# leaner-forever/SEGS-SLAM

Hardware: AMD Instinct MI355X
Metric: mapper train-iters/sec (fwd+bwd raster) (higher is better)
Workload: dtype f32; 1 GPU; 1080p_3m: 3000000 Gaussians, 1920x1080, 1 keyframe per GPU, fwd+bwd raster; P=3000000, P_visible=2096178, num_rendered=10472370, instances_binned=7913347, instances_live=6766534, width=1920, height=1080, parallelism=keyframe-dp1, forward=resident (no host sync), hipgraph=off

## Files before the change

include/segs_raster.h:

```cpp
#ifndef SEGS_RASTER_H_
#define SEGS_RASTER_H_

#include <stddef.h>
#include <stdint.h>

#ifdef __cplusplus
extern "C" {
#endif

#define SEGS_OK 0
#define SEGS_ERR_INVALID_ARGUMENT (-1)
#define SEGS_ERR_UNSUPPORTED (-2)
#define SEGS_ERR_ALLOC (-3)

typedef char* (*segs_alloc_fn)(void* ctx, size_t bytes);

const char* segs_last_error(void);

#define SEGS_RASTER_SKIP_NONPOSITIVE_OPACITY 1u
#define SEGS_RASTER_KEEP_DEAD_INSTANCES 2u
#define SEGS_RASTER_GATHER_TILES_TOUCHED 4u
#define SEGS_RASTER_TEST_NARROW_PACK 8u
#define SEGS_RASTER_UNFUSED_BINNING 16u
#define SEGS_RASTER_TIGHT_BINNING 32u
#define SEGS_RASTER_MFMA_MOMENTS 64u
uint32_t segs_raster_set_flags(uint32_t flags);

uint32_t* segs_raster_set_status_mirror(uint32_t* host_mapped_status);

size_t segs_geometry_bytes(int P);
size_t segs_image_bytes(int width, int height);
size_t segs_binning_bytes(int num_rendered);

int segs_rasterize_forward(segs_alloc_fn geometry_alloc, void* geometry_ctx,
                           segs_alloc_fn binning_alloc, void* binning_ctx,
                           segs_alloc_fn image_alloc, void* image_ctx,
                           int P, int D, int M,
                           const float* background, int width, int height,
                           const float* means3D, const float* shs, const float* colors_precomp,
                           const float* opacities, const float* scales, float scale_modifier,
                           const float* rotations, const float* cov3D_precomp,
                           const float* viewmatrix, const float* projmatrix, const float* cam_pos,
                           float tan_fovx, float tan_fovy, int prefiltered,
                           float* out_color, int* radii, void* stream, int* num_rendered);

int segs_rasterize_backward(int P, int D, int M, int R,
                            const float* background, int width, int height,
                            const float* means3D, const float* shs, const float* colors_precomp,
                            const float* scales, float scale_modifier, const float* rotations,
                            const float* cov3D_precomp, const float* viewmatrix, const float* projmatrix,
                            const float* campos, float tan_fovx, float tan_fovy, const int* radii,
                            char* geom_buffer, char* binning_buffer, char* image_buffer,
                            const float* dL_dpix, float* dL_dmean2D, float* dL_dconic, float* dL_dopacity,
                            float* dL_dcolor, float* dL_dmean3D, float* dL_dcov3D, float* dL_dsh,
                            float* dL_dscale, float* dL_drot, void* stream);

int segs_visible_filter(int P, int M, int width, int height, const float* means3D, const float* scales,
                        float scale_modifier, const float* rotations, const float* cov3D_precomp,
                        const float* viewmatrix, const float* projmatrix, float tan_fovx, float tan_fovy,
                        int prefiltered, int* radii, void* stream);

int segs_visible_filter_log_scales(int P, int width, int height, const float* means3D, const float* scaling_log, int stride,
                                   const float* rotations, const float* viewmatrix, const float* projmatrix, float tan_fovx,
                                   float tan_fovy, int* radii, void* stream);

int segs_mark_visible(int P, const float* means3D, const float* viewmatrix, const float* projmatrix,
                      uint8_t* present, void* stream);

int segs_project2_image(int P, int D, int M, int width, int height, const float* means3D, const float* shs,
                        const float* colors_precomp, const float* opacities, const float* scales,
                        float scale_modifier, const float* rotations, const float* cov3D_precomp,
                        const float* viewmatrix, const float* projmatrix, const float* cam_pos,
                        float tan_fovx, float tan_fovy, int prefiltered, float* out_color, float* points_image,
                        int* radii, void* stream);

int segs_debug_unpack_geometry(const char* geom_buffer, int P, const int* radii, float* means2D ,
                               float* conic_opacity , float* depths , uint32_t* tiles_touched ,
                               uint32_t* point_offsets , float* rgb , void* stream);
int segs_debug_unpack_binning(const char* binning_buffer, const char* geom_buffer, int P, int R, int width, int height,
                              uint64_t* keys_sorted , uint32_t* point_list , void* stream);
int segs_debug_instance_values(const char* binning_buffer, int R, uint32_t* values , void* stream);
int segs_debug_unpack_image(const char* image_buffer, int width, int height, uint32_t* ranges ,
                            float* final_T , uint32_t* n_contrib , void* stream);

int segs_debug_preprocess_backward(int P, int width, int height, const float* means3D, const int* radii,
                                   const float* scales, float scale_modifier, const float* rotations,
                                   const float* cov3D_precomp, const float* viewmatrix, const float* projmatrix,
                                   float tan_fovx, float tan_fovy, const float* dL_dmean2D, const float* dL_dconic,
                                   float* dL_dmean3D, float* dL_dcov3D, float* dL_dscale, float* dL_drot, void* stream);

int segs_sort_pairs(const uint64_t* keys_in, const uint32_t* vals_in, uint64_t* keys_out, uint32_t* vals_out,
                    int n, int end_bit, char* temp, void* stream);

size_t segs_resident_binning_bytes(int P, int capacity);
int segs_rasterize_forward_resident(char* geom_buffer, char* binning_buffer, char* image_buffer, int capacity,
                                    int geom_rows, int P, int D, int M, const float* background, int width, int height,
                                    const float* means3D, const float* shs, const float* colors_precomp,
                                    const float* opacities, const float* scales, float scale_modifier,
                                    const float* rotations, const float* cov3D_precomp, const float* viewmatrix,
                                    const float* projmatrix, const float* cam_pos, float tan_fovx, float tan_fovy,
                                    float* out_color, int* radii, uint32_t* status, void* stream);
int segs_rasterize_backward_resident(char* geom_buffer, char* binning_buffer, char* image_buffer, int capacity,
                                     int geom_rows, int P, int D, int M, const float* background, int width, int height,
                                     const float* means3D, const float* shs, const float* scales, float scale_modifier,
                                     const float* rotations, const float* cov3D_precomp, const float* viewmatrix,
                                     const float* projmatrix, const float* campos, float tan_fovx, float tan_fovy,
                                     const int* radii, const float* dL_dpix, float* dL_dmean2D, float* dL_dconic,
                                     float* dL_dopacity, float* dL_dcolor, float* dL_dmean3D, float* dL_dcov3D,
                                     float* dL_dsh, float* dL_dscale, float* dL_drot, void* stream);

typedef struct segs_projection_targets {
  float* records;
  int* radii;
  uint32_t* tiles_touched;
  uint32_t* depth_keys;
  uint32_t* tile_ranges;
  uint32_t* depth_overflow;
  int num_tiles;
  uint32_t flags;
} segs_projection_targets;
int segs_resident_projection_targets(char* geom_buffer, char* binning_buffer, char* image_buffer, int capacity, int geom_rows,
                                     int P, int width, int height, int* radii, uint32_t* status, segs_projection_targets* out);
int segs_rasterize_forward_resident_projected(char* geom_buffer, char* binning_buffer, char* image_buffer, int capacity,
                                              int geom_rows, int P, const float* background, int width, int height,
                                              float* out_color, uint32_t* status, void* stream);

typedef struct segs_depth_outputs {
  float* depth;
  float* alpha;
} segs_depth_outputs;
typedef struct segs_depth_grads {
  const float* dL_ddepth;
  const float* dL_dalpha;
} segs_depth_grads;
int segs_rasterize_forward_depth(segs_alloc_fn geometry_alloc, void* geometry_ctx,
                                 segs_alloc_fn binning_alloc, void* binning_ctx,
                                 segs_alloc_fn image_alloc, void* image_ctx,
                                 int P, int D, int M,
                                 const float* background, int width, int height,
                                 const float* means3D, const float* shs, const float* colors_precomp,
                                 const float* opacities, const float* scales, float scale_modifier,
                                 const float* rotations, const float* cov3D_precomp,
                                 const float* viewmatrix, const float* projmatrix, const float* cam_pos,
                                 float tan_fovx, float tan_fovy, int prefiltered,
                                 float* out_color, int* radii, const segs_depth_outputs* depth_out, void* stream,
                                 int* num_rendered);
int segs_rasterize_backward_depth(int P, int D, int M, int R,
                                  const float* background, int width, int height,
                                  const float* means3D, const float* shs, const float* colors_precomp,
                                  const float* scales, float scale_modifier, const float* rotations,
                                  const float* cov3D_precomp, const float* viewmatrix, const float* projmatrix,
                                  const float* campos, float tan_fovx, float tan_fovy, const int* radii,
                                  char* geom_buffer, char* binning_buffer, char* image_buffer,
                                  const float* dL_dpix, float* dL_dmean2D, float* dL_dconic, float* dL_dopacity,
                                  float* dL_dcolor, float* dL_dmean3D, float* dL_dcov3D, float* dL_dsh,
                                  float* dL_dscale, float* dL_drot, const segs_depth_grads* depth_grads, void* stream);
int segs_rasterize_forward_resident_depth(char* geom_buffer, char* binning_buffer, char* image_buffer, int capacity,
                                          int geom_rows, int P, int D, int M, const float* background, int width, int height,
                                          const float* means3D, const float* shs, const float* colors_precomp,
                                          const float* opacities, const float* scales, float scale_modifier,
                                          const float* rotations, const float* cov3D_precomp, const float* viewmatrix,
                                          const float* projmatrix, const float* cam_pos, float tan_fovx, float tan_fovy,
                                          float* out_color, int* radii, uint32_t* status, const segs_depth_outputs* depth_out,
                                          void* stream);
int segs_rasterize_forward_resident_projected_depth(char* geom_buffer, char* binning_buffer, char* image_buffer, int capacity,
                                                    int geom_rows, int P, const float* background, int width, int height,
                                                    float* out_color, uint32_t* status, const segs_depth_outputs* depth_out,
                                                    void* stream);
int segs_rasterize_backward_resident_depth(char* geom_buffer, char* binning_buffer, char* image_buffer, int capacity,
                                           int geom_rows, int P, int D, int M, const float* background, int width, int height,
                                           const float* means3D, const float* shs, const float* scales, float scale_modifier,
                                           const float* rotations, const float* cov3D_precomp, const float* viewmatrix,
                                           const float* projmatrix, const float* campos, float tan_fovx, float tan_fovy,
                                           const int* radii, const float* dL_dpix, float* dL_dmean2D, float* dL_dconic,
                                           float* dL_dopacity, float* dL_dcolor, float* dL_dmean3D, float* dL_dcov3D,
                                           float* dL_dsh, float* dL_dscale, float* dL_drot, const segs_depth_grads* depth_grads,
                                           void* stream);

typedef struct segs_camera_grads {
  float* dL_dviewmatrix;
  float* dL_dprojmatrix;
  char* temp;
} segs_camera_grads;
size_t segs_camera_grad_temp_bytes(int rows);
int segs_rasterize_backward_camera(int P, int D, int M, int R,
                                   const float* background, int width, int height,
                                   const float* means3D, const float* shs, const float* colors_precomp,
                                   const float* scales, float scale_modifier, const float* rotations,
                                   const float* cov3D_precomp, const float* viewmatrix, const float* projmatrix,
                                   const float* campos, float tan_fovx, float tan_fovy, const int* radii,
                                   char* geom_buffer, char* binning_buffer, char* image_buffer,
                                   const float* dL_dpix, float* dL_dmean2D, float* dL_dconic, float* dL_dopacity,
                                   float* dL_dcolor, float* dL_dmean3D, float* dL_dcov3D, float* dL_dsh,
                                   float* dL_dscale, float* dL_drot, const segs_depth_grads* depth_grads,
                                   const segs_camera_grads* camera_grads, void* stream);
int segs_rasterize_backward_resident_camera(char* geom_buffer, char* binning_buffer, char* image_buffer, int capacity,
                                            int geom_rows, int P, int D, int M, const float* background, int width, int height,
                                            const float* means3D, const float* shs, const float* scales, float scale_modifier,
                                            const float* rotations, const float* cov3D_precomp, const float* viewmatrix,
                                            const float* projmatrix, const float* campos, float tan_fovx, float tan_fovy,
                                            const int* radii, const float* dL_dpix, float* dL_dmean2D, float* dL_dconic,
                                            float* dL_dopacity, float* dL_dcolor, float* dL_dmean3D, float* dL_dcov3D,
                                            float* dL_dsh, float* dL_dscale, float* dL_drot, const segs_depth_grads* depth_grads,
                                            const segs_camera_grads* camera_grads, void* stream);
int segs_debug_preprocess_backward_camera(int P, int width, int height, const float* means3D, const int* radii,
                                          const float* scales, float scale_modifier, const float* rotations,
                                          const float* cov3D_precomp, const float* viewmatrix, const float* projmatrix,
                                          float tan_fovx, float tan_fovy, const float* dL_dmean2D, const float* dL_dconic,
                                          float* dL_dmean3D, float* dL_dcov3D, float* dL_dscale, float* dL_drot,
                                          const float* dL_dz, const segs_camera_grads* camera_grads, void* stream);

int segs_profile_begin(unsigned kernel_mask);
int segs_profile_end(void);
int segs_profile_kernel_count(void);
const char* segs_profile_kernel_name(int id);
int segs_profile_query(int id, double* total_ms, long* launches);

#ifdef __cplusplus
}
#endif
#endif
```

segs-slam_amd/_capi.py:

```python
from __future__ import annotations

import ctypes as C
import os
import subprocess

_HERE = os.path.dirname(os.path.abspath(__file__))
CSRC = os.path.join(_HERE, "csrc")
LIB_PATH = os.environ.get("SEGS_RASTER_LIB") or os.path.join(CSRC, "libsegs_raster.so")

ALLOC_FN = C.CFUNCTYPE(C.c_void_p, C.c_void_p, C.c_size_t)


class NeuralDims(C.Structure):
    _fields_ = [("feat_dim", C.c_int), ("n_offsets", C.c_int), ("appearance_dim", C.c_int), ("use_feat_bank", C.c_int),
                ("add_opacity_dist", C.c_int), ("add_cov_dist", C.c_int), ("add_color_dist", C.c_int)]


class ProjectionTargets(C.Structure):
    _fields_ = [("records", C.c_void_p), ("radii", C.c_void_p), ("tiles_touched", C.c_void_p), ("depth_keys", C.c_void_p),
                ("tile_ranges", C.c_void_p), ("depth_overflow", C.c_void_p), ("num_tiles", C.c_int), ("flags", C.c_uint32)]


class DepthOutputs(C.Structure):
    _fields_ = [("depth", C.c_void_p), ("alpha", C.c_void_p)]


class DepthGrads(C.Structure):
    _fields_ = [("dL_ddepth", C.c_void_p), ("dL_dalpha", C.c_void_p)]


class CameraGrads(C.Structure):
    _fields_ = [("dL_dviewmatrix", C.c_void_p), ("dL_dprojmatrix", C.c_void_p), ("temp", C.c_void_p)]


class AdamSegment(C.Structure):
    _fields_ = [("offset", C.c_int64), ("count", C.c_int64), ("lr", C.c_double)]

_vp, _i, _f, _sz = C.c_void_p, C.c_int, C.c_float, C.c_size_t
SYMBOLS = {
    "segs_last_error": (C.c_char_p, []),
    "segs_raster_set_flags": (C.c_uint, [C.c_uint]),
    "segs_raster_set_status_mirror": (_vp, [_vp]),
    "segs_training_statis": (_i, [_i, _i] + [_vp] * 9),
    "segs_training_statis_guarded": (_i, [_i, _i] + [_vp] * 10),
    "segs_anchor_growing_temp_bytes": (_sz, [_i, _i]),
    "segs_anchor_growing_level": (_i, [_i, _i, _i, _i] + [_vp] * 7 + [_f, _f, _f, _i] + [_vp] * 5),
    "segs_neural_set_flags": (C.c_uint, [C.c_uint]),
    "segs_neural_param_layout": (_i, [_vp, _vp, _vp, _vp, _vp]),
    "segs_neural_temp_bytes": (_sz, [_vp, _i]),
    "segs_neural_forward": (_i, [_vp, _i] + [_vp] * 16),
    "segs_neural_forward_projected": (_i, [_vp, _i] + [_vp] * 16 + [_i, _i, _f, _f, _f, _vp, _vp]),
    "segs_neural_backward": (_i, [_vp, _i] + [_vp] * 17 + [_f, _vp, _vp, _vp]),
    "segs_geometry_bytes": (_sz, [_i]),
    "segs_image_bytes": (_sz, [_i, _i]),
    "segs_binning_bytes": (_sz, [_i]),
    "segs_rasterize_forward": (_i, [ALLOC_FN, _vp, ALLOC_FN, _vp, ALLOC_FN, _vp, _i, _i, _i, _vp, _i, _i, _vp, _vp, _vp,
                                     _vp, _vp, _f, _vp, _vp, _vp, _vp, _vp, _f, _f, _i, _vp, _vp, _vp, C.POINTER(_i)]),
    "segs_rasterize_backward": (_i, [_i, _i, _i, _i, _vp, _i, _i, _vp, _vp, _vp, _vp, _f, _vp, _vp, _vp, _vp, _vp, _f, _f,
                                      _vp, _vp, _vp, _vp, _vp, _vp, _vp, _vp, _vp, _vp, _vp, _vp, _vp, _vp, _vp]),
    "segs_resident_binning_bytes": (_sz, [_i, _i]),
    "segs_rasterize_forward_resident": (_i, [_vp, _vp, _vp, _i, _i, _i, _i, _i, _vp, _i, _i, _vp, _vp, _vp, _vp, _vp, _f, _vp, _vp, _vp,
                                              _vp, _vp, _f, _f, _vp, _vp, _vp, _vp]),
    "segs_resident_projection_targets": (_i, [_vp, _vp, _vp, _i, _i, _i, _i, _i, _vp, _vp, _vp]),
    "segs_rasterize_forward_resident_projected": (_i, [_vp, _vp, _vp, _i, _i, _i, _vp, _i, _i, _vp, _vp, _vp]),
    "segs_rasterize_backward_resident": (_i, [_vp, _vp, _vp, _i, _i, _i, _i, _i, _vp, _i, _i, _vp, _vp, _vp, _f, _vp, _vp, _vp, _vp, _vp,
                                               _f, _f, _vp, _vp, _vp, _vp, _vp, _vp, _vp, _vp, _vp, _vp, _vp, _vp]),
}
for _name in ("segs_rasterize_forward", "segs_rasterize_backward", "segs_rasterize_forward_resident",
              "segs_rasterize_forward_resident_projected", "segs_rasterize_backward_resident"):
    _res, _args = SYMBOLS[_name]
    _at = len(_args) - (2 if _name == "segs_rasterize_forward" else 1)
    SYMBOLS[_name + "_depth"] = (_res, _args[:_at] + [_vp] + _args[_at:])
for _name in ("segs_rasterize_backward", "segs_rasterize_backward_resident"):
    _res, _args = SYMBOLS[_name + "_depth"]
    SYMBOLS[_name + "_camera"] = (_res, _args[:-1] + [_vp] + _args[-1:])
SYMBOLS["segs_camera_grad_temp_bytes"] = (_sz, [_i])
SYMBOLS.update({
    "segs_visible_filter": (_i, [_i, _i, _i, _i, _vp, _vp, _f, _vp, _vp, _vp, _vp, _f, _f, _i, _vp, _vp]),
    "segs_visible_filter_log_scales": (_i, [_i, _i, _i, _vp, _vp, _i, _vp, _vp, _vp, _f, _f, _vp, _vp]),
    "segs_mark_visible": (_i, [_i, _vp, _vp, _vp, _vp, _vp]),
    "segs_project2_image": (_i, [_i, _i, _i, _i, _i, _vp, _vp, _vp, _vp, _vp, _f, _vp, _vp, _vp, _vp, _vp, _f, _f, _i,
                                  _vp, _vp, _vp, _vp]),
    "segs_debug_unpack_geometry": (_i, [_vp, _i, _vp, _vp, _vp, _vp, _vp, _vp, _vp, _vp]),
    "segs_debug_instance_values": (_i, [_vp, _i, _vp, _vp]),
    "segs_debug_unpack_binning": (_i, [_vp, _vp, _i, _i, _i, _i, _vp, _vp, _vp]),
    "segs_debug_unpack_image": (_i, [_vp, _i, _i, _vp, _vp, _vp, _vp]),
    "segs_debug_preprocess_backward": (_i, [_i, _i, _i, _vp, _vp, _vp, _f, _vp, _vp, _vp, _vp, _f, _f, _vp, _vp, _vp,
                                             _vp, _vp, _vp, _vp]),
    "segs_debug_preprocess_backward_camera": (_i, [_i, _i, _i, _vp, _vp, _vp, _f, _vp, _vp, _vp, _vp, _f, _f, _vp, _vp, _vp,
                                                    _vp, _vp, _vp, _vp, _vp, _vp]),
    "segs_sort_pairs": (_i, [_vp, _vp, _vp, _vp, _i, _i, _vp, _vp]),
    "segs_knn_temp_bytes": (_sz, [_i]),
    "segs_knn_mean_dist2": (_i, [_i, _vp, _vp, _vp, _vp]),
    "segs_transform_points": (_i, [_i, _vp, _vp, _vp, _vp]),
    "segs_scale_and_transform_points": (_i, [_i, _f, _vp, _vp, _vp, _vp, _vp, _vp, _vp]),
    "segs_reproject_depths_pinhole": (_i, [_i, _i, _f, _f, _f, _f, _vp, _vp, _vp, _vp]),
    "segs_search_neighborhood_depth": (_i, [_i, _i, _f, _f, _f, _f, _f, _vp, _vp, _vp, _vp, _vp, _vp, _vp]),
    "segs_l1_ssim_temp_bytes": (_sz, [_i, _i]),
    "segs_l1_ssim_loss": (_i, [_vp, _vp, _i, _i, _f, _vp, _vp, _vp, _vp]),
    "segs_freq_pyramid": (_i, [_vp, _i, _i, _i, _i, _vp, _vp, _vp, _vp]),
    "segs_spectrum_magnitude": (_i, [_vp, _sz, _vp, _vp]),
    "segs_freq_temp_bytes": (_sz, [_i, _i, _vp, _vp]),
    "segs_freq_spectrum_loss": (_i, [_i, _i, _vp, _vp, _vp, _vp, _vp, _vp, _vp, _vp, _vp]),
    "segs_freq_pyramid_backward_add": (_i, [_vp, _i, _i, _i, _i, _vp, _vp, _vp, _vp]),
    "segs_freq_plan_create": (_i, [_i, _i, _i, _vp, _f, _vp]),
    "segs_freq_plan_destroy": (None, [_vp]),
    "segs_freq_plan_levels": (_i, [_vp, _vp, _vp, _vp]),
    "segs_freq_target_floats": (_sz, [_vp]),
    "segs_freq_target": (_i, [_vp, _vp, _vp, _vp]),
    "segs_freq_loss": (_i, [_vp, _vp, _vp, _vp, _vp, _vp, _vp]),
    "segs_adam_step": (_i, [_vp, _vp, _vp, _vp, _vp, _i, C.c_double, C.c_double, C.c_double, C.c_int64, _f, _i, _vp]),
    "segs_adam_step_guarded": (_i, [_vp, _vp, _vp, _vp, _vp, _i, C.c_double, C.c_double, C.c_double, C.c_int64, _f, _i, _vp, _vp]),
    "segs_adam_step_device": (_i, [_vp, _vp, _vp, _vp, _vp, _i, C.c_double, C.c_double, C.c_double, _vp, _i, _f, _i, _vp, _vp]),
    "segs_adam_step_graph": (_i, [_vp, _vp, _vp, _vp, _vp, _i, _vp, C.c_double, C.c_double, C.c_double, _vp, _f, _i, _vp, _vp]),
    "segs_set_doubles": (_i, [_vp, _vp, _i, _vp]),
    "segs_profile_begin": (_i, [C.c_uint]),
    "segs_profile_end": (_i, []),
    "segs_profile_kernel_count": (_i, []),
    "segs_profile_kernel_name": (C.c_char_p, [_i]),
    "segs_profile_query": (_i, [_i, C.POINTER(C.c_double), C.POINTER(C.c_long)]),
})

_lib = None


def build(force: bool = False) -> str:
    cmd = ["make", "-C", CSRC, "-s", "-j4"] + (["-B"] if force else [])
    subprocess.check_call(cmd)
    return LIB_PATH


def lib() -> C.CDLL:
    global _lib
    if _lib is None:
        if not os.path.exists(LIB_PATH):
            raise RuntimeError(
                f"{LIB_PATH} is missing: the HIP extension must be built (python -c 'import __graft_entry__ as g; "
                "g.build()' or make -C segs-slam_amd/csrc). There is no CPU fallback.")
        import torch
        l = C.CDLL(LIB_PATH)
        for name, (res, args) in SYMBOLS.items():
            try:
                fn = getattr(l, name)
            except AttributeError as e:
                raise RuntimeError(f"libsegs_raster.so does not export {name}") from e
            fn.restype = res
            fn.argtypes = args
        _lib = l
    return _lib


class SegsError(RuntimeError):
    pass


def check(status: int, what: str) -> None:
    if status != 0:
        msg = lib().segs_last_error()
        raise SegsError(f"{what} failed with status {status}: {msg.decode() if msg else ''}")
```

segs-slam_amd/csrc/binning.hip:

```cpp
#include <hip/hip_runtime.h>
#include <cstdint>
#include "gs_layout.h"
#include "kernels.h"

namespace segs {

constexpr int PREFIX_ROWS = PREFIX_ROWS_PER_WG;

__global__ void __launch_bounds__(1024) scan_block_sums_kernel(uint32_t* __restrict__ block_sums, int nblocks,
                                                               const uint32_t* __restrict__ depth_range,
                                                               uint32_t* __restrict__ total) {
  __shared__ uint32_t w_sum[16], w_dmax[16], w_dnmin[16];
  const int tid = threadIdx.x, lane = tid & 63, wv = tid >> 6;
  uint32_t sum = 0, dmax = 0, dnmin = 0;
  for (int i = tid; i < nblocks; i += 1024) {
    sum += block_sums[i];
    dmax = max(dmax, depth_range[i]);
    dnmin = max(dnmin, depth_range[nblocks + i]);
  }
#pragma unroll
  for (int off = 32; off > 0; off >>= 1) {
    sum += __shfl_down(sum, off, 64);
    dmax = max(dmax, (uint32_t)__shfl_down((int)dmax, off, 64));
    dnmin = max(dnmin, (uint32_t)__shfl_down((int)dnmin, off, 64));
// ... 247 lines not shown
    if (col < nchunks) {
      constexpr int ND = 1 << BITS;
      for (int d = threadIdx.x; d < ND; d += SORT_THREADS) chunk_hist[(size_t)d * nchunks + col] = 0u;
    }
    return;
  }
  if (chunk_id >= nchunks) return;
  const int b0 = chunk_id * chunk_tiles;
  auto load_tile = [&](int b, K* dst) {
    const size_t wave_base = (size_t)b * SORT_TILE + (size_t)wv * (SORT_TILE / 4);
#pragma unroll
    for (int r = 0; r < SORT_ITEMS_PER_THREAD; r++) {
      const size_t i = wave_base + (size_t)r * 64 + lane;
      dst[r] = (b < nblocks && i < (size_t)n) ? keys[i] : (K)DEAD_KEY_OF(K);
    }
  };
  load_tile(b0, kreg);
  for (int t = 0; t < chunk_tiles; t++) {
    const int b = b0 + t;
    if (b >= nblocks) break;
    for (int i = tid; i < 4 * NDIG; i += SORT_THREADS) (&cnt[0][0])[i] = 0;
    if (t + 1 < chunk_tiles) load_tile(b + 1, knext);
    __syncthreads();
    const size_t wave_base = (size_t)b * SORT_TILE + (size_t)wv * (SORT_TILE / 4);
#pragma unroll
    for (int r = 0; r < SORT_ITEMS_PER_THREAD; r++) {
      const size_t i = wave_base + (size_t)r * 64 + lane;
      if (i < (size_t)n && !(drop_dead && kreg[r] == (K)DEAD_KEY_OF(K))) atomicAdd(&my[digit_of<BITS>(kreg[r], shift, km) & dmask], 1u);
    }
    __syncthreads();
#pragma unroll
    for (int j = 0; j < DPT; j++) {
      const int d = tid * DPT + j;
      tile_prefix[(size_t)b * NDIG + d] = running[j];
      running[j] += cnt[0][d] + cnt[1][d] + cnt[2][d] + cnt[3][d];
    }
    __syncthreads();
#pragma unroll
    for (int r = 0; r < SORT_ITEMS_PER_THREAD; r++) kreg[r] = knext[r];
  }
#pragma unroll
  for (int j = 0; j < DPT; j++) chunk_hist[(size_t)(tid * DPT + j) * nchunks + chunk_id] = running[j];
}

__global__ void __launch_bounds__(256) radix_scan_kernel(uint32_t* __restrict__ block_hist, int nblocks,
                                                         uint32_t* __restrict__ digit_totals) {
  constexpr int ITEMS = 8;
  __shared__ uint32_t wave_tot[4];
  const int tid = threadIdx.x, lane = tid & 63, wv = tid >> 6;
  uint32_t* row = block_hist + (size_t)blockIdx.x * nblocks;
  uint32_t carry = 0;
  for (int base = 0; base < nblocks; base += 256 * ITEMS) {
    const int i0 = base + tid * ITEMS;
    uint32_t v[ITEMS], sum = 0;
#pragma unroll
    for (int q = 0; q < ITEMS; q++) { v[q] = (i0 + q < nblocks) ? row[i0 + q] : 0u; sum += v[q]; }
    uint32_t x = sum;
#pragma unroll
    for (int off = 1; off < 64; off <<= 1) {
      const uint32_t y = __shfl_up(x, off, 64);
      if (lane >= off) x += y;
    }
    if (lane == 63) wave_tot[wv] = x;
    __syncthreads();
    uint32_t wbase = 0, total = 0;
#pragma unroll
    for (int w = 0; w < 4; w++) { const uint32_t t = wave_tot[w]; if (w < wv) wbase += t; total += t; }
    uint32_t run = carry + wbase + x - sum;
#pragma unroll
    for (int q = 0; q < ITEMS; q++) { if (i0 + q < nblocks) row[i0 + q] = run; run += v[q]; }
    carry += total;
    __syncthreads();
  }
  if (tid == 0) digit_totals[blockIdx.x] = carry;
}

template <typename K, int BITS, bool AUX>
__global__ void __launch_bounds__(SORT_THREADS) radix_scatter_kernel(
    const K* __restrict__ keys_in, const uint32_t* __restrict__ vals_in, K* __restrict__ keys_out,
    uint32_t* __restrict__ vals_out, int n, int shift, uint32_t dmin, int dbits, const uint32_t* __restrict__ tile_prefix,
    const uint32_t* __restrict__ chunk_prefix , const uint32_t* __restrict__ digit_totals,
    int nblocks, int nchunks, const uint32_t* __restrict__ n_dev, int drop_dead, uint32_t* __restrict__ n_live_out,
    const uint32_t* __restrict__ aux_in, uint32_t* __restrict__ aux_out, int nbits ,
    int chunk_tiles ,
    int pack_shift ,
    uint2* __restrict__ ranges_out ,
    uint32_t* __restrict__ status, uint32_t* __restrict__ status_mirror ,
    int write_keys ) {
  const KeyMap km{dmin, dbits};
  const uint32_t dmask = (1u << nbits) - 1u;
  if (ranges_out != nullptr && status != nullptr && blockIdx.x == 0 && threadIdx.x == 0) {
    const uint32_t ntot = status[0];
    const uint32_t over = (ntot > (uint32_t)n || status[2] != 0u) ? 1u : 0u;
    status[2] = 0u;
    status[3] = over;
    const uint32_t live = min(n_dev ? *n_dev : ntot, min(ntot, (uint32_t)n));
    status[1] = live;
    if (status_mirror) { status_mirror[0] = ntot; status_mirror[1] = live; status_mirror[3] = over; }
  }
  if (n_dev) n = (int)min(*n_dev, (uint32_t)n);
  constexpr int NDIG = 1 << BITS;
  constexpr int DPT = NDIG / SORT_THREADS;
  static_assert(NDIG % SORT_THREADS == 0 && BITS <= 11, "digit | rank << BITS must fit the rank of 2048 keys");
  __shared__ K s_keys[SORT_TILE];
  __shared__ uint32_t s_vals[SORT_TILE];
  __shared__ uint32_t s_aux[AUX ? SORT_TILE : 1];
  __shared__ uint32_t cnt[4][NDIG];
  __shared__ uint32_t local_start[NDIG];
  __shared__ int32_t gdelta[NDIG];
  __shared__ uint32_t scan_tmp[4];
  const int tid = threadIdx.x, lane = tid & 63, wv = tid >> 6;
  for (int i = tid; i < 4 * NDIG; i += SORT_THREADS) (&cnt[0][0])[i] = 0;
  __syncthreads();

#if defined(SEGS_MEASURE) && defined(SORT_TILE_IDENTITY)
  const int tile_id = (int)blockIdx.x;
#else
  const int tiles_in_use = (int)(((size_t)n + SORT_TILE - 1) / SORT_TILE);
  const int tiles_per_xcd = (tiles_in_use + 7) >> 3;
  const int tile_id = (int)(blockIdx.x & 7u) * tiles_per_xcd + (int)(blockIdx.x >> 3);
  if (tiles_in_use == 0 && n_live_out != nullptr && blockIdx.x == 0 && tid == 0) *n_live_out = 0u;
  if ((int)(blockIdx.x >> 3) >= tiles_per_xcd) return;
#endif
  if (tile_id >= nblocks) return;
  const size_t tile_base = (size_t)tile_id * SORT_TILE;
  const size_t wave_base = tile_base + (size_t)wv * (SORT_TILE / 4);
  const int nvalid = (size_t)n > tile_base ? (int)min((size_t)SORT_TILE, (size_t)n - tile_base) : 0;

  K key[SORT_ITEMS_PER_THREAD];
  uint32_t val[SORT_ITEMS_PER_THREAD];
  uint32_t aux[AUX ? SORT_ITEMS_PER_THREAD : 1];
  uint32_t drank[SORT_ITEMS_PER_THREAD];
  volatile uint32_t* my = cnt[wv];
#pragma unroll
  for (int r = 0; r < SORT_ITEMS_PER_THREAD; r++) {
    const size_t i = wave_base + (size_t)r * 64 + lane;
    const bool valid = i < (size_t)n;
    key[r] = valid ? keys_in[i] : (K)0;
    val[r] = vals_in ? (valid ? vals_in[i] : 0u) : (uint32_t)i;
    if (AUX) aux[r] = valid ? aux_in[val[r]] : 0u;
    if (!AUX && pack_shift > 0 && valid) val[r] |= min(aux_in[i], (0xFFFFFFFFu >> pack_shift)) << pack_shift;
  }
#pragma unroll
  for (int r = 0; r < SORT_ITEMS_PER_THREAD; r++) {
    const size_t i = wave_base + (size_t)r * 64 + lane;
    const bool valid = i < (size_t)n && !(drop_dead && key[r] == (K)DEAD_KEY_OF(K));
    const uint32_t d = valid ? (digit_of<BITS>(key[r], shift, km) & dmask) : 0u;
    const uint64_t vmask = __ballot(valid);
    const uint64_t peers = match_digit<BITS>(d, vmask, nbits);
    const uint32_t below = mbcnt(peers);
    uint32_t old = 0;
    if (valid) old = my[d];
    __builtin_amdgcn_wave_barrier();
    if (valid && below == 0) my[d] = old + (uint32_t)__popcll(peers);
    __builtin_amdgcn_wave_barrier();
    drank[r] = valid ? (d | ((old + below) << BITS)) : 0xFFFFFFFFu;
  }
  __syncthreads();

  uint32_t run[DPT], tot[DPT], thread_run = 0, thread_tot = 0;
#pragma unroll
  for (int j = 0; j < DPT; j++) {
    const int d = tid * DPT + j;
    uint32_t r = 0;
#pragma unroll
    for (int w = 0; w < 4; w++) { const uint32_t c = cnt[w][d]; cnt[w][d] = r; r += c; }
    run[j] = r; thread_run += r;
    tot[j] = digit_totals[d]; thread_tot += tot[j];
  }
  uint32_t x = thread_run;
#pragma unroll
  for (int off = 1; off < 64; off <<= 1) {
    uint32_t y = __shfl_up(x, off, 64);
    if (lane >= off) x += y;
  }
  if (lane == 63) scan_tmp[wv] = x;
  uint32_t tx = thread_tot;
#pragma unroll
  for (int off = 1; off < 64; off <<= 1) {
    uint32_t y = __shfl_up(tx, off, 64);
    if (lane >= off) tx += y;
  }
  __shared__ uint32_t tot_tmp[4];
  if (lane == 63) tot_tmp[wv] = tx;
  __syncthreads();
  uint32_t lbase = 0, gbase = 0;
  for (int w = 0; w < wv; w++) { lbase += scan_tmp[w]; gbase += tot_tmp[w]; }
  uint32_t lstart = lbase + x - thread_run, gstart = gbase + tx - thread_tot;
#pragma unroll
  for (int j = 0; j < DPT; j++) {
    const int d = tid * DPT + j;
    local_start[d] = lstart;
    gdelta[d] = (int32_t)(gstart + chunk_prefix[(size_t)d * nchunks + tile_id / chunk_tiles] +
                          tile_prefix[(size_t)tile_id * NDIG + d] - lstart);
    lstart += run[j]; gstart += tot[j];
  }
  const int nout = drop_dead ? (int)(scan_tmp[0] + scan_tmp[1] + scan_tmp[2] + scan_tmp[3]) : nvalid;
  if (n_live_out != nullptr && tile_id == 0 && tid == 0) *n_live_out = tot_tmp[0] + tot_tmp[1] + tot_tmp[2] + tot_tmp[3];
  __syncthreads();

#pragma unroll
  for (int r = 0; r < SORT_ITEMS_PER_THREAD; r++) {
    if (drank[r] != 0xFFFFFFFFu) {
      const uint32_t d = drank[r] & (uint32_t)(NDIG - 1);
      const uint32_t pos = local_start[d] + cnt[wv][d] + (drank[r] >> BITS);
      s_keys[pos] = key[r];
      s_vals[pos] = val[r];
      if (AUX) s_aux[pos] = aux[r];
    }
  }
  __syncthreads();
#pragma unroll 4
  for (int r = 0; r < SORT_ITEMS_PER_THREAD; r++) {
    const int lp = r * SORT_THREADS + tid;
    if (lp < nout) {
      const K k = s_keys[lp];
#if defined(SEGS_MEASURE) && defined(ABLATE_SCATTER_LINEAR)
      const size_t gp = tile_base + (size_t)lp + (size_t)(gdelta[digit_of<BITS>(k, shift, km) & dmask] & 0);
#else
      const size_t gp = (size_t)((int64_t)lp + (int64_t)gdelta[digit_of<BITS>(k, shift, km) & dmask]);
#endif
#if defined(SEGS_MEASURE) && defined(ABLATE_SCATTER_NO_STORE)
      if (k == (K)0x12345677 && gp == 77) keys_out[gp] = k;
      continue;
#endif
      if (write_keys) keys_out[gp] = k;
      vals_out[gp] = s_vals[lp];
      if (AUX) aux_out[gp] = s_aux[lp];
      if constexpr (sizeof(K) == 4) {
        if (ranges_out != nullptr) {
          const K prev = lp > 0 ? s_keys[lp - 1] : ~k, next = lp + 1 < nout ? s_keys[lp + 1] : ~k;
          if (k != prev) atomicMin(&ranges_out[k].x, (uint32_t)gp);
          if (k != next) atomicMax(&ranges_out[k].y, (uint32_t)gp + 1u);
        }
      }
    }
  }
}

#define SEGS_INSTANTIATE_RADIX(K, BITS)                                                                                          \
  template __global__ void radix_count_kernel<K, BITS>(const K*, int, int, uint32_t, int, uint32_t*, uint32_t*, int, int,       \
                                                       const uint32_t*, int, int, int);                                                  \
  template __global__ void radix_scatter_kernel<K, BITS, false>(const K*, const uint32_t*, K*, uint32_t*, int, int, uint32_t, int, \
                                                                const uint32_t*, const uint32_t*, const uint32_t*, int, int,        \
                                                                const uint32_t*, int, uint32_t*, const uint32_t*, uint32_t*, int, int, int, \
                                                                uint2*, uint32_t*, uint32_t*, int);
SEGS_INSTANTIATE_RADIX(uint64_t, 8)
SEGS_INSTANTIATE_RADIX(uint32_t, 8)
SEGS_INSTANTIATE_RADIX(uint32_t, 9)
SEGS_INSTANTIATE_RADIX(uint32_t, 11)
#undef SEGS_INSTANTIATE_RADIX
#define SEGS_INSTANTIATE_AUX(BITS)                                                                                                     \
  template __global__ void radix_scatter_kernel<uint32_t, BITS, true>(const uint32_t*, const uint32_t*, uint32_t*, uint32_t*, int, int, \
                                                                      uint32_t, int, const uint32_t*, const uint32_t*, const uint32_t*, \
                                                                      int, int, const uint32_t*, int, uint32_t*, const uint32_t*, uint32_t*, int, int, int, \
                                                                      uint2*, uint32_t*, uint32_t*, int);
SEGS_INSTANTIATE_AUX(8)
SEGS_INSTANTIATE_AUX(9)
#undef SEGS_INSTANTIATE_AUX

__global__ void __launch_bounds__(256) identify_tile_ranges_kernel(int L, const uint32_t* __restrict__ keys,
                                                                   uint2* __restrict__ ranges, const uint32_t* __restrict__ n_dev,
                                                                   uint32_t* __restrict__ status, uint32_t* __restrict__ status_mirror,
                                                                   const uint32_t* __restrict__ n_live ) {
  static_assert(RANGE_KEYS_PER_THREAD == 4, "one uint4 per thread");
  const int idx = blockIdx.x * 256 + threadIdx.x;
  if (n_dev) {
    const uint32_t n = *n_dev;
    if (idx == 0 && status) {
      const uint32_t over = (n > (uint32_t)L || status[2] != 0u) ? 1u : 0u;
      status[2] = 0u;
      status[3] = over;
      const uint32_t live = n_live ? min(*n_live, min(n, (uint32_t)L)) : min(n, (uint32_t)L);
      status[1] = live;
      if (status_mirror) { status_mirror[0] = n; status_mirror[1] = live; status_mirror[3] = over; }
    }
    L = (int)min(n, (uint32_t)L);
  }
  if (n_live) L = (int)min(*n_live, (uint32_t)L);
  const int i0 = idx * RANGE_KEYS_PER_THREAD;
  if (i0 >= L) return;
  uint32_t k[RANGE_KEYS_PER_THREAD];
  if (i0 + RANGE_KEYS_PER_THREAD <= L) {
    const uint4 v = *reinterpret_cast<const uint4*>(keys + i0);
    k[0] = v.x; k[1] = v.y; k[2] = v.z; k[3] = v.w;
  } else {
#pragma unroll
    for (int q = 0; q < RANGE_KEYS_PER_THREAD; q++) k[q] = i0 + q < L ? keys[i0 + q] : 0u;
  }
  uint32_t prev = i0 > 0 ? keys[i0 - 1] : 0u;
#pragma unroll
  for (int q = 0; q < RANGE_KEYS_PER_THREAD; q++) {
    const int i = i0 + q;
    if (i < L) {
      const uint32_t cur = k[q];
      if (i == 0) ranges[cur].x = 0;
      else if (cur != prev) { ranges[prev].y = i; ranges[cur].x = i; }
      if (i == L - 1) ranges[cur].y = L;
      prev = cur;
    }
  }
}

__global__ void __launch_bounds__(256) unpack_geometry_kernel(
    int P, const float* __restrict__ rec, const BinInfo* __restrict__ bin, const int* __restrict__ radii,
    float* __restrict__ means2D, float* __restrict__ conic_opacity, float* __restrict__ depths,
    uint32_t* __restrict__ tiles_touched, float* __restrict__ rgb) {
  const int idx = blockIdx.x * 256 + threadIdx.x;
  if (idx >= P) return;
  const bool vis = radii[idx] > 0;
  const float* r = rec + (size_t)idx * REC_DWORDS;
  means2D[2 * (size_t)idx + 0] = vis ? r[REC_X] : 0.f;
  means2D[2 * (size_t)idx + 1] = vis ? r[REC_Y] : 0.f;
  conic_opacity[4 * (size_t)idx + 0] = vis ? r[REC_CA] : 0.f;
  conic_opacity[4 * (size_t)idx + 1] = vis ? r[REC_CB] : 0.f;
  conic_opacity[4 * (size_t)idx + 2] = vis ? r[REC_CC] : 0.f;
  conic_opacity[4 * (size_t)idx + 3] = vis ? r[REC_O] : 0.f;
  depths[idx] = vis ? r[REC_DEPTH] : 0.f;
  tiles_touched[idx] = bin[idx].tiles_touched;
  if (rgb) {
    rgb[3 * (size_t)idx + 0] = vis ? r[REC_R] : 0.f;
    rgb[3 * (size_t)idx + 1] = vis ? r[REC_G] : 0.f;
    rgb[3 * (size_t)idx + 2] = vis ? r[REC_B] : 0.f;
  }
}

__global__ void __launch_bounds__(256) make_depth_keys_kernel(int P, const BinInfo* __restrict__ bin, uint32_t dcull,
                                                              uint32_t* __restrict__ keys, uint32_t* __restrict__ vals,
                                                              uint2* __restrict__ ranges, int num_tiles) {
  const int i = blockIdx.x * 256 + threadIdx.x;
  for (int t = i; t < num_tiles; t += gridDim.x * 256) ranges[t] = make_uint2(RANGE_EMPTY_START, 0u);
  if (i >= P) return;
  const uint4 b = reinterpret_cast<const uint4*>(bin)[i];
  keys[i] = b.w ? b.x : dcull;
  (void)vals;
}
__global__ void __launch_bounds__(256) ordered_block_sums_kernel(int P, const uint32_t* touched, const uint32_t* __restrict__ order,
                                                                 uint32_t* __restrict__ block_sums, uint32_t* sorted_touched,
                                                                 const uint32_t* __restrict__ ng_dev ,
                                                                 uint32_t* __restrict__ order_rw, int pack_shift) {
  __shared__ uint32_t wave_sums[4];
  const int ng = ng_dev ? (int)min(*ng_dev, (uint32_t)P) : P;
  uint32_t s = 0;
#pragma unroll
  for (int r = 0; r < PREFIX_ROWS; r++) {
    const int slot = (blockIdx.x * PREFIX_ROWS + r) * 256 + threadIdx.x;
    uint32_t v = 0u;
    if (slot < ng) {
      if (pack_shift > 0) {
        const uint32_t packed = order_rw[slot], idx = packed & ((1u << pack_shift) - 1u);
        v = packed >> pack_shift;
        if (v == (0xFFFFFFFFu >> pack_shift)) v = touched[idx];
        order_rw[slot] = idx;
      } else {
        v = order ? touched[order[slot]] : touched[slot];
      }
    }
    if (slot < P) sorted_touched[slot] = v;
    s += v;
  }
#pragma unroll
  for (int off = 32; off > 0; off >>= 1) s += __shfl_down(s, off, 64);
  if ((threadIdx.x & 63) == 0) wave_sums[threadIdx.x >> 6] = s;
  __syncthreads();
  if (threadIdx.x == 0) block_sums[blockIdx.x] = wave_sums[0] + wave_sums[1] + wave_sums[2] + wave_sums[3];
}
__global__ void __launch_bounds__(1024) point_offsets_kernel(int P, const BinInfo* __restrict__ bin, uint32_t* __restrict__ offsets) {
  __shared__ uint32_t wave_tot[16];
  __shared__ uint32_t carry_s;
  const int tid = threadIdx.x, lane = tid & 63, wv = tid >> 6;
  if (tid == 0) carry_s = 0;
  __syncthreads();
  for (int base = 0; base < P; base += 1024) {
    const int i = base + tid;
    uint32_t x = i < P ? bin[i].tiles_touched : 0u;
#pragma unroll
    for (int off = 1; off < 64; off <<= 1) {
      uint32_t y = __shfl_up(x, off, 64);
      if (lane >= off) x += y;
    }
    if (lane == 63) wave_tot[wv] = x;
    __syncthreads();
    uint32_t wbase = 0;
    for (int w = 0; w < wv; w++) wbase += wave_tot[w];
    const uint32_t carry = carry_s;
    if (i < P) offsets[i] = carry + wbase + x;
    __syncthreads();
    if (tid == 1023) carry_s = carry + wbase + x;
    __syncthreads();
  }
}

__global__ void __launch_bounds__(256) normalize_ranges_kernel(int num_tiles, uint2* __restrict__ ranges) {
  const int t = blockIdx.x * 256 + threadIdx.x;
  if (t < num_tiles && ranges[t].y == 0u) ranges[t].x = 0u;
}

__global__ void __launch_bounds__(256) strip_mask_kernel(int n, const uint32_t* __restrict__ vals, uint32_t* __restrict__ out) {
  const int i = blockIdx.x * 256 + threadIdx.x;
  if (i < n) out[i] = vals[i] & ID_MASK;
}

}

namespace segs {
__global__ void __launch_bounds__(256) rebuild_keys_kernel(int R, const uint32_t* __restrict__ tile_keys, const uint32_t* __restrict__ vals,
                                                           const BinInfo* __restrict__ bin, uint64_t* __restrict__ keys64) {
  const int i = blockIdx.x * 256 + threadIdx.x;
  if (i >= R) return;
  keys64[i] = ((uint64_t)tile_keys[i] << 32) | (uint64_t)bin[vals[i] & ID_MASK].depth_bits;
}
}
```

segs-slam_amd/csrc/capi.hip:

```cpp
#include <hip/hip_runtime.h>
#include <cstdio>
#include <cstdlib>
#include <algorithm>
#include <cstring>
#include <string>
#include <vector>
#include "../../include/segs_raster.h"
#include "gs_layout.h"
#include "kernels.h"

using namespace segs;

namespace {
thread_local std::string g_err;
}
int segs::set_error(int code, const char* what) {
  g_err = what;
  return code;
}
int segs::set_hip_error(hipError_t e, const char* where) {
  g_err = std::string(where) + ": " + hipGetErrorString(e);
  return (int)e > 0 ? (int)e : 1;
}

namespace {

thread_local uint32_t g_flags = 0u;
thread_local uint32_t* g_status_mirror = nullptr;

int fail(int code, const char* what) { return segs::set_error(code, what); }
int hip_fail(hipError_t e, const char* where) { return segs::set_hip_error(e, where); }
#define HIP_TRY(expr)                                   \
  do {                                                  \
    hipError_t _e = (expr);                             \
    if (_e != hipSuccess) return hip_fail(_e, #expr);   \
  } while (0)
#define LAUNCH_TRY(name)                                \
  do {                                                  \
    hipError_t _e = hipGetLastError();                  \
    if (_e != hipSuccess) return hip_fail(_e, name);    \
  } while (0)

enum KernelId { K_PREPROCESS_FWD = 0, K_SCAN, K_DUPLICATE, K_RADIX_COUNT, K_RADIX_SCAN, K_RADIX_SCATTER, K_RANGES,
                K_RENDER_FWD, K_RENDER_BWD, K_PREPROCESS_BWD, K_MEMSET, K_COUNT };
const char* const kKernelNames[K_COUNT] = {"preprocess_fwd_kernel", "scan_block_sums_kernel", "duplicate_with_keys_kernel",
                                           "radix_count_kernel", "radix_scan_kernel", "radix_scatter_kernel",
                                           "identify_tile_ranges_kernel", "render_fwd_kernel", "render_bwd_kernel",
                                           "preprocess_bwd_kernel", "memset"};
struct Profiler {
  unsigned mask = 0;
  std::vector<hipEvent_t> pool;
  size_t used = 0;
  struct Span { int id; size_t e0, e1; };
  std::vector<Span> spans;
  double total_ms[K_COUNT] = {0};
  long count[K_COUNT] = {0};
  hipEvent_t get() {
    if (used == pool.size()) { hipEvent_t e; if (hipEventCreate(&e) != hipSuccess) return nullptr; pool.push_back(e); }
    return pool[used++];
  }
} g_prof;
struct ProfScope {
  int id; hipStream_t st; size_t e0 = 0; bool on;
  ProfScope(int id_, hipStream_t st_) : id(id_), st(st_), on((g_prof.mask >> id_) & 1u) {
    if (on) { e0 = g_prof.used; hipEvent_t e = g_prof.get(); if (e) (void)hipEventRecord(e, st); else on = false; }
  }
  ~ProfScope() {
    if (on) { size_t e1 = g_prof.used; hipEvent_t e = g_prof.get(); if (e) { (void)hipEventRecord(e, st); g_prof.spans.push_back({id, e0, e1}); } }
  }
};
#define PROF(id) ProfScope _prof_scope_##id(id, st)

uint32_t getHigherMsb(uint32_t n) {
  uint32_t msb = sizeof(n) * 4, step = msb;
  while (step > 1) {
    step /= 2;
    if (n >> msb) msb += step; else msb -= step;
  }
  if (n >> msb) msb++;
  return msb;
}

int count_chunk_tiles(int nblocks) {
#ifdef SEGS_MEASURE
  static const int chunk_override = [] { const char* e = getenv("SEGS_COUNT_CHUNK"); const int v = e ? atoi(e) : 0; return (v == 1 || v == 2 || v == 4) ? v : 0; }();
  if (chunk_override > 0) return chunk_override;
#endif
  return nblocks <= 256 ? 1 : (nblocks <= 2048 ? 2 : SORT_COUNT_CHUNK_TILES);
}
struct SortFusion {
  uint2* ranges = nullptr;
  uint32_t* status = nullptr;
  uint32_t* status_mirror = nullptr;
  bool keep_sorted_keys = true;
};
template <typename K, int BITS = 8>
int sort_pairs(char* bin, const BinningLayout& L, int n, int end_bit, uint32_t dmin, int dbits, hipStream_t st,
               const uint32_t* n_dev = nullptr, bool drop_dead = false, bool iota_vals = false, const uint32_t* aux_in = nullptr,
               uint32_t* aux_final = nullptr, int pack_shift = 0 ,
               const SortFusion& fuse = SortFusion(), const K* first_keys = nullptr ) {
  if (n <= 0) return SEGS_OK;
  uint32_t* n_live = (uint32_t*)(bin + L.n_live);
  const int passes = (end_bit + BITS - 1) / BITS;
  int side = passes & 1;
  uint32_t* tile_prefix = (uint32_t*)(bin + L.tile_prefix);
  uint32_t* chunk_hist = (uint32_t*)(bin + L.chunk_hist);
  uint32_t* digit_totals = (uint32_t*)(bin + L.digit_totals);
  const int chunk_tiles = count_chunk_tiles(L.nblocks);
  const int nchunks = (L.nblocks + chunk_tiles - 1) / chunk_tiles;
  for (int p = 0; p < passes; p++) {
    const K* kin = (p == 0 && first_keys) ? first_keys : (const K*)(bin + L.keys[side]);
    const uint32_t* vin = (const uint32_t*)(bin + L.vals[side]);
    K* kout = (K*)(bin + L.keys[side ^ 1]);
    uint32_t* vout = (uint32_t*)(bin + L.vals[side ^ 1]);
    const int shift = BITS * p;
    const int drop = drop_dead && p == 0;
    const uint32_t* n_in = (drop_dead && p > 0) ? n_live : n_dev;
    const int nbits = std::min(BITS, end_bit - shift);
    { PROF(K_RADIX_COUNT);
    radix_count_kernel<K, BITS><<<(nchunks + 7) / 8 * 8, SORT_THREADS, 0, st>>>(kin, n, shift, dmin, dbits, tile_prefix, chunk_hist, L.nblocks, nchunks, n_in, drop, chunk_tiles, nbits);
    }
    LAUNCH_TRY("radix_count_kernel");
    const bool last = p == passes - 1;
    uint2* fr = last ? fuse.ranges : nullptr;
    uint32_t* fs = last ? fuse.status : nullptr;
    uint32_t* fm = last ? fuse.status_mirror : nullptr;
    const int wk = (last && !fuse.keep_sorted_keys) ? 0 : 1;
    { PROF(K_RADIX_SCAN);
    radix_scan_kernel<<<1 << BITS, 256, 0, st>>>(chunk_hist, nchunks, digit_totals);
    }
    LAUNCH_TRY("radix_scan_kernel");
    if (iota_vals && p == 0) vin = nullptr;
    const int scatter_grid = (L.nblocks + 7) / 8 * 8;
    { PROF(K_RADIX_SCATTER);
    if constexpr (sizeof(K) == 4) {
      if (aux_in && aux_final && p == passes - 1) {
        radix_scatter_kernel<K, BITS, true><<<scatter_grid, SORT_THREADS, 0, st>>>(kin, vin, kout, vout, n, shift, dmin, dbits, tile_prefix, chunk_hist,
                                                                        digit_totals, L.nblocks, nchunks, n_in, drop,
                                                                        drop ? n_live : nullptr, aux_in, aux_final, nbits, chunk_tiles, 0, fr, fs, fm, wk);
      } else {
        radix_scatter_kernel<K, BITS, false><<<scatter_grid, SORT_THREADS, 0, st>>>(kin, vin, kout, vout, n, shift, dmin, dbits, tile_prefix, chunk_hist,
                                                                         digit_totals, L.nblocks, nchunks, n_in, drop,
                                                                         drop ? n_live : nullptr, (pack_shift > 0 && p == 0) ? aux_in : nullptr, nullptr,
                                                                         nbits, chunk_tiles, (p == 0) ? pack_shift : 0, fr, fs, fm, wk);
      }
    } else {
      radix_scatter_kernel<K, BITS, false><<<scatter_grid, SORT_THREADS, 0, st>>>(kin, vin, kout, vout, n, shift, dmin, dbits, tile_prefix, chunk_hist,
                                                                       digit_totals, L.nblocks, nchunks, n_in, drop,
                                                                       drop ? n_live : nullptr, nullptr, nullptr, nbits, chunk_tiles, 0, nullptr, nullptr, nullptr, 1);
    }
    }
    LAUNCH_TRY("radix_scatter_kernel");
    side ^= 1;
  }
  return SEGS_OK;
}

struct Geom {
  GeomLayout L;
  char* base;
  float* rec() const { return (float*)(base + L.rec); }
  BinInfo* bin() const { return (BinInfo*)(base + L.bin); }
  uint32_t* offsets() const { return (uint32_t*)(base + L.offsets); }
  int* radii_internal() const { return (int*)(base + L.radii_internal); }
  uint32_t* block_sums() const { return (uint32_t*)(base + L.block_sums); }
  uint32_t* num_rendered() const { return (uint32_t*)(base + L.num_rendered); }
  uint32_t* clamped() const { return (uint32_t*)(base + L.clamped); }
  float* gacc() const { return (float*)(base + L.gacc); }
  uint32_t* touched() const { return (uint32_t*)(base + L.touched); }
};
Geom geom_at(char* p, int P) { return Geom{geom_layout(P), align_ptr(p)}; }
Geom geom_at(char* p, int P, int rows) {
  Geom g{geom_layout(rows), align_ptr(p)};
  g.L.P = P;
  g.L.nblocks = (P + 255) / 256;
  return g;
}

int run_preprocess(const Geom& G, int P, int W, int H, const float* means3D, const float* colors, const float* opac,
                   const float* scales, float mod, const float* rots, const float* cov3D_precomp, const float* view,
                   const float* proj, float tan_fovx, float tan_fovy, int* radii, const float* shs, int D, int M,
                   const float* cam_pos, hipStream_t st, uint32_t* depth_keys = nullptr, uint32_t* depth_vals = nullptr,
                   uint2* ranges = nullptr, uint32_t extra_flags = 0u, uint32_t* depth_overflow = nullptr) {
  const float focal_y = H / (2.0f * tan_fovy);
  const float focal_x = W / (2.0f * tan_fovx);
  const uint32_t gx = (W + TILE_X - 1) / TILE_X, gy = (H + TILE_Y - 1) / TILE_Y;
  { PROF(K_PREPROCESS_FWD);
  preprocess_fwd_kernel<<<G.L.nblocks, 256, 0, st>>>(P, means3D, scales, mod, rots, opac, colors, cov3D_precomp, view,
                                                     proj, W, H, tan_fovx, tan_fovy, focal_x, focal_y, gx, gy, radii,
                                                     G.rec(), G.bin(), G.block_sums(), G.block_sums() + (G.L.nblocks + 1), shs, D, M, cam_pos,
                                                     G.clamped(), g_flags | extra_flags, depth_keys, depth_vals, ranges, (int)(gx * gy),
                                                     depth_overflow, G.touched());
  }
  LAUNCH_TRY("preprocess_fwd_kernel");
  return SEGS_OK;
}

int run_binning(const Geom& G, char* bin, const BinningLayout& BL, const GaussSortLayout& GS, uint2* ranges, int P, int n_cap,
                const uint32_t* n_dev, uint32_t dmin, int dbits, uint32_t dcull, uint32_t gx, uint32_t gy, uint32_t* total_out,
                hipStream_t st, bool depth_keys_ready = false, bool drop_dead = false, bool nine_bit_depth = false,
                const uint32_t* depth_keys_src = nullptr ) {
  const int bit = (int)getHigherMsb(gx * gy);
  char* gbin = bin + GS.base;
  const BinningLayout& GL = GS.inner;
  const int gside = (nine_bit_depth ? (dbits + 8) / 9 : (dbits + 7) / 8) & 1;
  if (!depth_keys_ready) { PROF(K_DUPLICATE);
  make_depth_keys_kernel<<<G.L.nblocks, 256, 0, st>>>(P, G.bin(), dcull, (uint32_t*)(gbin + GL.keys[gside]), (uint32_t*)(gbin + GL.vals[gside]),
                                                      ranges, (int)(gx * gy));
  }
  LAUNCH_TRY("make_depth_keys_kernel");
  const bool drop_culled = depth_keys_ready;
  int idx_bits = 1;
  while (idx_bits < 32 && ((uint64_t)1 << idx_bits) < (uint64_t)P) idx_bits++;
  int pack_shift = (32 - idx_bits >= 6 && !(g_flags & SEGS_RASTER_GATHER_TILES_TOUCHED)) ? idx_bits : 0;
  if (pack_shift && (g_flags & SEGS_RASTER_TEST_NARROW_PACK)) pack_shift = 30;
  uint32_t* aux_final = pack_shift ? nullptr : G.offsets();
  int rc = nine_bit_depth ? sort_pairs<uint32_t, 9>(gbin, GL, P, dbits, dmin, dbits, st, nullptr, drop_culled, true, G.touched(), aux_final, pack_shift, SortFusion(), depth_keys_src)
                          : sort_pairs<uint32_t>(gbin, GL, P, dbits, dmin, dbits, st, nullptr, drop_culled, true, G.touched(), aux_final, pack_shift, SortFusion(), depth_keys_src);
  if (rc) return rc;
  uint32_t* order = (uint32_t*)(gbin + GL.vals[0]);
  const uint32_t* ng_dev = drop_culled ? (const uint32_t*)(gbin + GL.n_live) : nullptr;
  uint32_t* sums2 = (uint32_t*)(bin + GS.block_sums);
  uint32_t* first_owner = (uint32_t*)(bin + GS.first_owner);
  const int prefix_wgs = (P + 256 * PREFIX_ROWS_PER_WG - 1) / (256 * PREFIX_ROWS_PER_WG);
  { PROF(K_SCAN);
  ordered_block_sums_kernel<<<prefix_wgs, 256, 0, st>>>(P, pack_shift ? G.touched() : G.offsets(), nullptr, sums2, G.offsets(), ng_dev, order, pack_shift);
  }
  LAUNCH_TRY("ordered_block_sums_kernel");
#ifdef SEGS_MEASURE
  static const bool no_wide = getenv("SEGS_NO_WIDE_DIGIT") != nullptr;
#else
  constexpr bool no_wide = false;
#endif
  const bool wide_digit = !no_wide && bit <= 11 && BL.nblocks <= SORT_WIDE_MAX_TILES;
  const int tpasses = wide_digit ? 1 : (bit + 7) / 8;
  const int side = tpasses & 1;
  { PROF(K_SCAN);
  ordered_offsets_kernel<<<prefix_wgs, 256, 0, st>>>(P, sums2, G.offsets(), total_out, ng_dev, first_owner,
                                                      (uint32_t)(n_cap / EMIT_SLOTS_PER_WG + 2));
  }
  LAUNCH_TRY("ordered_offsets_kernel");
  const bool unfused = (g_flags & SEGS_RASTER_UNFUSED_BINNING) != 0u;
  { PROF(K_DUPLICATE);
  duplicate_with_keys_kernel<<<(n_cap + EMIT_SLOTS_PER_WG - 1) / EMIT_SLOTS_PER_WG, 256, 0, st>>>(P, n_cap, G.rec(), order, G.offsets(),
                                                                    (uint32_t*)(bin + BL.keys[side]), (uint32_t*)(bin + BL.vals[side]), gx, n_dev,
                                                                    drop_dead ? 1 : 0, ng_dev, first_owner);
  }
  LAUNCH_TRY("duplicate_with_keys_kernel");
  SortFusion fuse;
  const bool fused_ranges = !unfused && tpasses >= 2;
  if (fused_ranges) {
    fuse.ranges = ranges;
    fuse.status = n_dev ? total_out : nullptr;
    fuse.status_mirror = n_dev ? g_status_mirror : nullptr;
    fuse.keep_sorted_keys = n_dev == nullptr;
  }
  rc = wide_digit ? sort_pairs<uint32_t, 11>(bin, BL, n_cap, bit, 0u, 0, st, n_dev, drop_dead, false, nullptr, nullptr, 0, fuse)
                  : sort_pairs<uint32_t>(bin, BL, n_cap, bit, 0u, 0, st, n_dev, drop_dead, false, nullptr, nullptr, 0, fuse);
  if (rc) return rc;
  if (!fused_ranges) { PROF(K_RANGES);
  identify_tile_ranges_kernel<<<(n_cap + 256 * RANGE_KEYS_PER_THREAD - 1) / (256 * RANGE_KEYS_PER_THREAD), 256, 0, st>>>(n_cap, (const uint32_t*)(bin + BL.keys[0]), ranges, n_dev,
                                                                   n_dev ? total_out : nullptr, n_dev ? g_status_mirror : nullptr,
                                                                   drop_dead ? (const uint32_t*)(bin + BL.n_live) : nullptr);
  }
  LAUNCH_TRY("identify_tile_ranges_kernel");
  return SEGS_OK;
}

int launch_render_fwd(uint32_t tiles, const uint2* ranges, const uint32_t* point_list, int width, int height, const float* rec,
                      const float* background, float* final_T, uint32_t* n_contrib, float* out_color, const segs_depth_outputs* dout,
                      hipStream_t st) {
  PROF(K_RENDER_FWD);
  if (dout && (dout->depth || dout->alpha))
    render_fwd_depth_kernel<<<tiles, 256, 0, st>>>(ranges, point_list, width, height, rec, background, final_T, n_contrib, out_color,
                                                   dout->depth, dout->alpha);
  else
    render_fwd_kernel<<<tiles, 256, 0, st>>>(ranges, point_list, width, height, rec, background, final_T, n_contrib, out_color);
  LAUNCH_TRY("render_fwd_kernel");
  return SEGS_OK;
}

int camera_grads_begin(const segs_camera_grads* cam, const float* shs, bool empty, hipStream_t st, bool* live) {
  *live = false;
  if (!cam) return SEGS_OK;
  if (!cam->dL_dviewmatrix || !cam->dL_dprojmatrix || !cam->temp) return fail(SEGS_ERR_INVALID_ARGUMENT, "segs_camera_grads: null field");
  if (shs) return fail(SEGS_ERR_INVALID_ARGUMENT, "camera gradients need colors_precomp: the SH colours depend on campos, which they do not cover");
  if (empty) {
    HIP_TRY(hipMemsetAsync(cam->dL_dviewmatrix, 0, 16 * sizeof(float), st));
    HIP_TRY(hipMemsetAsync(cam->dL_dprojmatrix, 0, 16 * sizeof(float), st));
    return SEGS_OK;
  }
  *live = true;
  return SEGS_OK;
}
float* camera_partials(const segs_camera_grads* cam) { return (float*)align_ptr(cam->temp); }
int camera_grads_finish(const segs_camera_grads* cam, int nblocks, hipStream_t st) {
  camera_grad_reduce_kernel<<<1, 960, 0, st>>>(camera_partials(cam), nblocks, cam->dL_dviewmatrix, cam->dL_dprojmatrix);
  LAUNCH_TRY("camera_grad_reduce_kernel");
  return SEGS_OK;
}

}

extern "C" {

const char* segs_last_error(void) { return g_err.c_str(); }

uint32_t* segs_raster_set_status_mirror(uint32_t* host_mapped_status) {
  uint32_t* old = g_status_mirror;
  g_status_mirror = host_mapped_status;
  return old;
}

uint32_t segs_raster_set_flags(uint32_t flags) {
  const uint32_t old = g_flags;
  g_flags = flags;
  return old;
}

size_t segs_geometry_bytes(int P) { return geom_layout(P < 0 ? 0 : P).total; }
size_t segs_image_bytes(int width, int height) { return image_layout(width, height).total; }
size_t segs_binning_bytes(int num_rendered) { return binning_layout(num_rendered < 0 ? 0 : num_rendered).total; }

static int rasterize_forward_impl(segs_alloc_fn geometry_alloc, void* geometry_ctx, segs_alloc_fn binning_alloc, void* binning_ctx,
                           segs_alloc_fn image_alloc, void* image_ctx, int P, int D, int M, const float* background,
                           int width, int height, const float* means3D, const float* shs, const float* colors_precomp,
                           const float* opacities, const float* scales, float scale_modifier, const float* rotations,
                           const float* cov3D_precomp, const float* viewmatrix, const float* projmatrix,
                           const float* cam_pos, float tan_fovx, float tan_fovy, int prefiltered, float* out_color,
                           int* radii, const segs_depth_outputs* dout, void* stream, int* num_rendered) {
  (void)prefiltered;
  hipStream_t st = (hipStream_t)stream;
  if (!geometry_alloc || !binning_alloc || !image_alloc) return fail(SEGS_ERR_INVALID_ARGUMENT, "null allocator callback");
  if (P < 0 || width <= 0 || height <= 0) return fail(SEGS_ERR_INVALID_ARGUMENT, "bad P / image size");
  if (P > MAX_GAUSSIANS) return fail(SEGS_ERR_INVALID_ARGUMENT, "P exceeds 2^28 Gaussians (sort values carry a 4-bit quadrant mask)");
  if (!background || !out_color || !viewmatrix || !projmatrix || !num_rendered) return fail(SEGS_ERR_INVALID_ARGUMENT, "null required pointer");
  if (P > 0 && (!means3D || !opacities)) return fail(SEGS_ERR_INVALID_ARGUMENT, "null means3D/opacities");
  if (P > 0 && !colors_precomp) {
    if (!shs || !cam_pos || M <= 0 || D < 0 || (D + 1) * (D + 1) > M || D > 3)
      return fail(SEGS_ERR_INVALID_ARGUMENT, "need colors_precomp, or shs + cam_pos with (D+1)^2 <= M, D <= 3");
  }
  if (P > 0 && !cov3D_precomp && (!scales || !rotations)) return fail(SEGS_ERR_INVALID_ARGUMENT, "need scales+rotations or cov3D_precomp");
  const uint32_t gx = (width + TILE_X - 1) / TILE_X, gy = (height + TILE_Y - 1) / TILE_Y;
  if (gx > 0xFFFFu || gy > 0xFFFFu) return fail(SEGS_ERR_INVALID_ARGUMENT, "image too large for 16-bit tile coordinates");

  const GeomLayout GL = geom_layout(P);
  char* geom_raw = geometry_alloc(geometry_ctx, GL.total);
  const ImageLayout IL = image_layout(width, height);
  char* img_raw = image_alloc(image_ctx, IL.total);
  if (!geom_raw || !img_raw) return fail(SEGS_ERR_ALLOC, "allocator callback returned null");
  Geom G = geom_at(geom_raw, P);
  char* img = align_ptr(img_raw);
  if (!radii) radii = G.radii_internal();

  int R = 0;
  uint32_t hdr[3] = {0u, 0u, 0u};
  const bool tight = (g_flags & SEGS_RASTER_TIGHT_BINNING) != 0u;
  uint2* const ranges_early = (uint2*)(img + IL.ranges);
  bool fast_keys = tight;
  if (P > 0) {
    int rc = run_preprocess(G, P, width, height, means3D, colors_precomp, opacities, cov3D_precomp ? nullptr : scales,
                            scale_modifier, rotations, cov3D_precomp, viewmatrix, projmatrix, tan_fovx, tan_fovy, radii, shs, D, M,
                            cam_pos, st, fast_keys ? (uint32_t*)G.bin() : nullptr, nullptr, fast_keys ? ranges_early : nullptr,
                            tight ? PREPROCESS_TIGHT_RECT : 0u);
    if (rc) return rc;
    { PROF(K_SCAN);
    scan_block_sums_kernel<<<1, 1024, 0, st>>>(G.block_sums(), G.L.nblocks, G.block_sums() + (G.L.nblocks + 1), G.num_rendered());
    }
    LAUNCH_TRY("scan_block_sums_kernel");
    HIP_TRY(hipMemcpyAsync(hdr, G.num_rendered(), sizeof(hdr), hipMemcpyDeviceToHost, st));
    HIP_TRY(hipStreamSynchronize(st));
    R = (int)hdr[0];
    if (R < 0) return fail(SEGS_ERR_INVALID_ARGUMENT, "num_rendered overflows int32");
    if (fast_keys && R > 0 && (hdr[2] - DEPTH_KEY_MIN) >= ((1u << DEPTH_KEY_BITS) - 1u)) {
      fast_keys = false;
      rc = run_preprocess(G, P, width, height, means3D, colors_precomp, opacities, cov3D_precomp ? nullptr : scales, scale_modifier,
                          rotations, cov3D_precomp, viewmatrix, projmatrix, tan_fovx, tan_fovy, radii, shs, D, M, cam_pos, st, nullptr,
                          nullptr, nullptr, PREPROCESS_TIGHT_RECT);
      if (rc) return rc;
    }
  }
  const BinningLayout BL = binning_layout(R);
  const GaussSortLayout GS = gauss_sort_layout(R, P);
  char* bin_raw = binning_alloc(binning_ctx, GS.total);
  if (!bin_raw) return fail(SEGS_ERR_ALLOC, "binning allocator returned null");
  char* bin = align_ptr(bin_raw);

  uint2* ranges = (uint2*)(img + IL.ranges);
  if (R == 0) {
    PROF(K_MEMSET);
    HIP_TRY(hipMemsetAsync(ranges, 0, (size_t)gx * gy * sizeof(uint2), st));
  }
  if (R > 0) {
    const uint32_t dmin = ~hdr[1], dspan = hdr[2] - dmin + 1u;
    int dbits = 1;
    while (dbits < 32 && (dspan >> dbits) != 0u) dbits++;
    uint32_t* total_scratch = (uint32_t*)(bin + GS.block_sums) + G.L.nblocks;
    const bool nine = (dbits + 8) / 9 < (dbits + 7) / 8;
    int rc = fast_keys ? run_binning(G, bin, BL, GS, ranges, P, R, nullptr, DEPTH_KEY_MIN, DEPTH_KEY_BITS, 0xFFFFFFFFu, gx, gy, total_scratch,
                                     st, true, true, true, (const uint32_t*)G.bin())
                       : run_binning(G, bin, BL, GS, ranges, P, R, nullptr, dmin, dbits, dmin + dspan, gx, gy, total_scratch, st, false, tight, nine);
    if (rc) return rc;
  }
  const int rc = launch_render_fwd(gx * gy, ranges, (const uint32_t*)(bin + BL.vals[0]), width, height, G.rec(), background,
                                   (float*)(img + IL.final_T), (uint32_t*)(img + IL.n_contrib), out_color, dout, st);
  if (rc) return rc;
  *num_rendered = R;
  return SEGS_OK;
}

int segs_rasterize_forward(segs_alloc_fn geometry_alloc, void* geometry_ctx, segs_alloc_fn binning_alloc, void* binning_ctx,
                           segs_alloc_fn image_alloc, void* image_ctx, int P, int D, int M, const float* background,
                           int width, int height, const float* means3D, const float* shs, const float* colors_precomp,
                           const float* opacities, const float* scales, float scale_modifier, const float* rotations,
                           const float* cov3D_precomp, const float* viewmatrix, const float* projmatrix,
                           const float* cam_pos, float tan_fovx, float tan_fovy, int prefiltered, float* out_color,
                           int* radii, void* stream, int* num_rendered) {
  return rasterize_forward_impl(geometry_alloc, geometry_ctx, binning_alloc, binning_ctx, image_alloc, image_ctx, P, D, M, background,
                                width, height, means3D, shs, colors_precomp, opacities, scales, scale_modifier, rotations, cov3D_precomp,
                                viewmatrix, projmatrix, cam_pos, tan_fovx, tan_fovy, prefiltered, out_color, radii, nullptr, stream,
                                num_rendered);
}

int segs_rasterize_forward_depth(segs_alloc_fn geometry_alloc, void* geometry_ctx, segs_alloc_fn binning_alloc, void* binning_ctx,
                                 segs_alloc_fn image_alloc, void* image_ctx, int P, int D, int M, const float* background,
                                 int width, int height, const float* means3D, const float* shs, const float* colors_precomp,
                                 const float* opacities, const float* scales, float scale_modifier, const float* rotations,
                                 const float* cov3D_precomp, const float* viewmatrix, const float* projmatrix,
                                 const float* cam_pos, float tan_fovx, float tan_fovy, int prefiltered, float* out_color,
                                 int* radii, const segs_depth_outputs* depth_out, void* stream, int* num_rendered) {
  return rasterize_forward_impl(geometry_alloc, geometry_ctx, binning_alloc, binning_ctx, image_alloc, image_ctx, P, D, M, background,
                                width, height, means3D, shs, colors_precomp, opacities, scales, scale_modifier, rotations, cov3D_precomp,
                                viewmatrix, projmatrix, cam_pos, tan_fovx, tan_fovy, prefiltered, out_color, radii, depth_out, stream,
                                num_rendered);
}

static int rasterize_backward_impl(int P, int D, int M, int R, const float* background, int width, int height,
                            const float* means3D, const float* shs, const float* scales,
                            float scale_modifier, const float* rotations, const float* cov3D_precomp,
                            const float* viewmatrix, const float* projmatrix, const float* campos, float tan_fovx,
                            float tan_fovy, const int* radii, char* geom_buffer, char* binning_buffer, char* image_buffer,
                            const float* dL_dpix, float* dL_dmean2D, float* dL_dconic, float* dL_dopacity, float* dL_dcolor,
                            float* dL_dmean3D, float* dL_dcov3D, float* dL_dsh, float* dL_dscale, float* dL_drot, void* stream,
                            bool self_clean, int geom_rows, const segs_depth_grads* dgrad, const segs_camera_grads* cam) {
  hipStream_t st = (hipStream_t)stream;
  if (P < 0 || R < 0 || width <= 0 || height <= 0) return fail(SEGS_ERR_INVALID_ARGUMENT, "bad sizes");
  if (geom_rows < P) return fail(SEGS_ERR_INVALID_ARGUMENT, "geom_rows must be >= P");
  bool cam_live = false;
  if (int rc = camera_grads_begin(cam, shs, P == 0 || R == 0, st, &cam_live)) return rc;
  if (P == 0) return SEGS_OK;
  if (shs && (!campos || !dL_dsh || M <= 0)) return fail(SEGS_ERR_INVALID_ARGUMENT, "SH path needs campos, dL_dsh and M > 0");
  if (!geom_buffer || !binning_buffer || !image_buffer || !dL_dpix || !background || !means3D || !viewmatrix || !projmatrix)
    return fail(SEGS_ERR_INVALID_ARGUMENT, "null required pointer");
  if (!dL_dmean2D || !dL_dopacity || !dL_dcolor || !dL_dmean3D || (cov3D_precomp && !dL_dcov3D))
    return fail(SEGS_ERR_INVALID_ARGUMENT, "null gradient output");
  if (!cov3D_precomp && (!scales || !rotations || !dL_dscale || !dL_drot))
    return fail(SEGS_ERR_INVALID_ARGUMENT, "need scales+rotations (+ their gradient outputs) or cov3D_precomp");
  Geom G = geom_at(geom_buffer, P, geom_rows);
  if (!radii) radii = G.radii_internal();
  const ImageLayout IL = image_layout(width, height);
  const BinningLayout BL = binning_layout(R);
  char* img = align_ptr(image_buffer);
  char* bin = align_ptr(binning_buffer);
  const uint32_t gx = (width + TILE_X - 1) / TILE_X, gy = (height + TILE_Y - 1) / TILE_Y;
  const float focal_y = height / (2.0f * tan_fovy), focal_x = width / (2.0f * tan_fovx);

  if (!self_clean) { PROF(K_MEMSET);
  HIP_TRY(hipMemsetAsync(G.gacc(), 0, (size_t)P * GACC_DWORDS * 4, st));
  }
  const float* dL_ddepth = dgrad ? dgrad->dL_ddepth : nullptr;
  const float* dL_dalpha = dgrad ? dgrad->dL_dalpha : nullptr;
  const bool depth_form = dL_ddepth || dL_dalpha;
  if (R > 0 && depth_form) {
    { PROF(K_RENDER_BWD);
    render_bwd_depth_kernel<<<(gx * gy + 7) / 8 * 32, 64, 0, st>>>((const uint2*)(img + IL.ranges), (const uint32_t*)(bin + BL.vals[0]), width,
                                                                  height, G.rec(), background, (const float*)(img + IL.final_T),
                                                                  (const uint32_t*)(img + IL.n_contrib), dL_dpix, G.gacc(), gx * gy,
                                                                  dL_ddepth, dL_dalpha);
    }
    LAUNCH_TRY("render_bwd_depth_kernel");
  } else if (R > 0) {
    { PROF(K_RENDER_BWD);
    static const bool mfma_env = [] { const char* e = getenv("SEGS_RENDER_BWD_MFMA"); return e && e[0] == '1'; }();
    ((mfma_env || (g_flags & SEGS_RASTER_MFMA_MOMENTS)) ? render_bwd_mfma_kernel : render_bwd_kernel)<<<(gx * gy + 7) / 8 * 32, 64, 0, st>>>((const uint2*)(img + IL.ranges), (const uint32_t*)(bin + BL.vals[0]), width,
                                                    height, G.rec(), background, (const float*)(img + IL.final_T),
                                                    (const uint32_t*)(img + IL.n_contrib), dL_dpix, G.gacc(), gx * gy);
    }
    LAUNCH_TRY("render_bwd_kernel");
  }
  { PROF(K_PREPROCESS_BWD);
  auto* const kernel = cam_live ? (dL_ddepth ? preprocess_bwd_kernel<true, true> : preprocess_bwd_kernel<false, true>)
                                : (dL_ddepth ? preprocess_bwd_kernel<true, false> : preprocess_bwd_kernel<false, false>);
  kernel<<<G.L.nblocks, 256, 0, st>>>(P, means3D, radii, cov3D_precomp ? nullptr : scales, rotations,
                                                     scale_modifier, cov3D_precomp, viewmatrix, projmatrix, focal_x, focal_y,
                                                     tan_fovx, tan_fovy, G.gacc(), (float)width, (float)height, dL_dmean2D, dL_dconic, dL_dopacity, dL_dcolor,
                                                     dL_dmean3D, dL_dcov3D, dL_dscale, dL_drot, self_clean ? 1 : 0, nullptr,
                                                     cam_live ? camera_partials(cam) : nullptr);
  LAUNCH_TRY("preprocess_bwd_kernel");
  if (cam_live)
    if (int rc = camera_grads_finish(cam, G.L.nblocks, st)) return rc;
  }
  if (shs) {
    sh_backward_kernel<<<G.L.nblocks, 256, 0, st>>>(P, means3D, radii, shs, D, M, campos, G.clamped(), dL_dcolor, dL_dmean3D, dL_dsh);
    LAUNCH_TRY("sh_backward_kernel");
  }
  return SEGS_OK;
}

int segs_rasterize_backward(int P, int D, int M, int R, const float* background, int width, int height,
                            const float* means3D, const float* shs, const float* colors_precomp, const float* scales,
                            float scale_modifier, const float* rotations, const float* cov3D_precomp,
                            const float* viewmatrix, const float* projmatrix, const float* campos, float tan_fovx,
                            float tan_fovy, const int* radii, char* geom_buffer, char* binning_buffer, char* image_buffer,
                            const float* dL_dpix, float* dL_dmean2D, float* dL_dconic, float* dL_dopacity, float* dL_dcolor,
                            float* dL_dmean3D, float* dL_dcov3D, float* dL_dsh, float* dL_dscale, float* dL_drot, void* stream) {
  (void)colors_precomp;
  return rasterize_backward_impl(P, D, M, R, background, width, height, means3D, shs, scales, scale_modifier, rotations,
                                 cov3D_precomp, viewmatrix, projmatrix, campos, tan_fovx, tan_fovy, radii, geom_buffer, binning_buffer,
                                 image_buffer, dL_dpix, dL_dmean2D, dL_dconic, dL_dopacity, dL_dcolor, dL_dmean3D, dL_dcov3D, dL_dsh,
                                 dL_dscale, dL_drot, stream, false, P, nullptr, nullptr);
}

int segs_rasterize_backward_depth(int P, int D, int M, int R, const float* background, int width, int height,
                                  const float* means3D, const float* shs, const float* colors_precomp, const float* scales,
                                  float scale_modifier, const float* rotations, const float* cov3D_precomp,
                                  const float* viewmatrix, const float* projmatrix, const float* campos, float tan_fovx,
                                  float tan_fovy, const int* radii, char* geom_buffer, char* binning_buffer, char* image_buffer,
                                  const float* dL_dpix, float* dL_dmean2D, float* dL_dconic, float* dL_dopacity, float* dL_dcolor,
                                  float* dL_dmean3D, float* dL_dcov3D, float* dL_dsh, float* dL_dscale, float* dL_drot,
                                  const segs_depth_grads* depth_grads, void* stream) {
  (void)colors_precomp;
  return rasterize_backward_impl(P, D, M, R, background, width, height, means3D, shs, scales, scale_modifier, rotations,
                                 cov3D_precomp, viewmatrix, projmatrix, campos, tan_fovx, tan_fovy, radii, geom_buffer, binning_buffer,
                                 image_buffer, dL_dpix, dL_dmean2D, dL_dconic, dL_dopacity, dL_dcolor, dL_dmean3D, dL_dcov3D, dL_dsh,
                                 dL_dscale, dL_drot, stream, false, P, depth_grads, nullptr);
}

size_t segs_camera_grad_temp_bytes(int rows) { return align_up((size_t)((rows < 0 ? 0 : rows) + 255) / 256 * CAM_SUMS * sizeof(float)) + ALIGN; }

int segs_rasterize_backward_camera(int P, int D, int M, int R, const float* background, int width, int height,
                                   const float* means3D, const float* shs, const float* colors_precomp, const float* scales,
                                   float scale_modifier, const float* rotations, const float* cov3D_precomp,
                                   const float* viewmatrix, const float* projmatrix, const float* campos, float tan_fovx,
                                   float tan_fovy, const int* radii, char* geom_buffer, char* binning_buffer, char* image_buffer,
                                   const float* dL_dpix, float* dL_dmean2D, float* dL_dconic, float* dL_dopacity, float* dL_dcolor,
                                   float* dL_dmean3D, float* dL_dcov3D, float* dL_dsh, float* dL_dscale, float* dL_drot,
                                   const segs_depth_grads* depth_grads, const segs_camera_grads* camera_grads, void* stream) {
  (void)colors_precomp;
  return rasterize_backward_impl(P, D, M, R, background, width, height, means3D, shs, scales, scale_modifier, rotations,
                                 cov3D_precomp, viewmatrix, projmatrix, campos, tan_fovx, tan_fovy, radii, geom_buffer, binning_buffer,
                                 image_buffer, dL_dpix, dL_dmean2D, dL_dconic, dL_dopacity, dL_dcolor, dL_dmean3D, dL_dcov3D, dL_dsh,
                                 dL_dscale, dL_drot, stream, false, P, depth_grads, camera_grads);
}

static int visible_filter_impl(int P, int width, int height, const float* means3D, const float* scales, int log_scale_stride,
                               float scale_modifier, const float* rotations, const float* cov3D_precomp, const float* viewmatrix,
                               const float* projmatrix, float tan_fovx, float tan_fovy, int* radii, void* stream);

int segs_visible_filter(int P, int M, int width, int height, const float* means3D, const float* scales,
                        float scale_modifier, const float* rotations, const float* cov3D_precomp, const float* viewmatrix,
                        const float* projmatrix, float tan_fovx, float tan_fovy, int prefiltered, int* radii, void* stream) {
  (void)M; (void)prefiltered;
  return visible_filter_impl(P, width, height, means3D, scales, 0, scale_modifier, rotations, cov3D_precomp, viewmatrix, projmatrix,
                             tan_fovx, tan_fovy, radii, stream);
}

int segs_visible_filter_log_scales(int P, int width, int height, const float* means3D, const float* scaling_log, int stride,
                                   const float* rotations, const float* viewmatrix, const float* projmatrix, float tan_fovx,
                                   float tan_fovy, int* radii, void* stream) {
  if (stride < 3 || !scaling_log || !rotations) return fail(SEGS_ERR_INVALID_ARGUMENT, "need log-scales (stride >= 3) and rotations");
  return visible_filter_impl(P, width, height, means3D, scaling_log, stride, 1.0f, rotations, nullptr, viewmatrix, projmatrix, tan_fovx,
                             tan_fovy, radii, stream);
}

static int visible_filter_impl(int P, int width, int height, const float* means3D, const float* scales, int log_scale_stride,
                               float scale_modifier, const float* rotations, const float* cov3D_precomp, const float* viewmatrix,
                               const float* projmatrix, float tan_fovx, float tan_fovy, int* radii, void* stream) {
  hipStream_t st = (hipStream_t)stream;
  if (P < 0 || width <= 0 || height <= 0) return fail(SEGS_ERR_INVALID_ARGUMENT, "bad sizes");
  if (P == 0) return SEGS_OK;
  if (!means3D || !viewmatrix || !projmatrix || !radii) return fail(SEGS_ERR_INVALID_ARGUMENT, "null required pointer");
  if (!cov3D_precomp && (!scales || !rotations)) return fail(SEGS_ERR_INVALID_ARGUMENT, "need scales+rotations or cov3D_precomp");
  const float focal_y = height / (2.0f * tan_fovy), focal_x = width / (2.0f * tan_fovx);
  const uint32_t gx = (width + TILE_X - 1) / TILE_X, gy = (height + TILE_Y - 1) / TILE_Y;
  visible_filter_kernel<<<(P + 255) / 256, 256, 0, st>>>(P, means3D, cov3D_precomp ? nullptr : scales, scale_modifier, rotations,
                                                         cov3D_precomp, viewmatrix, projmatrix, width, height, tan_fovx, tan_fovy,
                                                         focal_x, focal_y, gx, gy, radii, log_scale_stride);
  LAUNCH_TRY("visible_filter_kernel");
  return SEGS_OK;
}

int segs_mark_visible(int P, const float* means3D, const float* viewmatrix, const float* projmatrix, uint8_t* present, void* stream) {
  (void)projmatrix;
  hipStream_t st = (hipStream_t)stream;
  if (P < 0) return fail(SEGS_ERR_INVALID_ARGUMENT, "bad P");
  if (P == 0) return SEGS_OK;
  if (!means3D || !viewmatrix || !present) return fail(SEGS_ERR_INVALID_ARGUMENT, "null required pointer");
  mark_visible_kernel<<<(P + 255) / 256, 256, 0, st>>>(P, means3D, viewmatrix, present);
  LAUNCH_TRY("mark_visible_kernel");
  return SEGS_OK;
}

int segs_debug_unpack_geometry(const char* geom_buffer, int P, const int* radii, float* means2D, float* conic_opacity,
                               float* depths, uint32_t* tiles_touched, uint32_t* point_offsets, float* rgb, void* stream) {
  hipStream_t st = (hipStream_t)stream;
  if (P <= 0) return SEGS_OK;
  if (!geom_buffer || !means2D || !conic_opacity || !depths || !tiles_touched) return fail(SEGS_ERR_INVALID_ARGUMENT, "null pointer");
  Geom G = geom_at(const_cast<char*>(geom_buffer), P);
  if (!radii) radii = G.radii_internal();
  unpack_geometry_kernel<<<(P + 255) / 256, 256, 0, st>>>(P, G.rec(), G.bin(), radii, means2D, conic_opacity, depths, tiles_touched, rgb);
  LAUNCH_TRY("unpack_geometry_kernel");
  if (point_offsets) {
    point_offsets_kernel<<<1, 1024, 0, st>>>(P, G.bin(), point_offsets);
    LAUNCH_TRY("point_offsets_kernel");
  }
  return SEGS_OK;
}

int segs_debug_unpack_binning(const char* binning_buffer, const char* geom_buffer, int P, int R, int width, int height,
                              uint64_t* keys_sorted, uint32_t* point_list, void* stream) {
  (void)width; (void)height;
  hipStream_t st = (hipStream_t)stream;
  if (R <= 0) return SEGS_OK;
  if (!binning_buffer || (keys_sorted && (!geom_buffer || P <= 0))) return fail(SEGS_ERR_INVALID_ARGUMENT, "null pointer");
  const BinningLayout BL = binning_layout(R);
  const char* bin = align_ptr(binning_buffer);
  if (keys_sorted) {
    const Geom G = geom_at(const_cast<char*>(geom_buffer), P);
    rebuild_keys_kernel<<<(R + 255) / 256, 256, 0, st>>>(R, (const uint32_t*)(bin + BL.keys[0]), (const uint32_t*)(bin + BL.vals[0]),
                                                        G.bin(), keys_sorted);
    LAUNCH_TRY("rebuild_keys_kernel");
  }
  if (point_list) {
    strip_mask_kernel<<<(R + 255) / 256, 256, 0, st>>>(R, (const uint32_t*)(bin + BL.vals[0]), point_list);
    LAUNCH_TRY("strip_mask_kernel");
  }
  return SEGS_OK;
}

int segs_debug_instance_values(const char* binning_buffer, int R, uint32_t* values, void* stream) {
  if (R <= 0) return SEGS_OK;
  if (!binning_buffer || !values) return fail(SEGS_ERR_INVALID_ARGUMENT, "null pointer");
  const BinningLayout BL = binning_layout(R);
  HIP_TRY(hipMemcpyAsync(values, align_ptr(binning_buffer) + BL.vals[0], (size_t)R * 4, hipMemcpyDeviceToDevice, (hipStream_t)stream));
  return SEGS_OK;
}

int segs_debug_unpack_image(const char* image_buffer, int width, int height, uint32_t* ranges, float* final_T,
                            uint32_t* n_contrib, void* stream) {
  hipStream_t st = (hipStream_t)stream;
  if (!image_buffer) return fail(SEGS_ERR_INVALID_ARGUMENT, "null pointer");
  const ImageLayout IL = image_layout(width, height);
  const char* img = align_ptr(image_buffer);
  const size_t tiles = (size_t)((width + TILE_X - 1) / TILE_X) * ((height + TILE_Y - 1) / TILE_Y);
  if (ranges) {
    HIP_TRY(hipMemcpyAsync(ranges, img + IL.ranges, tiles * 8, hipMemcpyDeviceToDevice, st));
    normalize_ranges_kernel<<<(int)((tiles + 255) / 256), 256, 0, st>>>((int)tiles, (uint2*)ranges);
    LAUNCH_TRY("normalize_ranges_kernel");
  }
  if (final_T) HIP_TRY(hipMemcpyAsync(final_T, img + IL.final_T, (size_t)width * height * 4, hipMemcpyDeviceToDevice, st));
  if (n_contrib) HIP_TRY(hipMemcpyAsync(n_contrib, img + IL.n_contrib, (size_t)width * height * 4, hipMemcpyDeviceToDevice, st));
  return SEGS_OK;
}

int segs_debug_preprocess_backward(int P, int width, int height, const float* means3D, const int* radii, const float* scales,
                                   float scale_modifier, const float* rotations, const float* cov3D_precomp,
                                   const float* viewmatrix, const float* projmatrix, float tan_fovx, float tan_fovy,
                                   const float* dL_dmean2D, const float* dL_dconic, float* dL_dmean3D, float* dL_dcov3D,
                                   float* dL_dscale, float* dL_drot, void* stream) {
  hipStream_t st = (hipStream_t)stream;
  if (P <= 0) return SEGS_OK;
  if (!means3D || !radii || !viewmatrix || !projmatrix || !dL_dmean2D || !dL_dconic || !dL_dmean3D || !dL_dcov3D)
    return fail(SEGS_ERR_INVALID_ARGUMENT, "null pointer");
  const float focal_y = height / (2.0f * tan_fovy), focal_x = width / (2.0f * tan_fovx);
  preprocess_bwd_kernel<false, false><<<(P + 255) / 256, 256, 0, st>>>(P, means3D, radii, cov3D_precomp ? nullptr : scales, rotations,
                                                         scale_modifier, cov3D_precomp, viewmatrix, projmatrix, focal_x, focal_y,
                                                         tan_fovx, tan_fovy, nullptr, (float)width, (float)height, const_cast<float*>(dL_dmean2D),
                                                         const_cast<float*>(dL_dconic), nullptr, nullptr, dL_dmean3D, dL_dcov3D,
                                                         dL_dscale, dL_drot, 0, nullptr, nullptr);
  LAUNCH_TRY("preprocess_bwd_kernel");
  return SEGS_OK;
}

int segs_debug_preprocess_backward_camera(int P, int width, int height, const float* means3D, const int* radii, const float* scales,
                                          float scale_modifier, const float* rotations, const float* cov3D_precomp,
                                          const float* viewmatrix, const float* projmatrix, float tan_fovx, float tan_fovy,
                                          const float* dL_dmean2D, const float* dL_dconic, float* dL_dmean3D, float* dL_dcov3D,
                                          float* dL_dscale, float* dL_drot, const float* dL_dz, const segs_camera_grads* camera_grads,
                                          void* stream) {
  if (!camera_grads)
    return segs_debug_preprocess_backward(P, width, height, means3D, radii, scales, scale_modifier, rotations, cov3D_precomp, viewmatrix,
                                          projmatrix, tan_fovx, tan_fovy, dL_dmean2D, dL_dconic, dL_dmean3D, dL_dcov3D, dL_dscale, dL_drot,
                                          stream);
  hipStream_t st = (hipStream_t)stream;
  bool cam_live = false;
  if (int rc = camera_grads_begin(camera_grads, nullptr, P <= 0, st, &cam_live)) return rc;
  if (P <= 0) return SEGS_OK;
  if (!means3D || !radii || !viewmatrix || !projmatrix || !dL_dmean2D || !dL_dconic || !dL_dmean3D || !dL_dcov3D)
    return fail(SEGS_ERR_INVALID_ARGUMENT, "null pointer");
  const float focal_y = height / (2.0f * tan_fovy), focal_x = width / (2.0f * tan_fovx);
  const int nblocks = (P + 255) / 256;
  (dL_dz ? preprocess_bwd_kernel<true, true> : preprocess_bwd_kernel<false, true>)<<<nblocks, 256, 0, st>>>(
      P, means3D, radii, cov3D_precomp ? nullptr : scales, rotations, scale_modifier, cov3D_precomp, viewmatrix, projmatrix, focal_x,
      focal_y, tan_fovx, tan_fovy, nullptr, (float)width, (float)height, const_cast<float*>(dL_dmean2D), const_cast<float*>(dL_dconic),
      nullptr, nullptr, dL_dmean3D, dL_dcov3D, dL_dscale, dL_drot, 0, dL_dz, camera_partials(camera_grads));
  LAUNCH_TRY("preprocess_bwd_kernel");
  return camera_grads_finish(camera_grads, nblocks, st);
}

int segs_sort_pairs(const uint64_t* keys_in, const uint32_t* vals_in, uint64_t* keys_out, uint32_t* vals_out, int n,
                    int end_bit, char* temp, void* stream) {
  hipStream_t st = (hipStream_t)stream;
  if (n < 0 || end_bit <= 0 || end_bit > 64) return fail(SEGS_ERR_INVALID_ARGUMENT, "bad n / end_bit");
  if (n == 0) return SEGS_OK;
  if (!keys_in || !vals_in || !keys_out || !vals_out || !temp) return fail(SEGS_ERR_INVALID_ARGUMENT, "null pointer");
  const BinningLayout BL = binning_layout(n);
  char* bin = align_ptr(temp);
  const int passes = (end_bit + 7) / 8;
  const int side = passes & 1;
  HIP_TRY(hipMemcpyAsync(bin + BL.keys[side], keys_in, (size_t)n * 8, hipMemcpyDeviceToDevice, st));
  HIP_TRY(hipMemcpyAsync(bin + BL.vals[side], vals_in, (size_t)n * 4, hipMemcpyDeviceToDevice, st));
  int rc = sort_pairs<uint64_t>(bin, BL, n, end_bit, 0u, 32, st);
  if (rc) return rc;
  HIP_TRY(hipMemcpyAsync(keys_out, bin + BL.keys[0], (size_t)n * 8, hipMemcpyDeviceToDevice, st));
  HIP_TRY(hipMemcpyAsync(vals_out, bin + BL.vals[0], (size_t)n * 4, hipMemcpyDeviceToDevice, st));
  return SEGS_OK;
}

int segs_project2_image(int P, int D, int M, int width, int height, const float* means3D, const float* shs,
                        const float* colors_precomp, const float* opacities, const float* scales, float scale_modifier,
                        const float* rotations, const float* cov3D_precomp, const float* viewmatrix, const float* projmatrix,
                        const float* cam_pos, float tan_fovx, float tan_fovy, int prefiltered, float* out_color,
                        float* points_image, int* radii, void* stream) {
  (void)prefiltered;
  hipStream_t st = (hipStream_t)stream;
  if (P < 0 || width <= 0 || height <= 0) return fail(SEGS_ERR_INVALID_ARGUMENT, "bad sizes");
  if (P == 0) return SEGS_OK;
  if (!colors_precomp && (!shs || !cam_pos || M <= 0)) return fail(SEGS_ERR_INVALID_ARGUMENT, "need colors_precomp or shs + cam_pos");
  if (!means3D || !opacities || !viewmatrix || !projmatrix || !out_color || !points_image || !radii)
    return fail(SEGS_ERR_INVALID_ARGUMENT, "null required pointer");
  const GeomLayout GL = geom_layout(P);
  char* raw = nullptr;
  HIP_TRY(hipMallocAsync((void**)&raw, GL.total + (size_t)P * 4 * 8, st));
  Geom G = geom_at(raw, P);
  float* tmp = (float*)(align_ptr(raw) + GL.total - ALIGN);
  int rc = run_preprocess(G, P, width, height, means3D, colors_precomp, opacities, cov3D_precomp ? nullptr : scales,
                          scale_modifier, rotations, cov3D_precomp, viewmatrix, projmatrix, tan_fovx, tan_fovy, radii, shs, D, M,
                          cam_pos, st);
  if (rc == SEGS_OK) {
    unpack_geometry_kernel<<<(P + 255) / 256, 256, 0, st>>>(P, G.rec(), G.bin(), radii, points_image, tmp, tmp + (size_t)4 * P,
                                                            (uint32_t*)(tmp + (size_t)5 * P), out_color);
    hipError_t e = hipGetLastError();
    if (e != hipSuccess) rc = hip_fail(e, "unpack_geometry_kernel");
  }
  hipError_t fe = hipFreeAsync(raw, st);
  if (rc == SEGS_OK && fe != hipSuccess) return hip_fail(fe, "hipFreeAsync");
  return rc;
}


size_t segs_resident_binning_bytes(int P, int capacity) { return gauss_sort_layout(capacity < 0 ? 0 : capacity, P < 0 ? 0 : P).total; }

static int rasterize_forward_resident_impl(char* geom_buffer, char* binning_buffer, char* image_buffer, int capacity, int geom_rows, int P, int D, int M,
                                    const float* background, int width, int height, const float* means3D, const float* shs,
                                    const float* colors_precomp, const float* opacities, const float* scales, float scale_modifier,
                                    const float* rotations, const float* cov3D_precomp, const float* viewmatrix,
                                    const float* projmatrix, const float* cam_pos, float tan_fovx, float tan_fovy, float* out_color,
                                    int* radii, uint32_t* status, const segs_depth_outputs* dout, void* stream) {
  hipStream_t st = (hipStream_t)stream;
  if (P <= 0 || capacity <= 0 || width <= 0 || height <= 0) return fail(SEGS_ERR_INVALID_ARGUMENT, "bad sizes");
  if (geom_rows < P) return fail(SEGS_ERR_INVALID_ARGUMENT, "geom_rows (rows the geometry buffer was sized for) must be >= P");
  if (geom_rows > MAX_GAUSSIANS) return fail(SEGS_ERR_INVALID_ARGUMENT, "P exceeds 2^28 Gaussians");
  if (!geom_buffer || !binning_buffer || !image_buffer || !status || !background || !out_color || !viewmatrix || !projmatrix ||
      !means3D || !opacities)
    return fail(SEGS_ERR_INVALID_ARGUMENT, "null required pointer");
  if (!colors_precomp && (!shs || !cam_pos || M <= 0 || D < 0 || (D + 1) * (D + 1) > M || D > 3))
    return fail(SEGS_ERR_INVALID_ARGUMENT, "need colors_precomp, or shs + cam_pos with (D+1)^2 <= M, D <= 3");
  if (!cov3D_precomp && (!scales || !rotations)) return fail(SEGS_ERR_INVALID_ARGUMENT, "need scales+rotations or cov3D_precomp");
  const uint32_t gx = (width + TILE_X - 1) / TILE_X, gy = (height + TILE_Y - 1) / TILE_Y;
  if (gx > 0xFFFFu || gy > 0xFFFFu) return fail(SEGS_ERR_INVALID_ARGUMENT, "image too large for 16-bit tile coordinates");
  Geom G = geom_at(geom_buffer, P, geom_rows);
  char* img = align_ptr(image_buffer);
  char* bin = align_ptr(binning_buffer);
  const ImageLayout IL = image_layout(width, height);
  const BinningLayout BL = binning_layout(capacity);
  const GaussSortLayout GS = gauss_sort_layout(capacity, P);
  if (!radii) radii = G.radii_internal();
  uint2* ranges = (uint2*)(img + IL.ranges);
  char* gbin = bin + GS.base;
  const int gside = (3 & 1);
  int rc = run_preprocess(G, P, width, height, means3D, colors_precomp, opacities, cov3D_precomp ? nullptr : scales, scale_modifier,
                          rotations, cov3D_precomp, viewmatrix, projmatrix, tan_fovx, tan_fovy, radii, shs, D, M, cam_pos, st,
                          (uint32_t*)(gbin + GS.inner.keys[gside]), (uint32_t*)(gbin + GS.inner.vals[gside]), ranges,
                          (g_flags & SEGS_RASTER_KEEP_DEAD_INSTANCES) ? 0u : PREPROCESS_TIGHT_RECT, status + 2);
  if (rc) return rc;
  rc = run_binning(G, bin, BL, GS, ranges, P, capacity, status, DEPTH_KEY_MIN, DEPTH_KEY_BITS, 0xFFFFFFFFu, gx, gy, status, st, true,
                   (g_flags & SEGS_RASTER_KEEP_DEAD_INSTANCES) == 0u, true);
  if (rc) return rc;
  return launch_render_fwd(gx * gy, ranges, (const uint32_t*)(bin + BL.vals[0]), width, height, G.rec(), background,
                           (float*)(img + IL.final_T), (uint32_t*)(img + IL.n_contrib), out_color, dout, st);
}

int segs_rasterize_forward_resident(char* geom_buffer, char* binning_buffer, char* image_buffer, int capacity, int geom_rows, int P, int D, int M,
                                    const float* background, int width, int height, const float* means3D, const float* shs,
                                    const float* colors_precomp, const float* opacities, const float* scales, float scale_modifier,
                                    const float* rotations, const float* cov3D_precomp, const float* viewmatrix,
                                    const float* projmatrix, const float* cam_pos, float tan_fovx, float tan_fovy, float* out_color,
                                    int* radii, uint32_t* status, void* stream) {
  return rasterize_forward_resident_impl(geom_buffer, binning_buffer, image_buffer, capacity, geom_rows, P, D, M, background, width, height,
                                         means3D, shs, colors_precomp, opacities, scales, scale_modifier, rotations, cov3D_precomp,
                                         viewmatrix, projmatrix, cam_pos, tan_fovx, tan_fovy, out_color, radii, status, nullptr, stream);
}

int segs_rasterize_forward_resident_depth(char* geom_buffer, char* binning_buffer, char* image_buffer, int capacity, int geom_rows, int P,
                                          int D, int M, const float* background, int width, int height, const float* means3D,
                                          const float* shs, const float* colors_precomp, const float* opacities, const float* scales,
                                          float scale_modifier, const float* rotations, const float* cov3D_precomp,
                                          const float* viewmatrix, const float* projmatrix, const float* cam_pos, float tan_fovx,
                                          float tan_fovy, float* out_color, int* radii, uint32_t* status,
                                          const segs_depth_outputs* depth_out, void* stream) {
  return rasterize_forward_resident_impl(geom_buffer, binning_buffer, image_buffer, capacity, geom_rows, P, D, M, background, width, height,
                                         means3D, shs, colors_precomp, opacities, scales, scale_modifier, rotations, cov3D_precomp,
                                         viewmatrix, projmatrix, cam_pos, tan_fovx, tan_fovy, out_color, radii, status, depth_out, stream);
}

int segs_resident_projection_targets(char* geom_buffer, char* binning_buffer, char* image_buffer, int capacity, int geom_rows, int P,
                                     int width, int height, int* radii, uint32_t* status, segs_projection_targets* out) {
  if (P <= 0 || capacity <= 0 || width <= 0 || height <= 0 || !out) return fail(SEGS_ERR_INVALID_ARGUMENT, "bad sizes");
  if (geom_rows < P) return fail(SEGS_ERR_INVALID_ARGUMENT, "geom_rows (rows the geometry buffer was sized for) must be >= P");
  if (geom_rows > MAX_GAUSSIANS) return fail(SEGS_ERR_INVALID_ARGUMENT, "P exceeds 2^28 Gaussians");
  if (!geom_buffer || !binning_buffer || !image_buffer || !status) return fail(SEGS_ERR_INVALID_ARGUMENT, "null required pointer");
  const uint32_t gx = (width + TILE_X - 1) / TILE_X, gy = (height + TILE_Y - 1) / TILE_Y;
  if (gx > 0xFFFFu || gy > 0xFFFFu) return fail(SEGS_ERR_INVALID_ARGUMENT, "image too large for 16-bit tile coordinates");
  Geom G = geom_at(geom_buffer, P, geom_rows);
  const ImageLayout IL = image_layout(width, height);
  const GaussSortLayout GS = gauss_sort_layout(capacity, P);
  const int gside = (3 & 1);
  out->records = G.rec();
  out->radii = radii ? radii : G.radii_internal();
  out->tiles_touched = G.touched();
  out->depth_keys = (uint32_t*)(align_ptr(binning_buffer) + GS.base + GS.inner.keys[gside]);
  out->tile_ranges = (uint32_t*)(align_ptr(image_buffer) + IL.ranges);
  out->depth_overflow = status + 2;
  out->num_tiles = (int)(gx * gy);
  out->flags = (g_flags & SEGS_RASTER_KEEP_DEAD_INSTANCES) ? 0u : PREPROCESS_TIGHT_RECT;
  return SEGS_OK;
}

static int rasterize_forward_resident_projected_impl(char* geom_buffer, char* binning_buffer, char* image_buffer, int capacity,
                                                    int geom_rows, int P, const float* background, int width, int height, float* out_color,
                                                    uint32_t* status, const segs_depth_outputs* dout, void* stream) {
  hipStream_t st = (hipStream_t)stream;
  if (P <= 0 || capacity <= 0 || width <= 0 || height <= 0) return fail(SEGS_ERR_INVALID_ARGUMENT, "bad sizes");
  if (geom_rows < P) return fail(SEGS_ERR_INVALID_ARGUMENT, "geom_rows (rows the geometry buffer was sized for) must be >= P");
  if (geom_rows > MAX_GAUSSIANS) return fail(SEGS_ERR_INVALID_ARGUMENT, "P exceeds 2^28 Gaussians");
  if (!geom_buffer || !binning_buffer || !image_buffer || !status || !background || !out_color)
    return fail(SEGS_ERR_INVALID_ARGUMENT, "null required pointer");
  const uint32_t gx = (width + TILE_X - 1) / TILE_X, gy = (height + TILE_Y - 1) / TILE_Y;
  if (gx > 0xFFFFu || gy > 0xFFFFu) return fail(SEGS_ERR_INVALID_ARGUMENT, "image too large for 16-bit tile coordinates");
  Geom G = geom_at(geom_buffer, P, geom_rows);
  char* img = align_ptr(image_buffer);
  char* bin = align_ptr(binning_buffer);
  const ImageLayout IL = image_layout(width, height);
  const BinningLayout BL = binning_layout(capacity);
  const GaussSortLayout GS = gauss_sort_layout(capacity, P);
  uint2* ranges = (uint2*)(img + IL.ranges);
  int rc = run_binning(G, bin, BL, GS, ranges, P, capacity, status, DEPTH_KEY_MIN, DEPTH_KEY_BITS, 0xFFFFFFFFu, gx, gy, status, st, true,
                       (g_flags & SEGS_RASTER_KEEP_DEAD_INSTANCES) == 0u, true);
  if (rc) return rc;
  return launch_render_fwd(gx * gy, ranges, (const uint32_t*)(bin + BL.vals[0]), width, height, G.rec(), background,
                           (float*)(img + IL.final_T), (uint32_t*)(img + IL.n_contrib), out_color, dout, st);
}

int segs_rasterize_forward_resident_projected(char* geom_buffer, char* binning_buffer, char* image_buffer, int capacity, int geom_rows, int P,
                                              const float* background, int width, int height, float* out_color, uint32_t* status,
                                              void* stream) {
  return rasterize_forward_resident_projected_impl(geom_buffer, binning_buffer, image_buffer, capacity, geom_rows, P, background, width,
                                                   height, out_color, status, nullptr, stream);
}

int segs_rasterize_forward_resident_projected_depth(char* geom_buffer, char* binning_buffer, char* image_buffer, int capacity,
                                                    int geom_rows, int P, const float* background, int width, int height,
                                                    float* out_color, uint32_t* status, const segs_depth_outputs* depth_out,
                                                    void* stream) {
  return rasterize_forward_resident_projected_impl(geom_buffer, binning_buffer, image_buffer, capacity, geom_rows, P, background, width,
                                                   height, out_color, status, depth_out, stream);
}

int segs_rasterize_backward_resident(char* geom_buffer, char* binning_buffer, char* image_buffer, int capacity, int geom_rows, int P, int D, int M,
                                     const float* background, int width, int height, const float* means3D, const float* shs,
                                     const float* scales, float scale_modifier, const float* rotations, const float* cov3D_precomp,
                                     const float* viewmatrix, const float* projmatrix, const float* campos, float tan_fovx,
                                     float tan_fovy, const int* radii, const float* dL_dpix, float* dL_dmean2D, float* dL_dconic,
                                     float* dL_dopacity, float* dL_dcolor, float* dL_dmean3D, float* dL_dcov3D, float* dL_dsh,
                                     float* dL_dscale, float* dL_drot, void* stream) {
  return rasterize_backward_impl(P, D, M, capacity, background, width, height, means3D, shs, scales, scale_modifier, rotations,
                                 cov3D_precomp, viewmatrix, projmatrix, campos, tan_fovx, tan_fovy, radii, geom_buffer, binning_buffer,
                                 image_buffer, dL_dpix, dL_dmean2D, dL_dconic, dL_dopacity, dL_dcolor, dL_dmean3D, dL_dcov3D, dL_dsh,
                                 dL_dscale, dL_drot, stream, true, geom_rows, nullptr, nullptr);
}

int segs_rasterize_backward_resident_depth(char* geom_buffer, char* binning_buffer, char* image_buffer, int capacity, int geom_rows, int P,
                                           int D, int M, const float* background, int width, int height, const float* means3D,
                                           const float* shs, const float* scales, float scale_modifier, const float* rotations,
                                           const float* cov3D_precomp, const float* viewmatrix, const float* projmatrix,
                                           const float* campos, float tan_fovx, float tan_fovy, const int* radii, const float* dL_dpix,
                                           float* dL_dmean2D, float* dL_dconic, float* dL_dopacity, float* dL_dcolor, float* dL_dmean3D,
                                           float* dL_dcov3D, float* dL_dsh, float* dL_dscale, float* dL_drot,
                                           const segs_depth_grads* depth_grads, void* stream) {
  return rasterize_backward_impl(P, D, M, capacity, background, width, height, means3D, shs, scales, scale_modifier, rotations,
                                 cov3D_precomp, viewmatrix, projmatrix, campos, tan_fovx, tan_fovy, radii, geom_buffer, binning_buffer,
                                 image_buffer, dL_dpix, dL_dmean2D, dL_dconic, dL_dopacity, dL_dcolor, dL_dmean3D, dL_dcov3D, dL_dsh,
                                 dL_dscale, dL_drot, stream, true, geom_rows, depth_grads, nullptr);
}

int segs_rasterize_backward_resident_camera(char* geom_buffer, char* binning_buffer, char* image_buffer, int capacity, int geom_rows, int P,
                                            int D, int M, const float* background, int width, int height, const float* means3D,
                                            const float* shs, const float* scales, float scale_modifier, const float* rotations,
                                            const float* cov3D_precomp, const float* viewmatrix, const float* projmatrix,
                                            const float* campos, float tan_fovx, float tan_fovy, const int* radii, const float* dL_dpix,
                                            float* dL_dmean2D, float* dL_dconic, float* dL_dopacity, float* dL_dcolor, float* dL_dmean3D,
                                            float* dL_dcov3D, float* dL_dsh, float* dL_dscale, float* dL_drot,
                                            const segs_depth_grads* depth_grads, const segs_camera_grads* camera_grads, void* stream) {
  return rasterize_backward_impl(P, D, M, capacity, background, width, height, means3D, shs, scales, scale_modifier, rotations,
                                 cov3D_precomp, viewmatrix, projmatrix, campos, tan_fovx, tan_fovy, radii, geom_buffer, binning_buffer,
                                 image_buffer, dL_dpix, dL_dmean2D, dL_dconic, dL_dopacity, dL_dcolor, dL_dmean3D, dL_dcov3D, dL_dsh,
                                 dL_dscale, dL_drot, stream, true, geom_rows, depth_grads, camera_grads);
}

int segs_profile_begin(unsigned kernel_mask) {
  g_prof.mask = kernel_mask; g_prof.used = 0; g_prof.spans.clear();
  for (int i = 0; i < K_COUNT; i++) { g_prof.total_ms[i] = 0; g_prof.count[i] = 0; }
  return SEGS_OK;
}
int segs_profile_end(void) {
  g_prof.mask = 0;
  for (const auto& sp : g_prof.spans) {
    HIP_TRY(hipEventSynchronize(g_prof.pool[sp.e1]));
    float ms = 0.f;
    HIP_TRY(hipEventElapsedTime(&ms, g_prof.pool[sp.e0], g_prof.pool[sp.e1]));
    g_prof.total_ms[sp.id] += ms; g_prof.count[sp.id]++;
  }
  g_prof.spans.clear(); g_prof.used = 0;
  return SEGS_OK;
}
int segs_profile_kernel_count(void) { return K_COUNT; }
const char* segs_profile_kernel_name(int id) { return (id >= 0 && id < K_COUNT) ? kKernelNames[id] : ""; }
int segs_profile_query(int id, double* total_ms, long* launches) {
  if (id < 0 || id >= K_COUNT || !total_ms || !launches) return fail(SEGS_ERR_INVALID_ARGUMENT, "bad profile query");
  *total_ms = g_prof.total_ms[id]; *launches = g_prof.count[id];
  return SEGS_OK;
}

}
```

segs-slam_amd/csrc/gs_layout.h:

```cpp
#pragma once
#include <algorithm>
#include <cstddef>
#include <cstdint>

namespace segs {

constexpr int TILE_X = 16;
constexpr int TILE_Y = 16;
constexpr int NUM_CHANNELS = 3;

constexpr float LOG2E = 1.4426950408889634f;

constexpr int REC_DWORDS = 16;
enum RecField { REC_X = 0, REC_Y, REC_A2, REC_B2, REC_C2, REC_O, REC_R, REC_G, REC_B, REC_DEPTH, REC_RECT_MIN, REC_RECT_MAX, REC_CA, REC_CB, REC_CC };

struct BinInfo { uint32_t depth_bits, rect_min, rect_max, tiles_touched; };
constexpr uint32_t ID_BITS = 28;
constexpr uint32_t ID_MASK = (1u << ID_BITS) - 1u;
constexpr int MAX_GAUSSIANS = 1 << ID_BITS;

constexpr int GACC_DWORDS = 16;

constexpr size_t ALIGN = 256;
inline size_t align_up(size_t v, size_t a = ALIGN) { return (v + a - 1) / a * a; }

struct GeomLayout {
  size_t rec, bin, offsets, radii_internal, block_sums, clamped, num_rendered, gacc, touched, total;
  int P, nblocks;
};
inline GeomLayout geom_layout(int P) {
  GeomLayout g{};
  g.P = P;
  g.nblocks = (P + 255) / 256;
  size_t o = 0;
  g.rec = o;            o = align_up(o + (size_t)P * REC_DWORDS * 4);
  g.bin = o;            o = align_up(o + (size_t)P * sizeof(BinInfo));
  g.offsets = o;        o = align_up(o + (size_t)P * 4);
  g.radii_internal = o; o = align_up(o + (size_t)P * 4);
  g.block_sums = o;     o = align_up(o + (size_t)(g.nblocks + 1) * 4 * 3);
  g.clamped = o;        o = align_up(o + (size_t)P * 4);
  g.num_rendered = o;   o = align_up(o + 64);
  g.gacc = o;           o = align_up(o + (size_t)P * GACC_DWORDS * 4);
  g.touched = o;        o = align_up(o + (size_t)P * 4);
  g.total = o + ALIGN;
  return g;
}

struct ImageLayout {
  size_t ranges, final_T, n_contrib, total;
};
inline ImageLayout image_layout(int W, int H) {
  ImageLayout l{};
  const size_t tiles = (size_t)((W + TILE_X - 1) / TILE_X) * ((H + TILE_Y - 1) / TILE_Y);
  size_t o = 0;
  l.ranges = o;    o = align_up(o + tiles * 8);
  l.final_T = o;   o = align_up(o + (size_t)W * H * 4);
  l.n_contrib = o; o = align_up(o + (size_t)W * H * 4);
  l.total = o + ALIGN;
  return l;
}

#ifndef SEGS_SORT_ITEMS_PER_THREAD
#define SEGS_SORT_ITEMS_PER_THREAD 8
#endif
constexpr int SORT_ITEMS_PER_THREAD = SEGS_SORT_ITEMS_PER_THREAD;
constexpr int SORT_THREADS = 256;
constexpr int SORT_TILE = SORT_ITEMS_PER_THREAD * SORT_THREADS;
constexpr int PREFIX_ROWS_PER_WG = 8;
constexpr int EMIT_SLOTS_PER_WG = 512;
constexpr int SORT_COUNT_CHUNK_TILES = 4;
constexpr int RANGE_KEYS_PER_THREAD = 4;
constexpr int SORT_WIDE_DIGITS = 2048;
constexpr int SORT_WIDE_MAX_TILES = 1024;
constexpr int SORT_MAX_DIGITS = 512;

struct BinningLayout {
  size_t keys[2], vals[2], tile_prefix, chunk_hist, digit_totals, n_live, total;
  int nchunks;
  int R, nblocks;
};
inline BinningLayout binning_layout(int R) {
  BinningLayout b{};
  b.R = R;
  b.nblocks = (R + SORT_TILE - 1) / SORT_TILE;
  size_t o = 0;
  for (int i = 0; i < 2; i++) { b.keys[i] = o; o = align_up(o + (size_t)R * 8); }
  for (int i = 0; i < 2; i++) { b.vals[i] = o; o = align_up(o + (size_t)R * 4); }
  b.nchunks = b.nblocks;
  const size_t cols = (size_t)(b.nblocks > 0 ? b.nblocks : 1);
  const size_t matrix = std::max((size_t)SORT_MAX_DIGITS * cols, (size_t)SORT_WIDE_DIGITS * std::min(cols, (size_t)SORT_WIDE_MAX_TILES));
  b.tile_prefix = o;  o = align_up(o + matrix * 4);
  b.chunk_hist = o;   o = align_up(o + matrix * 4);
  b.digit_totals = o; o = align_up(o + SORT_WIDE_DIGITS * 4);
  b.n_live = o;       o = align_up(o + 4);
  b.total = o + ALIGN;
  return b;
}
struct GaussSortLayout {
  size_t base, block_sums, first_owner, total;
  BinningLayout inner;
};
inline GaussSortLayout gauss_sort_layout(int R, int P) {
  GaussSortLayout g{};
  g.inner = binning_layout(P);
  g.base = align_up(binning_layout(R).total);
  g.block_sums = g.base + align_up(g.inner.total);
  g.first_owner = g.block_sums + align_up((size_t)((P + 255) / 256 + 4) * 4);
  g.total = g.first_owner + align_up((size_t)(R / EMIT_SLOTS_PER_WG + 4) * 4) + ALIGN;
  return g;
}

inline char* align_ptr(char* p) { return (char*)(((uintptr_t)p + ALIGN - 1) / ALIGN * ALIGN); }
inline const char* align_ptr(const char* p) { return (const char*)(((uintptr_t)p + ALIGN - 1) / ALIGN * ALIGN); }

}
```

segs-slam_amd/csrc/kernels.h:

```cpp
#pragma once
#include <hip/hip_runtime.h>
#include <cstdint>
#include "gs_layout.h"

namespace segs {

int set_error(int code, const char* what);
int set_hip_error(hipError_t e, const char* where);


__global__ void preprocess_fwd_kernel(
    int P, const float* __restrict__ means3D, const float* __restrict__ scales, float mod,
    const float* __restrict__ rotations, const float* __restrict__ opacities, const float* __restrict__ colors,
    const float* __restrict__ cov3D_precomp, const float* __restrict__ viewmatrix, const float* __restrict__ projmatrix,
    int W, int H, float tan_fovx, float tan_fovy, float focal_x, float focal_y, uint32_t gx, uint32_t gy,
    int* __restrict__ radii, float* __restrict__ rec, BinInfo* __restrict__ bin, uint32_t* __restrict__ block_sums,
    uint32_t* __restrict__ depth_range, const float* __restrict__ shs, int D, int M, const float* __restrict__ cam_pos,
    uint32_t* __restrict__ clamped, uint32_t flags, uint32_t* __restrict__ depth_keys, uint32_t* __restrict__ depth_vals,
    uint2* __restrict__ ranges, int num_tiles, uint32_t* __restrict__ depth_overflow, uint32_t* __restrict__ touched_dense);
constexpr uint32_t DEPTH_KEY_MIN = 0x3E4CCCCDu;
constexpr int DEPTH_KEY_BITS = 27;

__global__ void visible_filter_kernel(
    int P, const float* __restrict__ means3D, const float* __restrict__ scales, float mod,
    const float* __restrict__ rotations, const float* __restrict__ cov3D_precomp,
    const float* __restrict__ viewmatrix, const float* __restrict__ projmatrix, int W, int H,
    float tan_fovx, float tan_fovy, float focal_x, float focal_y, uint32_t gx, uint32_t gy, int* __restrict__ radii,
    int log_scale_stride);

__global__ void mark_visible_kernel(int P, const float* __restrict__ means3D, const float* __restrict__ viewmatrix,
                                    uint8_t* __restrict__ present);

constexpr int CAM_SUMS = 24;
template <bool DEPTH, bool CAM>
__global__ void preprocess_bwd_kernel(
    int P, const float* __restrict__ means3D, const int* __restrict__ radii, const float* __restrict__ scales,
    const float* __restrict__ rotations, float mod, const float* __restrict__ cov3D_precomp,
    const float* __restrict__ view, const float* __restrict__ proj, float h_x, float h_y, float tan_fovx, float tan_fovy,
    float* __restrict__ gacc, float img_w, float img_h,
    float* __restrict__ dL_dmean2D, float* __restrict__ dL_dconic,
    float* __restrict__ dL_dopacity, float* __restrict__ dL_dcolor, float* __restrict__ dL_dmean3D,
    float* __restrict__ dL_dcov3D, float* __restrict__ dL_dscale, float* __restrict__ dL_drot, int clean_gacc,
    const float* __restrict__ dz_in, float* __restrict__ cam_partials);
__global__ void camera_grad_reduce_kernel(const float* __restrict__ partials, int nblocks, float* __restrict__ dL_dview,
                                          float* __restrict__ dL_dproj);
__global__ void sh_backward_kernel(int P, const float* __restrict__ means3D, const int* __restrict__ radii,
                                   const float* __restrict__ shs, int D, int M, const float* __restrict__ cam_pos,
                                   const uint32_t* __restrict__ clamped, const float* __restrict__ dL_dcolor,
                                   float* __restrict__ dL_dmean3D, float* __restrict__ dL_dsh);

__global__ void scan_block_sums_kernel(uint32_t* __restrict__ block_sums, int nblocks, const uint32_t* __restrict__ depth_range,
                                       uint32_t* __restrict__ total);
__global__ void ordered_offsets_kernel(int P, const uint32_t* __restrict__ block_sums, uint32_t* __restrict__ incl,
                                       uint32_t* __restrict__ total_out, const uint32_t* __restrict__ ng_dev,
                                       uint32_t* __restrict__ first_owner, uint32_t owner_entries);
__global__ void duplicate_with_keys_kernel(int P, int R, const float* __restrict__ rec,
                                           const uint32_t* __restrict__ order, const uint32_t* __restrict__ incl,
                                           uint32_t* __restrict__ keys, uint32_t* __restrict__ vals, uint32_t gx,
                                           const uint32_t* __restrict__ n_dev, int mark_dead, const uint32_t* __restrict__ ng_dev,
                                           const uint32_t* __restrict__ first_owner);
constexpr uint32_t RANGE_EMPTY_START = 0xFFFFFFFFu;
__global__ void normalize_ranges_kernel(int num_tiles, uint2* __restrict__ ranges);
constexpr uint32_t PREPROCESS_TIGHT_RECT = 0x80000000u;
constexpr uint32_t DEAD_KEY = 0xFFFFFFFFu;
template <typename K, int BITS>
__global__ void radix_count_kernel(const K* __restrict__ keys, int n, int shift, uint32_t dmin, int dbits,
                                   uint32_t* __restrict__ tile_prefix, uint32_t* __restrict__ chunk_hist, int nblocks, int nchunks,
                                   const uint32_t* __restrict__ n_dev, int drop_dead, int chunk_tiles, int nbits);
__global__ void radix_scan_kernel(uint32_t* __restrict__ block_hist, int nblocks, uint32_t* __restrict__ digit_totals);
template <typename K, int BITS, bool AUX>
__global__ void radix_scatter_kernel(const K* __restrict__ keys_in, const uint32_t* __restrict__ vals_in,
                                     K* __restrict__ keys_out, uint32_t* __restrict__ vals_out, int n, int shift,
                                     uint32_t dmin, int dbits, const uint32_t* __restrict__ tile_prefix, const uint32_t* __restrict__ chunk_prefix,
                                     const uint32_t* __restrict__ digit_totals, int nblocks, int nchunks,
                                     const uint32_t* __restrict__ n_dev, int drop_dead, uint32_t* __restrict__ n_live_out,
                                     const uint32_t* __restrict__ aux_in, uint32_t* __restrict__ aux_out, int nbits, int chunk_tiles, int pack_shift,
                                     uint2* __restrict__ ranges_out, uint32_t* __restrict__ status, uint32_t* __restrict__ status_mirror,
                                     int write_keys);
__global__ void identify_tile_ranges_kernel(int L, const uint32_t* __restrict__ keys, uint2* __restrict__ ranges,
                                            const uint32_t* __restrict__ n_dev, uint32_t* __restrict__ status,
                                            uint32_t* __restrict__ status_mirror, const uint32_t* __restrict__ n_live);

__global__ void render_fwd_kernel(const uint2* __restrict__ ranges, const uint32_t* __restrict__ point_list, int W, int H,
                                  const float* __restrict__ rec, const float* __restrict__ bg,
                                  float* __restrict__ final_T, uint32_t* __restrict__ n_contrib, float* __restrict__ out_color);
__global__ void render_bwd_kernel(const uint2* __restrict__ ranges, const uint32_t* __restrict__ point_list, int W, int H,
                                  const float* __restrict__ rec, const float* __restrict__ bg,
                                  const float* __restrict__ final_T, const uint32_t* __restrict__ n_contrib,
                                  const float* __restrict__ dL_dpix, float* __restrict__ gacc, uint32_t num_tiles);
__global__ void render_bwd_mfma_kernel(const uint2* __restrict__ ranges, const uint32_t* __restrict__ point_list, int W, int H,
                                       const float* __restrict__ rec, const float* __restrict__ bg,
                                       const float* __restrict__ final_T, const uint32_t* __restrict__ n_contrib,
                                       const float* __restrict__ dL_dpix, float* __restrict__ gacc, uint32_t num_tiles);
__global__ void render_fwd_depth_kernel(const uint2* __restrict__ ranges, const uint32_t* __restrict__ point_list, int W, int H,
                                        const float* __restrict__ rec, const float* __restrict__ bg,
                                        float* __restrict__ final_T, uint32_t* __restrict__ n_contrib, float* __restrict__ out_color,
                                        float* __restrict__ out_depth, float* __restrict__ out_alpha);
__global__ void render_bwd_depth_kernel(const uint2* __restrict__ ranges, const uint32_t* __restrict__ point_list, int W, int H,
                                        const float* __restrict__ rec, const float* __restrict__ bg,
                                        const float* __restrict__ final_T, const uint32_t* __restrict__ n_contrib,
                                        const float* __restrict__ dL_dpix, float* __restrict__ gacc, uint32_t num_tiles,
                                        const float* __restrict__ dL_ddepth, const float* __restrict__ dL_dalpha);

__global__ void unpack_geometry_kernel(int P, const float* __restrict__ rec, const BinInfo* __restrict__ bin,
                                       const int* __restrict__ radii, float* __restrict__ means2D,
                                       float* __restrict__ conic_opacity, float* __restrict__ depths,
                                       uint32_t* __restrict__ tiles_touched, float* __restrict__ rgb);

__global__ void rebuild_keys_kernel(int R, const uint32_t* __restrict__ tile_keys, const uint32_t* __restrict__ vals,
                                    const BinInfo* __restrict__ bin, uint64_t* __restrict__ keys64);
__global__ void make_depth_keys_kernel(int P, const BinInfo* __restrict__ bin, uint32_t dcull, uint32_t* __restrict__ keys,
                                       uint32_t* __restrict__ vals, uint2* __restrict__ ranges, int num_tiles);
__global__ void ordered_block_sums_kernel(int P, const uint32_t* touched, const uint32_t* __restrict__ order,
                                          uint32_t* __restrict__ block_sums, uint32_t* sorted_touched,
                                          const uint32_t* __restrict__ ng_dev, uint32_t* __restrict__ order_rw, int pack_shift);
__global__ void point_offsets_kernel(int P, const BinInfo* __restrict__ bin, uint32_t* __restrict__ offsets);
__global__ void strip_mask_kernel(int n, const uint32_t* __restrict__ vals, uint32_t* __restrict__ out);

}
```

segs-slam_amd/csrc/preprocess.hip:

```cpp
#include <hip/hip_runtime.h>
#include <cstdint>
#include "gs_layout.h"
#include "kernels.h"
#include "project_gaussian.h"
#include "sh_color.h"

#pragma clang fp contract(off)

namespace segs {

__device__ __forceinline__ float3 load_row3(const float* __restrict__ a, int P, float* lds ) {
  const int tid = threadIdx.x;
  const size_t base = (size_t)blockIdx.x * 768;
  const size_t lim = (size_t)P * 3;
#pragma unroll
  for (int k = 0; k < 3; k++) {
    const size_t i = base + k * 256 + tid;
    lds[k * 256 + tid] = i < lim ? a[i] : 0.f;
  }
  __syncthreads();
  float3 v = make_float3(lds[3 * tid], lds[3 * tid + 1], lds[3 * tid + 2]);
  __syncthreads();
  return v;
}

__device__ __forceinline__ void load_rows3(const float* __restrict__ a0, const float* __restrict__ a1, const float* __restrict__ a2,
                                           int P, float* lds , float3& v0, float3& v1, float3& v2) {
  const int tid = threadIdx.x;
  const size_t base = (size_t)blockIdx.x * 768;
  const size_t lim = (size_t)P * 3;
  const float* arr[3] = {a0, a1, a2};
  float t[3][3];
#pragma unroll
  for (int m = 0; m < 3; m++)
#pragma unroll
    for (int k = 0; k < 3; k++) {
      const size_t i = base + k * 256 + tid;
      t[m][k] = (arr[m] && i < lim) ? arr[m][i] : 0.f;
    }
#pragma unroll
  for (int m = 0; m < 3; m++)
#pragma unroll
    for (int k = 0; k < 3; k++) lds[m * 768 + k * 256 + tid] = t[m][k];
  __syncthreads();
  v0 = make_float3(lds[3 * tid], lds[3 * tid + 1], lds[3 * tid + 2]);
  v1 = make_float3(lds[768 + 3 * tid], lds[768 + 3 * tid + 1], lds[768 + 3 * tid + 2]);
  v2 = make_float3(lds[1536 + 3 * tid], lds[1536 + 3 * tid + 1], lds[1536 + 3 * tid + 2]);
  __syncthreads();
}

__global__ void __launch_bounds__(256) preprocess_fwd_kernel(
    int P, const float* __restrict__ means3D, const float* __restrict__ scales, float mod,
    const float* __restrict__ rotations, const float* __restrict__ opacities, const float* __restrict__ colors,
    const float* __restrict__ cov3D_precomp, const float* __restrict__ viewmatrix, const float* __restrict__ projmatrix,
    int W, int H, float tan_fovx, float tan_fovy, float focal_x, float focal_y, uint32_t gx, uint32_t gy,
    int* __restrict__ radii, float* __restrict__ rec, BinInfo* __restrict__ bin, uint32_t* __restrict__ block_sums,
    uint32_t* __restrict__ depth_range ,
    const float* __restrict__ shs, int D, int M, const float* __restrict__ cam_pos, uint32_t* __restrict__ clamped,
    uint32_t flags, uint32_t* __restrict__ depth_keys, uint32_t* __restrict__ depth_vals, uint2* __restrict__ ranges,
    int num_tiles, uint32_t* __restrict__ depth_overflow ,
    uint32_t* __restrict__ touched_dense) {
  __shared__ float lds[3 * 768];
  __shared__ uint32_t wave_sums[4], wave_dmax[4], wave_dnmin[4];
  const int idx = blockIdx.x * 256 + threadIdx.x;
  float4 rot = make_float4(0, 0, 0, 0);
  if (scales && idx < P) rot = reinterpret_cast<const float4*>(rotations)[idx];
  float3 p, sc, col;
  load_rows3(means3D, scales, colors, P, lds, p, sc, col);

  uint32_t touched = 0, dbits_mine = 0;
  float4 rq0 = make_float4(0, 0, 0, 0), rq1 = rq0, rq2 = rq0, rq3 = rq0;
  bool has_record = false;
  if (idx < P) {
    Projected g = project_gaussian(p, sc, mod, rot, cov3D_precomp ? cov3D_precomp + (size_t)6 * idx : nullptr,
                                   viewmatrix, projmatrix, W, H, tan_fovx, tan_fovy, focal_x, focal_y, gx, gy);
    if ((flags & 1u) && !(opacities[idx] > 0.f)) g.radius = 0;
    BinInfo b{0u, 0u, 0u, 0u};
    if (g.radius > 0) {
      const float op = opacities[idx];
      if (!colors) {
        uint32_t cb;
        col = sh::to_rgb(idx, D, M, p, cam_pos, shs, &cb);
        clamped[idx] = cb;
      }
      const BinnedRecord br = make_record(g, op, col, flags);
      touched = br.touched;
      b.depth_bits = br.depth_bits;
      dbits_mine = b.depth_bits;
      b.rect_min = br.rect_min;
      b.rect_max = br.rect_max;
      b.tiles_touched = touched;
      rq0 = br.q0; rq1 = br.q1; rq2 = br.q2; rq3 = br.q3;
      has_record = true;
    }
    radii[idx] = g.radius;
    if (!depth_keys) reinterpret_cast<uint4*>(bin)[idx] = make_uint4(b.depth_bits, b.rect_min, b.rect_max, b.tiles_touched);
    touched_dense[idx] = b.tiles_touched;
    if (depth_keys) {
      depth_keys[idx] = b.tiles_touched ? b.depth_bits : 0xFFFFFFFFu;
      (void)depth_vals;
      if (depth_overflow && b.tiles_touched && (b.depth_bits - DEPTH_KEY_MIN) >= ((1u << DEPTH_KEY_BITS) - 1u)) *depth_overflow = 1u;
    }
  }
  {
    const int lane = threadIdx.x & 63;
    float* const wl = lds + (threadIdx.x >> 6) * 576;
    const uint64_t recs = __ballot(has_record);
    const size_t wave_first = (size_t)blockIdx.x * 256 + (threadIdx.x & ~63);
#pragma unroll
    for (int half = 0; half < 2; half++) {
      if ((lane >> 5) == half) {
        float4* mine = reinterpret_cast<float4*>(wl + (lane & 31) * REC_DWORDS);
        mine[0] = rq0; mine[1] = rq1; mine[2] = rq2; mine[3] = rq3;
      }
      asm volatile("" ::: "memory");
#pragma unroll
      for (int j = 0; j < 2; j++) {
        const int r = 16 * j + (lane >> 2);
        const int owner = 32 * half + r;
        if ((recs >> owner) & 1ull)
          reinterpret_cast<float4*>(rec + (wave_first + owner) * REC_DWORDS)[lane & 3] = reinterpret_cast<const float4*>(wl + r * REC_DWORDS)[lane & 3];
      }
      asm volatile("" ::: "memory");
    }
  }
  if (ranges)
    for (int t = idx; t < num_tiles; t += gridDim.x * 256) ranges[t] = make_uint2(RANGE_EMPTY_START, 0u);
  uint32_t s = touched;
  uint32_t dmax = touched ? dbits_mine : 0u, dnmin = touched ? ~dbits_mine : 0u;
#pragma unroll
  for (int off = 32; off > 0; off >>= 1) {
    s += __shfl_down(s, off, 64);
    dmax = max(dmax, (uint32_t)__shfl_down((int)dmax, off, 64));
    dnmin = max(dnmin, (uint32_t)__shfl_down((int)dnmin, off, 64));
  }
  if ((threadIdx.x & 63) == 0) {
    wave_sums[threadIdx.x >> 6] = s; wave_dmax[threadIdx.x >> 6] = dmax; wave_dnmin[threadIdx.x >> 6] = dnmin;
  }
  __syncthreads();
  if (threadIdx.x == 0) {
    block_sums[blockIdx.x] = wave_sums[0] + wave_sums[1] + wave_sums[2] + wave_sums[3];
    depth_range[blockIdx.x] = max(max(wave_dmax[0], wave_dmax[1]), max(wave_dmax[2], wave_dmax[3]));
    depth_range[gridDim.x + blockIdx.x] = max(max(wave_dnmin[0], wave_dnmin[1]), max(wave_dnmin[2], wave_dnmin[3]));
  }
}

__global__ void __launch_bounds__(256) visible_filter_kernel(
    int P, const float* __restrict__ means3D, const float* __restrict__ scales, float mod,
    const float* __restrict__ rotations, const float* __restrict__ cov3D_precomp,
    const float* __restrict__ viewmatrix, const float* __restrict__ projmatrix, int W, int H,
    float tan_fovx, float tan_fovy, float focal_x, float focal_y, uint32_t gx, uint32_t gy, int* __restrict__ radii,
    int log_scale_stride ) {
  __shared__ float lds[768];
  const int idx = blockIdx.x * 256 + threadIdx.x;
  const float3 p = load_row3(means3D, P, lds);
  float3 sc = make_float3(0, 0, 0);
  float4 rot = make_float4(0, 0, 0, 0);
  if (scales) {
    if (log_scale_stride > 0) {
      if (idx < P) {
        const float* r = scales + (size_t)idx * log_scale_stride;
        sc = make_float3(expf(r[0]), expf(r[1]), expf(r[2]));
      }
    } else {
      sc = load_row3(scales, P, lds);
    }
    if (idx < P) rot = reinterpret_cast<const float4*>(rotations)[idx];
  }
  if (idx >= P) return;
  Projected g = project_gaussian(p, sc, mod, rot, cov3D_precomp ? cov3D_precomp + (size_t)6 * idx : nullptr,
                                 viewmatrix, projmatrix, W, H, tan_fovx, tan_fovy, focal_x, focal_y, gx, gy);
  radii[idx] = g.radius;
}

__global__ void __launch_bounds__(256) mark_visible_kernel(int P, const float* __restrict__ means3D,
                                                           const float* __restrict__ viewmatrix, uint8_t* __restrict__ present) {
  __shared__ float lds[768];
  const int idx = blockIdx.x * 256 + threadIdx.x;
  const float3 p = load_row3(means3D, P, lds);
  if (idx >= P) return;
  float3 p_view = transformPoint4x3(p, viewmatrix);
  present[idx] = (p_view.z <= 0.2f) ? 0 : 1;
}

__device__ __forceinline__ void store_row3(float* __restrict__ a, int P, float* lds , float x, float y, float z) {
  const int tid = threadIdx.x;
  lds[3 * tid] = x; lds[3 * tid + 1] = y; lds[3 * tid + 2] = z;
  __syncthreads();
  const size_t base = (size_t)blockIdx.x * 768;
  const size_t lim = (size_t)P * 3;
#pragma unroll
  for (int k = 0; k < 3; k++) {
    const size_t i = base + k * 256 + tid;
    if (i < lim) a[i] = lds[k * 256 + tid];
  }
  __syncthreads();
}

struct Sym2 { float xx, xy, yy; };

__device__ __forceinline__ void quat_rows(float4 q, float R[3][3]) {
  const float r = q.x, x = q.y, y = q.z, z = q.w;
  R[0][0] = 1.f - 2.f * (y * y + z * z); R[0][1] = 2.f * (x * y - r * z);       R[0][2] = 2.f * (x * z + r * y);
  R[1][0] = 2.f * (x * y + r * z);       R[1][1] = 1.f - 2.f * (x * x + z * z); R[1][2] = 2.f * (y * z - r * x);
  R[2][0] = 2.f * (x * z - r * y);       R[2][1] = 2.f * (y * z + r * x);       R[2][2] = 1.f - 2.f * (x * x + y * y);
}

template <bool DEPTH, bool CAM>
__global__ void __launch_bounds__(256) preprocess_bwd_kernel(
    int P, const float* __restrict__ means3D, const int* __restrict__ radii, const float* __restrict__ scales,
    const float* __restrict__ rotations, float mod, const float* __restrict__ cov3D_precomp,
    const float* __restrict__ view, const float* __restrict__ proj, float h_x, float h_y, float tan_fovx, float tan_fovy,
    float* __restrict__ gacc, float img_w, float img_h,
    float* __restrict__ dL_dmean2D, float* __restrict__ dL_dconic,
    float* __restrict__ dL_dopacity, float* __restrict__ dL_dcolor, float* __restrict__ dL_dmean3D,
    float* __restrict__ dL_dcov3D, float* __restrict__ dL_dscale, float* __restrict__ dL_drot,
    int clean_gacc ,
    const float* __restrict__ dz_in, float* __restrict__ cam_partials ) {
  __shared__ float lds[3 * 768];
  const int idx = blockIdx.x * 256 + threadIdx.x;
  const bool live = idx < P;
  const bool binned = live && radii[idx] > 0;
  float3 mean, scale, unused;
  load_rows3(means3D, scales, nullptr, P, lds, mean, scale, unused);

  float g2x = 0.f, g2y = 0.f;
  Sym2 G{0.f, 0.f, 0.f};
  float dcol0 = 0.f, dcol1 = 0.f, dcol2 = 0.f, dop = 0.f, dz = 0.f;
  float4 a0 = make_float4(0.f, 0.f, 0.f, 0.f), a1 = a0;
  if (gacc) {
    {
      __shared__ __attribute__((aligned(16))) float gl[4][32 * GACC_DWORDS];
      const int lane = threadIdx.x & 63;
      float* const wl = gl[threadIdx.x >> 6];
      const uint64_t rows = __ballot(binned);
      const size_t wave_first = (size_t)blockIdx.x * 256 + (threadIdx.x & ~63);
#pragma unroll
      for (int half = 0; half < 2; half++) {
        float4 q[2];
#pragma unroll
        for (int j = 0; j < 2; j++) {
          const int r = 16 * j + (lane >> 2), owner = 32 * half + r;
          q[j] = make_float4(0.f, 0.f, 0.f, 0.f);
          if (((rows >> owner) & 1ull) && (lane & 3) < 3) {
            float4* src = reinterpret_cast<float4*>(gacc + (wave_first + owner) * GACC_DWORDS) + (lane & 3);
            q[j] = *src;
            if (clean_gacc) *src = make_float4(0.f, 0.f, 0.f, 0.f);
          }
        }
#pragma unroll
        for (int j = 0; j < 2; j++) reinterpret_cast<float4*>(wl + (16 * j + (lane >> 2)) * GACC_DWORDS)[lane & 3] = q[j];
        asm volatile("" ::: "memory");
        if ((lane >> 5) == half) {
          const float4* mine = reinterpret_cast<const float4*>(wl + (lane & 31) * GACC_DWORDS);
          a0 = mine[0]; a1 = mine[1]; dcol2 = wl[(lane & 31) * GACC_DWORDS + 8];
          if (DEPTH) dz = wl[(lane & 31) * GACC_DWORDS + 9];
        }
        asm volatile("" ::: "memory");
      }
    }
    if (binned) {
      G.xx = -0.5f * a0.z; G.xy = -0.5f * a0.w; G.yy = -0.5f * a1.x;
      dop = a1.y;
      dcol0 = a1.z; dcol1 = a1.w;
    }
    store_row3(dL_dcolor, P, lds, dcol0, dcol1, dcol2);
    if (live) {
      if (dL_dconic) reinterpret_cast<float4*>(dL_dconic)[idx] = make_float4(G.xx, G.xy, 0.f, G.yy);
      dL_dopacity[idx] = dop;
    }
  } else if (live) {
    g2x = dL_dmean2D[3 * (size_t)idx + 0]; g2y = dL_dmean2D[3 * (size_t)idx + 1];
    G.xx = dL_dconic[4 * (size_t)idx + 0]; G.xy = dL_dconic[4 * (size_t)idx + 1]; G.yy = dL_dconic[4 * (size_t)idx + 3];
    if constexpr (CAM && DEPTH) { if (dz_in) dz = dz_in[idx]; }
  }

  float out_mean[3] = {0, 0, 0}, out_cov[6] = {0, 0, 0, 0, 0, 0}, out_scale[3] = {0, 0, 0}, out_rot[4] = {0, 0, 0, 0};
  float cam[CAM ? CAM_SUMS : 1] = {0};
  if (binned) {
    const float tx0 = view[0] * mean.x + view[4] * mean.y + view[8] * mean.z + view[12];
    const float ty0 = view[1] * mean.x + view[5] * mean.y + view[9] * mean.z + view[13];
    const float tz = view[2] * mean.x + view[6] * mean.y + view[10] * mean.z + view[14];
    const float limx = 1.3f * tan_fovx, limy = 1.3f * tan_fovy;
    const float rx = tx0 / tz, ry = ty0 / tz;
    const bool free_x = !(rx < -limx || rx > limx), free_y = !(ry < -limy || ry > limy);
    const float tx = fminf(limx, fmaxf(-limx, rx)) * tz, ty = fminf(limy, fmaxf(-limy, ry)) * tz;
    const float iz = 1.f / tz, iz2 = iz * iz;
    const float J00 = h_x * iz, J02 = -h_x * tx * iz2, J11 = h_y * iz, J12 = -h_y * ty * iz2;
    float M2[2][3];
#pragma unroll
    for (int j = 0; j < 3; j++) {
      M2[0][j] = J00 * view[4 * j] + J02 * view[4 * j + 2];
      M2[1][j] = J11 * view[4 * j + 1] + J12 * view[4 * j + 2];
    }
    float R[3][3] = {{0, 0, 0}, {0, 0, 0}, {0, 0, 0}}, s3[3] = {0, 0, 0};
    float4 q = make_float4(0, 0, 0, 0);
    float E[2][3];
    float U[2][3] = {{0, 0, 0}, {0, 0, 0}};
    float a, b, c;
    if (cov3D_precomp) {
      const float* cv = cov3D_precomp + (size_t)6 * idx;
      const float S[3][3] = {{cv[0], cv[1], cv[2]}, {cv[1], cv[3], cv[4]}, {cv[2], cv[4], cv[5]}};
#pragma unroll
      for (int r = 0; r < 2; r++)
#pragma unroll
        for (int j = 0; j < 3; j++) E[r][j] = M2[r][0] * S[0][j] + M2[r][1] * S[1][j] + M2[r][2] * S[2][j];
      a = E[0][0] * M2[0][0] + E[0][1] * M2[0][1] + E[0][2] * M2[0][2] + 0.3f;
      b = E[0][0] * M2[1][0] + E[0][1] * M2[1][1] + E[0][2] * M2[1][2];
      c = E[1][0] * M2[1][0] + E[1][1] * M2[1][1] + E[1][2] * M2[1][2] + 0.3f;
    } else {
      q = reinterpret_cast<const float4*>(rotations)[idx];
      quat_rows(q, R);
      s3[0] = mod * scale.x; s3[1] = mod * scale.y; s3[2] = mod * scale.z;
#pragma unroll
      for (int r = 0; r < 2; r++)
#pragma unroll
        for (int k = 0; k < 3; k++) U[r][k] = (M2[r][0] * R[0][k] + M2[r][1] * R[1][k] + M2[r][2] * R[2][k]) * s3[k];
#pragma unroll
      for (int r = 0; r < 2; r++)
#pragma unroll
        for (int j = 0; j < 3; j++) E[r][j] = U[r][0] * R[j][0] * s3[0] + U[r][1] * R[j][1] * s3[1] + U[r][2] * R[j][2] * s3[2];
      a = U[0][0] * U[0][0] + U[0][1] * U[0][1] + U[0][2] * U[0][2] + 0.3f;
      b = U[0][0] * U[1][0] + U[0][1] * U[1][1] + U[0][2] * U[1][2];
      c = U[1][0] * U[1][0] + U[1][1] * U[1][1] + U[1][2] * U[1][2] + 0.3f;
    }
    const float det = a * c - b * b;
    const float k = 1.0f / (det * det + 0.0000001f);
    if (gacc) {
      const float di = 1.0f / det;
      const float cA = c * di, cB = -b * di, cC = a * di;
      g2x = -(cA * a0.x + cB * a0.y) * (0.5f * img_w);
      g2y = -(cC * a0.y + cB * a0.x) * (0.5f * img_h);
    }
    const float h0 = c * G.xx - b * G.xy, h1 = c * G.xy - b * G.yy;
    const float h2 = a * G.xy - b * G.xx, h3 = a * G.yy - b * G.xy;
    Sym2 Dc;
    Dc.xx = -k * (h0 * c - h1 * b);
    Dc.xy = -k * (h1 * a - h0 * b);
    Dc.yy = -k * (h3 * a - h2 * b);
    float DM[2][3];
#pragma unroll
    for (int j = 0; j < 3; j++) { DM[0][j] = Dc.xx * M2[0][j] + Dc.xy * M2[1][j]; DM[1][j] = Dc.xy * M2[0][j] + Dc.yy * M2[1][j]; }
    if (dL_dcov3D || cov3D_precomp) {
      const int ii[6] = {0, 0, 0, 1, 1, 2}, jj[6] = {0, 1, 2, 1, 2, 2};
#pragma unroll
      for (int e = 0; e < 6; e++) {
        const float v = M2[0][ii[e]] * DM[0][jj[e]] + M2[1][ii[e]] * DM[1][jj[e]];
        out_cov[e] = ii[e] == jj[e] ? v : 2.f * v;
      }
    }
    float dM2[2][3];
#pragma unroll
    for (int j = 0; j < 3; j++) {
      dM2[0][j] = 2.f * (Dc.xx * E[0][j] + Dc.xy * E[1][j]);
      dM2[1][j] = 2.f * (Dc.xy * E[0][j] + Dc.yy * E[1][j]);
    }
    const float dJ00 = dM2[0][0] * view[0] + dM2[0][1] * view[4] + dM2[0][2] * view[8];
    const float dJ02 = dM2[0][0] * view[2] + dM2[0][1] * view[6] + dM2[0][2] * view[10];
    const float dJ11 = dM2[1][0] * view[1] + dM2[1][1] * view[5] + dM2[1][2] * view[9];
    const float dJ12 = dM2[1][0] * view[2] + dM2[1][1] * view[6] + dM2[1][2] * view[10];
    const float iz3 = iz2 * iz;
    const float dtx = free_x ? -h_x * iz2 * dJ02 : 0.f;
    const float dty = free_y ? -h_y * iz2 * dJ12 : 0.f;
    const float dtz = -h_x * iz2 * dJ00 - h_y * iz2 * dJ11 + 2.f * h_x * tx * iz3 * dJ02 + 2.f * h_y * ty * iz3 * dJ12;
    const float hx = proj[0] * mean.x + proj[4] * mean.y + proj[8] * mean.z + proj[12];
    const float hy = proj[1] * mean.x + proj[5] * mean.y + proj[9] * mean.z + proj[13];
    const float hw = proj[3] * mean.x + proj[7] * mean.y + proj[11] * mean.z + proj[15];
    const float w = 1.0f / (hw + 0.0000001f);
    const float ux = hx * w * w, uy = hy * w * w;
#pragma unroll
    for (int j = 0; j < 3; j++) {
      const float from_cov = view[4 * j] * dtx + view[4 * j + 1] * dty + view[4 * j + 2] * dtz;
      const float from_proj = (proj[4 * j] * w - proj[4 * j + 3] * ux) * g2x + (proj[4 * j + 1] * w - proj[4 * j + 3] * uy) * g2y;
      out_mean[j] = from_cov + from_proj;
    }
    if (DEPTH) {
#pragma unroll
      for (int j = 0; j < 3; j++) out_mean[j] += dz * view[4 * j + 2];
    }
    if constexpr (CAM) {
      const float dtz_all = DEPTH ? dtz + dz : dtz;
      const float pm[3] = {mean.x, mean.y, mean.z};
      const float dh0 = g2x * w, dh1 = g2y * w, dh3 = -(g2x * hx + g2y * hy) * (w * w);
#pragma unroll
      for (int j = 0; j < 3; j++) {
        cam[3 * j + 0] = dtx * pm[j] + J00 * dM2[0][j];
        cam[3 * j + 1] = dty * pm[j] + J11 * dM2[1][j];
        cam[3 * j + 2] = dtz_all * pm[j] + (J02 * dM2[0][j] + J12 * dM2[1][j]);
        cam[12 + 3 * j + 0] = dh0 * pm[j];
        cam[12 + 3 * j + 1] = dh1 * pm[j];
        cam[12 + 3 * j + 2] = dh3 * pm[j];
      }
      cam[9] = dtx; cam[10] = dty; cam[11] = dtz_all;
      cam[21] = dh0; cam[22] = dh1; cam[23] = dh3;
    }
    if (scales) {
      float DU[2][3];
#pragma unroll
      for (int kk = 0; kk < 3; kk++) { DU[0][kk] = Dc.xx * U[0][kk] + Dc.xy * U[1][kk]; DU[1][kk] = Dc.xy * U[0][kk] + Dc.yy * U[1][kk]; }
      float GR[3][3];
#pragma unroll
      for (int kk = 0; kk < 3; kk++) {
        float ds = 0.f;
#pragma unroll
        for (int i = 0; i < 3; i++) {
          const float dLik = 2.f * (M2[0][i] * DU[0][kk] + M2[1][i] * DU[1][kk]);
          ds += R[i][kk] * dLik;
          GR[i][kk] = dLik * s3[kk];
        }
        out_scale[kk] = ds;
      }
      const float r = q.x, x = q.y, y = q.z, z = q.w;
      out_rot[0] = 2.f * (z * (GR[1][0] - GR[0][1]) + y * (GR[0][2] - GR[2][0]) + x * (GR[2][1] - GR[1][2]));
      out_rot[1] = 2.f * (y * (GR[0][1] + GR[1][0]) + z * (GR[0][2] + GR[2][0]) + r * (GR[2][1] - GR[1][2])) - 4.f * x * (GR[1][1] + GR[2][2]);
      out_rot[2] = 2.f * (x * (GR[0][1] + GR[1][0]) + r * (GR[0][2] - GR[2][0]) + z * (GR[1][2] + GR[2][1])) - 4.f * y * (GR[0][0] + GR[2][2]);
      out_rot[3] = 2.f * (r * (GR[1][0] - GR[0][1]) + x * (GR[0][2] + GR[2][0]) + y * (GR[1][2] + GR[2][1])) - 4.f * z * (GR[0][0] + GR[1][1]);
    }
  }
  if constexpr (CAM) {
    const int v = threadIdx.x >> 5, l = threadIdx.x & 31;
#pragma unroll
    for (int pass = 0; pass < CAM_SUMS / 8; pass++) {
#pragma unroll
      for (int k = 0; k < 8; k++) lds[k * 256 + threadIdx.x] = cam[pass * 8 + k];
      __syncthreads();
      float s = lds[v * 256 + l];
#pragma unroll
      for (int q = 1; q < 8; q++) s += lds[v * 256 + l + 32 * q];
#pragma unroll
      for (int off = 16; off > 0; off >>= 1) s += __shfl_down(s, off, 64);
      if (l == 0) cam_partials[(size_t)blockIdx.x * CAM_SUMS + pass * 8 + v] = s;
      __syncthreads();
    }
  }
  if (gacc) store_row3(dL_dmean2D, P, lds, g2x, g2y, 0.f);
  store_row3(dL_dmean3D, P, lds, out_mean[0], out_mean[1], out_mean[2]);
  if (dL_dscale) store_row3(dL_dscale, P, lds, out_scale[0], out_scale[1], out_scale[2]);
  if (!live) return;
  if (dL_dcov3D) {
#pragma unroll
    for (int e = 0; e < 6; e++) dL_dcov3D[6 * (size_t)idx + e] = out_cov[e];
  }
  if (dL_drot) reinterpret_cast<float4*>(dL_drot)[idx] = make_float4(out_rot[0], out_rot[1], out_rot[2], out_rot[3]);
}

#define SEGS_PREPROCESS_BWD_ARGS int, const float*, const int*, const float*, const float*, float, const float*, const float*, \
    const float*, float, float, float, float, float*, float, float, float*, float*, float*, float*, float*, float*, float*, float*, int, \
    const float*, float*
template __global__ void preprocess_bwd_kernel<false, false>(SEGS_PREPROCESS_BWD_ARGS);
template __global__ void preprocess_bwd_kernel<true, false>(SEGS_PREPROCESS_BWD_ARGS);
template __global__ void preprocess_bwd_kernel<false, true>(SEGS_PREPROCESS_BWD_ARGS);
template __global__ void preprocess_bwd_kernel<true, true>(SEGS_PREPROCESS_BWD_ARGS);
#undef SEGS_PREPROCESS_BWD_ARGS

__global__ void __launch_bounds__(960) camera_grad_reduce_kernel(const float* __restrict__ partials, int nblocks,
                                                                 float* __restrict__ dL_dview, float* __restrict__ dL_dproj) {
  __shared__ float rows[160 * CAM_SUMS];
  __shared__ float mid[10 * CAM_SUMS];
  __shared__ float sums[CAM_SUMS];
  const int t = threadIdx.x, q = t % 6, r0 = t / 6;
  float4 acc = make_float4(0.f, 0.f, 0.f, 0.f);
#pragma unroll 8
  for (int r = r0; r < nblocks; r += 160) {
    const float4 x = reinterpret_cast<const float4*>(partials + (size_t)r * CAM_SUMS)[q];
    acc.x += x.x; acc.y += x.y; acc.z += x.z; acc.w += x.w;
  }
  reinterpret_cast<float4*>(rows + r0 * CAM_SUMS)[q] = acc;
  __syncthreads();
  if (t < 10 * CAM_SUMS) {
    const int v = t % CAM_SUMS, g = t / CAM_SUMS;
    float s = 0.f;
    for (int k = 0; k < 16; k++) s += rows[(16 * g + k) * CAM_SUMS + v];
    mid[g * CAM_SUMS + v] = s;
  }
  __syncthreads();
  if (t < CAM_SUMS) {
    float s = 0.f;
    for (int g = 0; g < 10; g++) s += mid[g * CAM_SUMS + t];
    sums[t] = s;
  }
  __syncthreads();
  if (t < 32) {
    const int e = t & 15, i = e & 3, j = e >> 2;
    if (t < 16) dL_dview[e] = i < 3 ? sums[3 * j + i] : 0.f;
    else dL_dproj[e] = i != 2 ? sums[12 + 3 * j + (i == 3 ? 2 : i)] : 0.f;
  }
}

__global__ void __launch_bounds__(256) sh_backward_kernel(int P, const float* __restrict__ means3D, const int* __restrict__ radii,
                                                          const float* __restrict__ shs, int D, int M, const float* __restrict__ cam_pos,
                                                          const uint32_t* __restrict__ clamped, const float* __restrict__ dL_dcolor,
                                                          float* __restrict__ dL_dmean3D, float* __restrict__ dL_dsh) {
  const int idx = blockIdx.x * 256 + threadIdx.x;
  if (idx >= P || radii[idx] <= 0) return;
  const float3 mean = make_float3(means3D[3 * (size_t)idx], means3D[3 * (size_t)idx + 1], means3D[3 * (size_t)idx + 2]);
  const float3 dcol = make_float3(dL_dcolor[3 * (size_t)idx], dL_dcolor[3 * (size_t)idx + 1], dL_dcolor[3 * (size_t)idx + 2]);
  const float3 g = sh::backward(idx, D, M, mean, cam_pos, shs, clamped[idx], dcol, dL_dsh);
  dL_dmean3D[3 * (size_t)idx] += g.x; dL_dmean3D[3 * (size_t)idx + 1] += g.y; dL_dmean3D[3 * (size_t)idx + 2] += g.z;
}

}
```

segs-slam_amd/csrc/render.hip:

```cpp
#include <hip/hip_runtime.h>
#include <cstdint>
#include "gs_layout.h"
#include "kernels.h"

namespace segs {

__device__ __forceinline__ uint32_t xcd_tile(uint32_t wg, uint32_t num_tiles) {
  const uint32_t full = num_tiles & ~63u;
  if (wg >= full) return wg;
  const uint32_t xcd = wg & 7u, local = wg >> 3;
  return (local >> 3) * 64u + xcd * 8u + (local & 7u);
}

__device__ __forceinline__ float fast_exp2(float x) { return __builtin_amdgcn_exp2f(x); }
__device__ __forceinline__ float fast_rcp(float x) { return __builtin_amdgcn_rcpf(x); }
__device__ __forceinline__ uint32_t readlane_u32(uint32_t v, int lane) {
  return (uint32_t)__builtin_amdgcn_readlane((int)v, lane);
}


__device__ __forceinline__ float rl(float v, int lane) {
  return __int_as_float(__builtin_amdgcn_readlane(__float_as_int(v), lane));
}

__device__ __forceinline__ void wave_lds_fence() { asm volatile("" ::: "memory"); }

struct Compacted { uint32_t val; uint32_t pos; int n; };
template <bool REVERSE>
__device__ __forceinline__ Compacted compact_chunk(uint32_t v, uint32_t qbit, int lane) {
  const bool rel = (v & qbit) != 0u;
  const uint64_t m = __ballot(rel);
  const int n = __popcll(m);
  const int below = (int)__builtin_amdgcn_mbcnt_hi((uint32_t)(m >> 32), __builtin_amdgcn_mbcnt_lo((uint32_t)m, 0u));
  const int rank = REVERSE ? (n - 1 - below) : below;
  const int dest = rel ? rank : n + (lane - below);
  Compacted c;
  c.val = (uint32_t)__builtin_amdgcn_ds_permute(dest << 2, (int)v);
  c.pos = (uint32_t)__builtin_amdgcn_ds_permute(dest << 2, lane);
  c.n = n;
  return c;
}

constexpr int FWD_REC = 12;

template <bool DEPTH>
__device__ __forceinline__ void load_rec_tail(const float4* p, float& rb, float& rz) {
  if (DEPTH) { const float2 t = reinterpret_cast<const float2*>(p)[4]; rb = t.x; rz = t.y; }
  else rb = reinterpret_cast<const float*>(p)[8];
}

template <bool DEPTH>
__device__ __forceinline__ void render_fwd_body(
    const uint2* __restrict__ ranges, const uint32_t* __restrict__ point_list, int W, int H,
    const float* __restrict__ rec, const float* __restrict__ bg, float* __restrict__ final_T,
    uint32_t* __restrict__ n_contrib, float* __restrict__ out_color, float* __restrict__ out_depth,
    float* __restrict__ out_alpha) {
  __shared__ float4 s_rec[4][64][FWD_REC / 4];
  const uint32_t tiles_x = (W + TILE_X - 1) / TILE_X;
  const uint32_t tile = xcd_tile(blockIdx.x, gridDim.x);
  const uint32_t tile_x = tile % tiles_x, tile_y = tile / tiles_x;
  const int lane = threadIdx.x & 63;
  const int wv = __builtin_amdgcn_readfirstlane(threadIdx.x >> 6);
  const uint32_t px = tile_x * TILE_X + (wv & 1) * 8 + (lane & 7);
  const uint32_t py = tile_y * TILE_Y + (wv >> 1) * 8 + (lane >> 3);
  const bool inside = px < (uint32_t)W && py < (uint32_t)H;
  const float pxf = (float)px, pyf = (float)py;
  const uint32_t qbit = 1u << (ID_BITS + wv);

  const uint2 range = ranges[tile];
  float T = inside ? 1.0f : 0.f, thr = inside ? 0.0001f : -1.f;
  float Tfin = 0.f, C0 = 0.f, C1 = 0.f, C2 = 0.f, Dz = 0.f;
  uint32_t last = 0u, lastfin = 0u;

  uint32_t v_nxt, v_nn = 0u;
  Compacted cc;
  float4 r0, r1; float rb, rz = 0.f;
  {
    const uint32_t i0 = range.x + lane, i1 = range.x + 64 + lane;
    const uint32_t v0 = i0 < range.y ? point_list[i0] : 0u;
    v_nxt = i1 < range.y ? point_list[i1] : 0u;
    cc = compact_chunk<false>(v0, qbit, lane);
    r0 = make_float4(0.f, 0.f, 0.f, 0.f); r1 = r0; rb = 0.f;
    if (lane < cc.n) {
      const float4* p = reinterpret_cast<const float4*>(rec + (size_t)(cc.val & ID_MASK) * REC_DWORDS);
      r0 = p[0]; r1 = p[1]; load_rec_tail<DEPTH>(p, rb, rz);
    }
  }
  bool alive = true;
  for (uint32_t base = range.x; base < range.y && alive; base += 64) {
    const int n = __builtin_amdgcn_readfirstlane(cc.n);
    const int n4 = (n + 3) & ~3;
    if (lane < n4) {
      const bool real = lane < n;
      s_rec[wv][lane][0] = real ? r0 : make_float4(0.f, 0.f, 0.f, 0.f);
      s_rec[wv][lane][1] = real ? r1 : make_float4(0.f, 0.f, 0.f, 0.f);
      s_rec[wv][lane][2] = make_float4(real ? rb : 0.f, __uint_as_float(base - range.x + cc.pos + 1u), (DEPTH && real) ? rz : 0.f, 0.f);
    }
    wave_lds_fence();
    {
      const uint32_t i2 = base + 128 + lane;
      v_nn = i2 < range.y ? point_list[i2] : 0u;
      cc = compact_chunk<false>(v_nxt, qbit, lane);
      if (lane < cc.n) {
        const float4* p = reinterpret_cast<const float4*>(rec + (size_t)(cc.val & ID_MASK) * REC_DWORDS);
        r0 = p[0]; r1 = p[1]; load_rec_tail<DEPTH>(p, rb, rz);
      }
      v_nxt = v_nn;
    }
    for (int k0 = 0; k0 < n4 && alive; k0 += 4) {
#pragma unroll
    for (int u = 0; u < 4; u++) {
      const int k = k0 + u;
      const float4 q0 = s_rec[wv][k][0], q1 = s_rec[wv][k][1];
      const float2 q2 = *reinterpret_cast<const float2*>(&s_rec[wv][k][2]);
      const float qz = DEPTH ? s_rec[wv][k][2].z : 0.f;
      const float dx = q0.x - pxf, dy = q0.y - pyf;
      const float power2 = dx * (q0.z * dx + q0.w * dy) + (q1.x * dy) * dy;
      const float alpha = fminf(0.99f, q1.y * fast_exp2(power2));
      const bool ok = power2 <= 0.0f && alpha >= 1.0f / 255.0f;
      const float ae = ok ? alpha : 0.f;
      float w = ae * T;
      float test_T = T - w;
      const bool stop = test_T < thr;
      if (__ballot(stop) != 0ull) {
        Tfin = stop ? T : Tfin;
        lastfin = stop ? last : lastfin;
        thr = stop ? -1.f : thr;
        w = stop ? 0.f : w;
        test_T = stop ? 0.f : test_T;
        alive = __ballot(thr > 0.f) != 0ull;
      }
      T = test_T;
      C0 += q1.z * w; C1 += q1.w * w; C2 += q2.x * w;
      if (DEPTH) Dz += qz * w;
      last = ok ? __float_as_uint(q2.y) : last;
      if (!alive) break;
    }
    }
  }
  if (inside) {
    const bool dead = thr < 0.f;
    const size_t pix_id = (size_t)W * py + px;
    const size_t HW = (size_t)H * W;
    const float Tout = dead ? Tfin : T;
    final_T[pix_id] = Tout;
    n_contrib[pix_id] = dead ? lastfin : last;
    out_color[pix_id] = C0 + Tout * bg[0];
    out_color[HW + pix_id] = C1 + Tout * bg[1];
    out_color[2 * HW + pix_id] = C2 + Tout * bg[2];
    if (DEPTH) {
      if (out_depth) out_depth[pix_id] = Dz;
      if (out_alpha) out_alpha[pix_id] = 1.0f - Tout;
    }
  }
}

__global__ void __launch_bounds__(256) render_fwd_kernel(
    const uint2* __restrict__ ranges, const uint32_t* __restrict__ point_list, int W, int H,
    const float* __restrict__ rec, const float* __restrict__ bg, float* __restrict__ final_T,
    uint32_t* __restrict__ n_contrib, float* __restrict__ out_color) {
  render_fwd_body<false>(ranges, point_list, W, H, rec, bg, final_T, n_contrib, out_color, nullptr, nullptr);
}
__global__ void __launch_bounds__(256) render_fwd_depth_kernel(
    const uint2* __restrict__ ranges, const uint32_t* __restrict__ point_list, int W, int H,
    const float* __restrict__ rec, const float* __restrict__ bg, float* __restrict__ final_T,
    uint32_t* __restrict__ n_contrib, float* __restrict__ out_color, float* __restrict__ out_depth,
    float* __restrict__ out_alpha) {
  render_fwd_body<true>(ranges, point_list, W, H, rec, bg, final_T, n_contrib, out_color, out_depth, out_alpha);
}

__device__ __forceinline__ float fold32(float a, float b) {
  auto r = __builtin_amdgcn_permlane32_swap(__float_as_uint(a), __float_as_uint(b), false, false);
  return __uint_as_float(r[0]) + __uint_as_float(r[1]);
}
__device__ __forceinline__ float fold16(float x, float y) {
  auto r = __builtin_amdgcn_permlane16_swap(__float_as_uint(x), __float_as_uint(y), false, false);
  return __uint_as_float(r[0]) + __uint_as_float(r[1]);
}
__device__ __forceinline__ float fold_rows4(float a, float b, float c, float d) {
  return fold16(fold32(a, b), fold32(c, d));
}

template <int I>
__device__ __forceinline__ void fmac_row_bcast(float& acc, float v, float a) {
  asm("v_fmac_f32_dpp %0, %1, %2 row_newbcast:%3 row_mask:0xf bank_mask:0xf bound_ctrl:1" : "+v"(acc) : "v"(v), "v"(a), "n"(I));
}
constexpr int BW_SLOTS = 16;
constexpr int BW_STRIDE = 65;
struct BwdLds {
  float4 rec[BW_SLOTS][3];
  float2 wa[BW_SLOTS][BW_STRIDE];
};


template <bool USE_BG, bool DEPTH>
__device__ __forceinline__ void pixel_role(BwdLds& L, int nb, int lane, float pxf, float pyf, uint32_t last_contributor,
                                           float dp0, float dp1, float dp2, float dpz, float T_final, float bg_dot_dpixel,
                                           float& T, float& accd) {
#ifndef PIX_UNROLL
#define PIX_UNROLL 4
#endif
#pragma unroll PIX_UNROLL
  for (int sl = 0; sl < nb; sl++) {
    const float4 q0 = L.rec[sl][0], q1 = L.rec[sl][1];
    const float2 q2 = *reinterpret_cast<const float2*>(&L.rec[sl][2]);
    const float qz = DEPTH ? L.rec[sl][2].w : 0.f;
    const float dx = q0.x - pxf, dy = q0.y - pyf;
    const float power2 = dx * (q0.z * dx + q0.w * dy) + (q1.x * dy) * dy;
#if defined(SEGS_MEASURE) && defined(ABLATE_NO_TRANS)
    const float ar = q1.y * (power2 * 0.001f + 1.0f);
#else
    const float ar = q1.y * fast_exp2(power2);
#endif
    const bool ok = __float_as_uint(q2.y) < last_contributor && power2 <= 0.0f && ar >= 1.0f / 255.0f;
    const float aw = ok ? ar : 0.f;
    const float ae = fminf(0.99f, aw);
#if defined(SEGS_MEASURE) && defined(ABLATE_NO_TRANS)
    const float rinv = 1.f + ae;
#else
    const float rinv = fast_rcp(1.f - ae);
#endif
    T = T * rinv;
    const float diff = (DEPTH ? (q1.z * dp0 + q1.w * dp1 + q2.x * dp2 + qz * dpz) : (q1.z * dp0 + q1.w * dp1 + q2.x * dp2)) - accd;
    float dL_dalpha = diff * T;
    if (USE_BG) dL_dalpha += (-T_final * rinv) * bg_dot_dpixel;
    accd += ae * diff;
    L.wa[sl][lane] = make_float2(aw * dL_dalpha , ae * T );
  }
}

typedef float f32x4 __attribute__((ext_vector_type(4)));

template <bool MFMA, bool DEPTH>
__device__ __forceinline__ void render_bwd_body(
    const uint2* __restrict__ ranges, const uint32_t* __restrict__ point_list, int W, int H,
    const float* __restrict__ rec, const float* __restrict__ bg, const float* __restrict__ final_T,
    const uint32_t* __restrict__ n_contrib, const float* __restrict__ dL_dpix, float* __restrict__ gacc, uint32_t num_tiles,
    const float* __restrict__ dL_ddepth, const float* __restrict__ dL_dalpha) {
  static_assert(!(MFMA && DEPTH), "the depth form of the tile backward is the VALU form");
  __shared__ BwdLds lds_one;
  const uint32_t tiles_x = (W + TILE_X - 1) / TILE_X;
  const uint32_t xcd = blockIdx.x & 7u, local = blockIdx.x >> 3;
  const uint32_t v = ((local >> 2) << 3) | xcd;
  if (v >= num_tiles) return;
  const uint32_t tile = xcd_tile(v, num_tiles);
  const uint32_t tile_x = tile % tiles_x, tile_y = tile / tiles_x;
  const int lane = threadIdx.x & 63;
  const int wv = __builtin_amdgcn_readfirstlane((int)(local & 3u));
  BwdLds& L = lds_one;
  const uint32_t qx0 = tile_x * TILE_X + (wv & 1) * 8, qy0 = tile_y * TILE_Y + (wv >> 1) * 8;
  const uint32_t px = qx0 + (lane & 7), py = qy0 + (lane >> 3);
  const bool inside = px < (uint32_t)W && py < (uint32_t)H;
  const float pxf = (float)px, pyf = (float)py;
  const size_t pix_id = (size_t)W * py + px;
  const size_t HW = (size_t)H * W;
  const uint32_t qbit = 1u << (ID_BITS + wv);

  const uint2 range = ranges[tile];
  const float T_final = inside ? final_T[pix_id] : 0.f;
  const uint32_t last_contributor = inside ? n_contrib[pix_id] : 0u;
  float dp0 = 0.f, dp1 = 0.f, dp2 = 0.f;
  if (inside) { dp0 = dL_dpix[pix_id]; dp1 = dL_dpix[HW + pix_id]; dp2 = dL_dpix[2 * HW + pix_id]; }
  float dpz = 0.f, dpa = 0.f;
  if (DEPTH && inside) { dpz = dL_ddepth ? dL_ddepth[pix_id] : 0.f; dpa = dL_dalpha ? dL_dalpha[pix_id] : 0.f; }
  const float bg_dot_dpixel = DEPTH ? (bg[0] * dp0 + bg[1] * dp1 + bg[2] * dp2) - dpa : bg[0] * dp0 + bg[1] * dp1 + bg[2] * dp2;
  const bool use_bg = __ballot(bg_dot_dpixel != 0.f) != 0ull;

  uint32_t wave_last = last_contributor;
#pragma unroll
  for (int off = 32; off > 0; off >>= 1) wave_last = max(wave_last, (uint32_t)__shfl_xor((int)wave_last, off, 64));
  wave_last = __builtin_amdgcn_readfirstlane(wave_last);
  if (wave_last == 0u) return;

  float T = T_final, accd = 0.f;

  const int gs = lane & 15, part = lane >> 4;
  const float pyl0 = (float)(part * 2), pyl1 = pyl0 + 1.0f;
  const float qx0f = (float)qx0, qy0f = (float)qy0;

  float bmono[16], bcol[16];
  if (MFMA) {
    float* dps = reinterpret_cast<float*>(&L.wa[0][0]);
    dps[lane] = dp0; dps[64 + lane] = dp1; dps[128 + lane] = dp2;
    wave_lds_fence();
    const float j1 = gs == 1 ? 1.f : 0.f, j3 = gs == 3 ? 1.f : 0.f, j4 = gs == 4 ? 1.f : 0.f;
    const bool colour = gs >= 6 && gs < 9;
    const int crow = colour ? (gs - 6) * 64 + part * 16 : 0;
#pragma unroll
    for (int h = 0; h < 2; h++) {
      const float y = (float)(2 * part + h) - 3.5f;
      const float c0 = gs == 0 ? 1.f : gs == 2 ? y : gs == 5 ? y * y : 0.f;
      const float c1 = j1 + j4 * y;
#pragma unroll
      for (int c = 0; c < 8; c++) {
        const float x = (float)c - 3.5f;
        bmono[8 * h + c] = c0 + x * (c1 + x * j3);
      }
    }
#pragma unroll
    for (int t = 0; t < 16; t++) { const float v = dps[crow + t]; bcol[t] = colour ? v : 0.f; }
    wave_lds_fence();
  }

  const int32_t cfirst = (int32_t)((wave_last - 1u) & ~63u);
  uint32_t v_nxt = 0u;
  Compacted cc;
  float4 r0, r1; float rb, rz = 0.f;
  {
    const uint32_t p0 = (uint32_t)cfirst + lane;
    const uint32_t v0 = p0 < wave_last ? point_list[range.x + p0] : 0u;
    if (cfirst >= 64) v_nxt = point_list[range.x + (uint32_t)(cfirst - 64) + lane];
    cc = compact_chunk<true>(v0, qbit, lane);
    r0 = make_float4(0.f, 0.f, 0.f, 0.f); r1 = r0; rb = 0.f;
    if (lane < cc.n) {
      const float4* p = reinterpret_cast<const float4*>(rec + (size_t)(cc.val & ID_MASK) * REC_DWORDS);
      r0 = p[0]; r1 = p[1]; load_rec_tail<DEPTH>(p, rb, rz);
    }
  }
  float (*mom)[12] = reinterpret_cast<float (*)[12]>(&L.wa[0][0]);
  int fill = 0;
  for (int32_t cbase = cfirst;; cbase -= 64) {
    const bool tail = cbase < 0;
    const int n = tail ? 0 : __builtin_amdgcn_readfirstlane(cc.n);
    const float4 c0 = r0, c1 = r1;
    const float4 c2 = make_float4(rb, __uint_as_float((uint32_t)cbase + cc.pos), __uint_as_float(cc.val & ID_MASK), DEPTH ? rz : 0.f);
    if (cbase >= 64) {
      uint32_t v_nn = 0u;
      if (cbase >= 128) v_nn = point_list[range.x + (uint32_t)(cbase - 128) + lane];
      cc = compact_chunk<true>(v_nxt, qbit, lane);
      if (lane < cc.n) {
        const float4* p = reinterpret_cast<const float4*>(rec + (size_t)(cc.val & ID_MASK) * REC_DWORDS);
        r0 = p[0]; r1 = p[1]; load_rec_tail<DEPTH>(p, rb, rz);
      }
      v_nxt = v_nn;
    }
    int taken = 0;
    do {
      const int take = min(BW_SLOTS - fill, n - taken);
      if (lane >= taken && lane < taken + take) {
        const int s = fill + lane - taken;
        L.rec[s][0] = c0; L.rec[s][1] = c1; L.rec[s][2] = c2;
      }
      fill += take; taken += take;
      if (fill < BW_SLOTS && !(tail && fill > 0)) continue;
      const int nb = fill;
      fill = 0;
      wave_lds_fence();
      if (use_bg) pixel_role<true, DEPTH>(L, nb, lane, pxf, pyf, last_contributor, dp0, dp1, dp2, dpz, T_final, bg_dot_dpixel, T, accd);
      else pixel_role<false, DEPTH>(L, nb, lane, pxf, pyf, last_contributor, dp0, dp1, dp2, dpz, T_final, bg_dot_dpixel, T, accd);
      wave_lds_fence();
#if defined(SEGS_MEASURE) && defined(ABLATE_NO_GAUSS_ROLE)
      continue;
#endif
      const float2 gxy = *reinterpret_cast<const float2*>(&L.rec[gs][0]);
      const float gxr = gxy.x - qx0f, gyr = gxy.y - qy0f;
      float cx, cy;
      if (MFMA) {
        cx = 3.5f; cy = 3.5f;
        f32x4 dw = {0.f, 0.f, 0.f, 0.f}, da = {0.f, 0.f, 0.f, 0.f};
        const float2* warow = &L.wa[gs][part * 16];
#pragma unroll
        for (int t = 0; t < 16; t++) {
          const float2 wa_t = warow[t];
#ifdef SEGS_MFMA_ONE_CHAIN
          dw = __builtin_amdgcn_mfma_f32_16x16x4f32(wa_t.x, bmono[t], dw, 0, 0, 0);
          dw = __builtin_amdgcn_mfma_f32_16x16x4f32(wa_t.y, bcol[t], dw, 0, 0, 0);
#else
          dw = __builtin_amdgcn_mfma_f32_16x16x4f32(wa_t.x, bmono[t], dw, 0, 0, 0);
          da = __builtin_amdgcn_mfma_f32_16x16x4f32(wa_t.y, bcol[t], da, 0, 0, 0);
#endif
        }
        if (gs < 9) {
#pragma unroll
          for (int r = 0; r < 4; r++) mom[4 * part + r][gs] = dw[r] + da[r];
        }
      } else {
      cx = fminf(7.f, fmaxf(0.f, rintf(gxr))); cy = fminf(7.f, fmaxf(0.f, rintf(gyr)));
      float px8[8], px8q[8];
#pragma unroll
      for (int c = 0; c < 8; c++) { px8[c] = (float)c - cx; px8q[c] = px8[c] * px8[c]; }
      const float pyc0 = pyl0 - cy, pyc1 = pyl1 - cy;
      float S0, S1x, S1y, Sxx, Sxy, Syy, Sr = 0.f, Sg = 0.f, Sb = 0.f, Sz = 0.f;
      {
        float R0[2] = {0.f, 0.f}, R1[2] = {0.f, 0.f}, R2[2] = {0.f, 0.f};
        const float2* warow = &L.wa[gs][part * 16];
#define GAUSS_STEP(i)                                                                         \
        {                                                                                     \
          const float2 wa_i = warow[i];                                                       \
          const float w = wa_i.x, a = wa_i.y;                                                 \
          R0[(i) >> 3] += w; R1[(i) >> 3] += w * px8[(i) & 7]; R2[(i) >> 3] += w * px8q[(i) & 7]; \
          fmac_row_bcast<(i)>(Sr, dp0, a); fmac_row_bcast<(i)>(Sg, dp1, a); fmac_row_bcast<(i)>(Sb, dp2, a); \
          if (DEPTH) fmac_row_bcast<(i)>(Sz, dpz, a);                                         \
        }
        GAUSS_STEP(0) GAUSS_STEP(1) GAUSS_STEP(2) GAUSS_STEP(3) GAUSS_STEP(4) GAUSS_STEP(5) GAUSS_STEP(6) GAUSS_STEP(7)
        GAUSS_STEP(8) GAUSS_STEP(9) GAUSS_STEP(10) GAUSS_STEP(11) GAUSS_STEP(12) GAUSS_STEP(13) GAUSS_STEP(14) GAUSS_STEP(15)
#undef GAUSS_STEP
        S0 = R0[0] + R0[1]; S1x = R1[0] + R1[1]; Sxx = R2[0] + R2[1];
        S1y = pyc0 * R0[0] + pyc1 * R0[1];
        Sxy = pyc0 * R1[0] + pyc1 * R1[1];
        Syy = (pyc0 * pyc0) * R0[0] + (pyc1 * pyc1) * R0[1];
      }
      const float g1 = fold_rows4(S0, S1y, S1x, Sxx);
      const float g2 = fold_rows4(Sxy, Sr, Syy, Sg);
      if (DEPTH) {
        const float g3 = fold_rows4(Sb, Sz, Sb, Sz);
        mom[gs][part] = g1;
        mom[gs][4 + part] = g2;
        if ((part & 1) == 0) mom[gs][8 + (part >> 1)] = g3;
      } else {
      const float g3 = fold_rows4(Sb, Sb, Sb, Sb);
      mom[gs][part] = g1;
      mom[gs][4 + part] = g2;
      if (part == 0) mom[gs][8] = g3;
      }
      }
      wave_lds_fence();
      {
        const float4 m0 = *reinterpret_cast<const float4*>(&mom[gs][0]);
        const float4 m1 = *reinterpret_cast<const float4*>(&mom[gs][4]);
        const float m8 = mom[gs][8];
        const float hx = gxr - cx, hy = gyr - cy;
        const float Mx = hx * m0.x - m0.y, My = hy * m0.x - m0.z;
        const float Mxx = hx * (hx * m0.x - 2.f * m0.y) + m0.w;
        const float Mxy = hx * (hy * m0.x - m0.z) - hy * m0.y + m1.x;
        const float Myy = hy * (hy * m0.x - 2.f * m0.z) + m1.y;
        wave_lds_fence();
        const float inv_o = fast_rcp(reinterpret_cast<const float*>(&L.rec[gs][1])[1]);
        wave_lds_fence();
        if (part == 0) {
          *reinterpret_cast<float4*>(&mom[gs][0]) = make_float4(Mx, My, Mxx, Mxy);
          *reinterpret_cast<float4*>(&mom[gs][4]) = make_float4(Myy, m0.x * inv_o, m1.z, m1.w);
          mom[gs][8] = m8;
        }
      }
      wave_lds_fence();
#pragma unroll
      for (int j = 0; j < 4; j++) {
        const int slot = 4 * j + part;
        if (slot < nb && gs < (DEPTH ? 10 : 9)) {
          const uint32_t id = __float_as_uint(reinterpret_cast<const float*>(&L.rec[slot][2])[2]);
#if !(defined(SEGS_MEASURE) && defined(ABLATE_NO_ATOMICS))
          atomicAdd(gacc + (size_t)id * GACC_DWORDS + gs, mom[slot][gs]);
#endif
        }
      }
      wave_lds_fence();
    } while (taken < n);
    if (tail) break;
  }
}

__global__ void __launch_bounds__(64) render_bwd_kernel(
    const uint2* __restrict__ ranges, const uint32_t* __restrict__ point_list, int W, int H,
    const float* __restrict__ rec, const float* __restrict__ bg, const float* __restrict__ final_T,
    const uint32_t* __restrict__ n_contrib, const float* __restrict__ dL_dpix, float* __restrict__ gacc, uint32_t num_tiles) {
  render_bwd_body<false, false>(ranges, point_list, W, H, rec, bg, final_T, n_contrib, dL_dpix, gacc, num_tiles, nullptr, nullptr);
}
__global__ void __launch_bounds__(64) render_bwd_mfma_kernel(
    const uint2* __restrict__ ranges, const uint32_t* __restrict__ point_list, int W, int H,
    const float* __restrict__ rec, const float* __restrict__ bg, const float* __restrict__ final_T,
    const uint32_t* __restrict__ n_contrib, const float* __restrict__ dL_dpix, float* __restrict__ gacc, uint32_t num_tiles) {
  render_bwd_body<true, false>(ranges, point_list, W, H, rec, bg, final_T, n_contrib, dL_dpix, gacc, num_tiles, nullptr, nullptr);
}
__global__ void __launch_bounds__(64) render_bwd_depth_kernel(
    const uint2* __restrict__ ranges, const uint32_t* __restrict__ point_list, int W, int H,
    const float* __restrict__ rec, const float* __restrict__ bg, const float* __restrict__ final_T,
    const uint32_t* __restrict__ n_contrib, const float* __restrict__ dL_dpix, float* __restrict__ gacc, uint32_t num_tiles,
    const float* __restrict__ dL_ddepth, const float* __restrict__ dL_dalpha) {
  render_bwd_body<false, true>(ranges, point_list, W, H, rec, bg, final_T, n_contrib, dL_dpix, gacc, num_tiles, dL_ddepth, dL_dalpha);
}

}
```

Measured before the change: 1008 iters/s.

## Skip non-contributing gaussians in tile backward and track hit rows for preprocess

The tile backward pass now records, for each batch of gaussians, which slots actually contributed to any pixel in the wave. Batches with no contributor skip the gaussian-role moment computation entirely, and only contributing slots issue atomic adds into the gradient accumulator. A per-gaussian hit byte is set for contributors and consumed (and cleared) by the preprocess backward, which then skips unhit rows instead of every binned row. The cost is an extra ballot per slot, scattered byte stores, padding of the slot records, a new per-gaussian buffer, and a debug counting kernel.

```diff
diff --git a/include/segs_raster.h b/include/segs_raster.h
--- a/include/segs_raster.h
+++ b/include/segs_raster.h
@@ -80,6 +80,7 @@
 int segs_debug_unpack_binning(const char* binning_buffer, const char* geom_buffer, int P, int R, int width, int height,
                               uint64_t* keys_sorted , uint32_t* point_list , void* stream);
 int segs_debug_instance_values(const char* binning_buffer, int R, uint32_t* values , void* stream);
+int segs_debug_accumulator_state(const char* geom_buffer, int geom_rows, uint32_t* counts , void* stream);
 int segs_debug_unpack_image(const char* image_buffer, int width, int height, uint32_t* ranges ,
                             float* final_T , uint32_t* n_contrib , void* stream);
 
diff --git a/segs-slam_amd/_capi.py b/segs-slam_amd/_capi.py
--- a/segs-slam_amd/_capi.py
+++ b/segs-slam_amd/_capi.py
@@ -83,6 +83,7 @@
                                   _vp, _vp, _vp, _vp]),
     "segs_debug_unpack_geometry": (_i, [_vp, _i, _vp, _vp, _vp, _vp, _vp, _vp, _vp, _vp]),
     "segs_debug_instance_values": (_i, [_vp, _i, _vp, _vp]),
+    "segs_debug_accumulator_state": (_i, [_vp, _i, _vp, _vp]),
     "segs_debug_unpack_binning": (_i, [_vp, _vp, _i, _i, _i, _i, _vp, _vp, _vp]),
     "segs_debug_unpack_image": (_i, [_vp, _i, _i, _vp, _vp, _vp, _vp]),
     "segs_debug_preprocess_backward": (_i, [_i, _i, _i, _vp, _vp, _vp, _f, _vp, _vp, _vp, _vp, _f, _f, _vp, _vp, _vp,
diff --git a/segs-slam_amd/csrc/binning.hip b/segs-slam_amd/csrc/binning.hip
--- a/segs-slam_amd/csrc/binning.hip
+++ b/segs-slam_amd/csrc/binning.hip
@@ -573,6 +573,23 @@
   }
 }
 
+__global__ void __launch_bounds__(256) accumulator_state_kernel(int rows, const float* __restrict__ gacc, const uint8_t* __restrict__ hit,
+                                                               uint32_t* __restrict__ counts) {
+  const int idx = blockIdx.x * 256 + threadIdx.x;
+  bool nonzero = false, set = false;
+  if (idx < rows) {
+    const uint4* r = reinterpret_cast<const uint4*>(gacc + (size_t)idx * GACC_DWORDS);
+#pragma unroll
+    for (int j = 0; j < GACC_DWORDS / 4; j++) { const uint4 v = r[j]; nonzero = nonzero || (v.x | v.y | v.z | v.w) != 0u; }
+    set = hit[idx] != 0;
+  }
+  const uint64_t a = __ballot(nonzero), b = __ballot(set);
+  if ((threadIdx.x & 63) == 0) {
+    if (a) atomicAdd(&counts[0], (uint32_t)__popcll(a));
+    if (b) atomicAdd(&counts[1], (uint32_t)__popcll(b));
+  }
+}
+
 __global__ void __launch_bounds__(256) unpack_geometry_kernel(
     int P, const float* __restrict__ rec, const BinInfo* __restrict__ bin, const int* __restrict__ radii,
     float* __restrict__ means2D, float* __restrict__ conic_opacity, float* __restrict__ depths,
diff --git a/segs-slam_amd/csrc/capi.hip b/segs-slam_amd/csrc/capi.hip
--- a/segs-slam_amd/csrc/capi.hip
+++ b/segs-slam_amd/csrc/capi.hip
@@ -168,6 +168,7 @@
   uint32_t* clamped() const { return (uint32_t*)(base + L.clamped); }
   float* gacc() const { return (float*)(base + L.gacc); }
   uint32_t* touched() const { return (uint32_t*)(base + L.touched); }
+  uint8_t* hit() const { return (uint8_t*)(base + L.hit); }
 };
 Geom geom_at(char* p, int P) { return Geom{geom_layout(P), align_ptr(p)}; }
 Geom geom_at(char* p, int P, int rows) {
@@ -471,12 +472,13 @@
   const float* dL_ddepth = dgrad ? dgrad->dL_ddepth : nullptr;
   const float* dL_dalpha = dgrad ? dgrad->dL_dalpha : nullptr;
   const bool depth_form = dL_ddepth || dL_dalpha;
+  uint8_t* const hit = self_clean ? G.hit() : nullptr;
   if (R > 0 && depth_form) {
     { PROF(K_RENDER_BWD);
     render_bwd_depth_kernel<<<(gx * gy + 7) / 8 * 32, 64, 0, st>>>((const uint2*)(img + IL.ranges), (const uint32_t*)(bin + BL.vals[0]), width,
                                                                   height, G.rec(), background, (const float*)(img + IL.final_T),
                                                                   (const uint32_t*)(img + IL.n_contrib), dL_dpix, G.gacc(), gx * gy,
-                                                                  dL_ddepth, dL_dalpha);
+                                                                  dL_ddepth, dL_dalpha, hit);
     }
     LAUNCH_TRY("render_bwd_depth_kernel");
   } else if (R > 0) {
@@ -484,7 +486,7 @@
     static const bool mfma_env = [] { const char* e = getenv("SEGS_RENDER_BWD_MFMA"); return e && e[0] == '1'; }();
     ((mfma_env || (g_flags & SEGS_RASTER_MFMA_MOMENTS)) ? render_bwd_mfma_kernel : render_bwd_kernel)<<<(gx * gy + 7) / 8 * 32, 64, 0, st>>>((const uint2*)(img + IL.ranges), (const uint32_t*)(bin + BL.vals[0]), width,
                                                     height, G.rec(), background, (const float*)(img + IL.final_T),
-                                                    (const uint32_t*)(img + IL.n_contrib), dL_dpix, G.gacc(), gx * gy);
+                                                    (const uint32_t*)(img + IL.n_contrib), dL_dpix, G.gacc(), gx * gy, hit);
     }
     LAUNCH_TRY("render_bwd_kernel");
   }
@@ -495,7 +497,7 @@
                                                      scale_modifier, cov3D_precomp, viewmatrix, projmatrix, focal_x, focal_y,
                                                      tan_fovx, tan_fovy, G.gacc(), (float)width, (float)height, dL_dmean2D, dL_dconic, dL_dopacity, dL_dcolor,
                                                      dL_dmean3D, dL_dcov3D, dL_dscale, dL_drot, self_clean ? 1 : 0, nullptr,
-                                                     cam_live ? camera_partials(cam) : nullptr);
+                                                     cam_live ? camera_partials(cam) : nullptr, hit);
   LAUNCH_TRY("preprocess_bwd_kernel");
   if (cam_live)
     if (int rc = camera_grads_finish(cam, G.L.nblocks, st)) return rc;
@@ -646,6 +648,18 @@
   return SEGS_OK;
 }
 
+int segs_debug_accumulator_state(const char* geom_buffer, int geom_rows, uint32_t* counts, void* stream) {
+  hipStream_t st = (hipStream_t)stream;
+  if (geom_rows < 0 || geom_rows > MAX_GAUSSIANS) return fail(SEGS_ERR_INVALID_ARGUMENT, "bad geom_rows");
+  if (!geom_buffer || !counts) return fail(SEGS_ERR_INVALID_ARGUMENT, "null pointer");
+  HIP_TRY(hipMemsetAsync(counts, 0, 2 * sizeof(uint32_t), st));
+  if (geom_rows == 0) return SEGS_OK;
+  const Geom G = geom_at(const_cast<char*>(geom_buffer), geom_rows);
+  accumulator_state_kernel<<<(geom_rows + 255) / 256, 256, 0, st>>>(geom_rows, G.gacc(), G.hit(), counts);
+  LAUNCH_TRY("accumulator_state_kernel");
+  return SEGS_OK;
+}
+
 int segs_debug_unpack_image(const char* image_buffer, int width, int height, uint32_t* ranges, float* final_T,
                             uint32_t* n_contrib, void* stream) {
   hipStream_t st = (hipStream_t)stream;
@@ -677,7 +691,7 @@
                                                          scale_modifier, cov3D_precomp, viewmatrix, projmatrix, focal_x, focal_y,
                                                          tan_fovx, tan_fovy, nullptr, (float)width, (float)height, const_cast<float*>(dL_dmean2D),
                                                          const_cast<float*>(dL_dconic), nullptr, nullptr, dL_dmean3D, dL_dcov3D,
-                                                         dL_dscale, dL_drot, 0, nullptr, nullptr);
+                                                         dL_dscale, dL_drot, 0, nullptr, nullptr, nullptr);
   LAUNCH_TRY("preprocess_bwd_kernel");
   return SEGS_OK;
 }
@@ -703,7 +717,7 @@
   (dL_dz ? preprocess_bwd_kernel<true, true> : preprocess_bwd_kernel<false, true>)<<<nblocks, 256, 0, st>>>(
       P, means3D, radii, cov3D_precomp ? nullptr : scales, rotations, scale_modifier, cov3D_precomp, viewmatrix, projmatrix, focal_x,
       focal_y, tan_fovx, tan_fovy, nullptr, (float)width, (float)height, const_cast<float*>(dL_dmean2D), const_cast<float*>(dL_dconic),
-      nullptr, nullptr, dL_dmean3D, dL_dcov3D, dL_dscale, dL_drot, 0, dL_dz, camera_partials(camera_grads));
+      nullptr, nullptr, dL_dmean3D, dL_dcov3D, dL_dscale, dL_drot, 0, dL_dz, camera_partials(camera_grads), nullptr);
   LAUNCH_TRY("preprocess_bwd_kernel");
   return camera_grads_finish(camera_grads, nblocks, st);
 }
diff --git a/segs-slam_amd/csrc/gs_layout.h b/segs-slam_amd/csrc/gs_layout.h
--- a/segs-slam_amd/csrc/gs_layout.h
+++ b/segs-slam_amd/csrc/gs_layout.h
@@ -25,7 +25,7 @@
 inline size_t align_up(size_t v, size_t a = ALIGN) { return (v + a - 1) / a * a; }
 
 struct GeomLayout {
-  size_t rec, bin, offsets, radii_internal, block_sums, clamped, num_rendered, gacc, touched, total;
+  size_t rec, bin, offsets, radii_internal, block_sums, clamped, num_rendered, gacc, touched, hit, total;
   int P, nblocks;
 };
 inline GeomLayout geom_layout(int P) {
@@ -42,6 +42,7 @@
   g.num_rendered = o;   o = align_up(o + 64);
   g.gacc = o;           o = align_up(o + (size_t)P * GACC_DWORDS * 4);
   g.touched = o;        o = align_up(o + (size_t)P * 4);
+  g.hit = o;            o = align_up(o + (size_t)P);
   g.total = o + ALIGN;
   return g;
 }
diff --git a/segs-slam_amd/csrc/kernels.h b/segs-slam_amd/csrc/kernels.h
--- a/segs-slam_amd/csrc/kernels.h
+++ b/segs-slam_amd/csrc/kernels.h
@@ -41,7 +41,7 @@
     float* __restrict__ dL_dmean2D, float* __restrict__ dL_dconic,
     float* __restrict__ dL_dopacity, float* __restrict__ dL_dcolor, float* __restrict__ dL_dmean3D,
     float* __restrict__ dL_dcov3D, float* __restrict__ dL_dscale, float* __restrict__ dL_drot, int clean_gacc,
-    const float* __restrict__ dz_in, float* __restrict__ cam_partials);
+    const float* __restrict__ dz_in, float* __restrict__ cam_partials, uint8_t* __restrict__ hit);
 __global__ void camera_grad_reduce_kernel(const float* __restrict__ partials, int nblocks, float* __restrict__ dL_dview,
                                           float* __restrict__ dL_dproj);
 __global__ void sh_backward_kernel(int P, const float* __restrict__ means3D, const int* __restrict__ radii,
@@ -87,11 +87,13 @@
 __global__ void render_bwd_kernel(const uint2* __restrict__ ranges, const uint32_t* __restrict__ point_list, int W, int H,
                                   const float* __restrict__ rec, const float* __restrict__ bg,
                                   const float* __restrict__ final_T, const uint32_t* __restrict__ n_contrib,
-                                  const float* __restrict__ dL_dpix, float* __restrict__ gacc, uint32_t num_tiles);
+                                  const float* __restrict__ dL_dpix, float* __restrict__ gacc, uint32_t num_tiles,
+                                  uint8_t* __restrict__ hit);
 __global__ void render_bwd_mfma_kernel(const uint2* __restrict__ ranges, const uint32_t* __restrict__ point_list, int W, int H,
                                        const float* __restrict__ rec, const float* __restrict__ bg,
                                        const float* __restrict__ final_T, const uint32_t* __restrict__ n_contrib,
-                                       const float* __restrict__ dL_dpix, float* __restrict__ gacc, uint32_t num_tiles);
+                                       const float* __restrict__ dL_dpix, float* __restrict__ gacc, uint32_t num_tiles,
+                                       uint8_t* __restrict__ hit);
 __global__ void render_fwd_depth_kernel(const uint2* __restrict__ ranges, const uint32_t* __restrict__ point_list, int W, int H,
                                         const float* __restrict__ rec, const float* __restrict__ bg,
                                         float* __restrict__ final_T, uint32_t* __restrict__ n_contrib, float* __restrict__ out_color,
@@ -100,8 +102,11 @@
                                         const float* __restrict__ rec, const float* __restrict__ bg,
                                         const float* __restrict__ final_T, const uint32_t* __restrict__ n_contrib,
                                         const float* __restrict__ dL_dpix, float* __restrict__ gacc, uint32_t num_tiles,
-                                        const float* __restrict__ dL_ddepth, const float* __restrict__ dL_dalpha);
+                                        const float* __restrict__ dL_ddepth, const float* __restrict__ dL_dalpha,
+                                        uint8_t* __restrict__ hit);
 
+__global__ void accumulator_state_kernel(int rows, const float* __restrict__ gacc, const uint8_t* __restrict__ hit,
+                                         uint32_t* __restrict__ counts);
 __global__ void unpack_geometry_kernel(int P, const float* __restrict__ rec, const BinInfo* __restrict__ bin,
                                        const int* __restrict__ radii, float* __restrict__ means2D,
                                        float* __restrict__ conic_opacity, float* __restrict__ depths,
diff --git a/segs-slam_amd/csrc/preprocess.hip b/segs-slam_amd/csrc/preprocess.hip
--- a/segs-slam_amd/csrc/preprocess.hip
+++ b/segs-slam_amd/csrc/preprocess.hip
@@ -216,11 +216,18 @@
     float* __restrict__ dL_dopacity, float* __restrict__ dL_dcolor, float* __restrict__ dL_dmean3D,
     float* __restrict__ dL_dcov3D, float* __restrict__ dL_dscale, float* __restrict__ dL_drot,
     int clean_gacc ,
-    const float* __restrict__ dz_in, float* __restrict__ cam_partials ) {
+    const float* __restrict__ dz_in, float* __restrict__ cam_partials ,
+    uint8_t* __restrict__ hit ) {
   __shared__ float lds[3 * 768];
   const int idx = blockIdx.x * 256 + threadIdx.x;
   const bool live = idx < P;
   const bool binned = live && radii[idx] > 0;
+  bool live_row = binned;
+  if (hit) {
+    const bool marked = live && hit[idx] != 0;
+    if (marked) hit[idx] = 0;
+    live_row = binned && marked;
+  }
   float3 mean, scale, unused;
   load_rows3(means3D, scales, nullptr, P, lds, mean, scale, unused);
 
@@ -233,7 +240,7 @@
       __shared__ __attribute__((aligned(16))) float gl[4][32 * GACC_DWORDS];
       const int lane = threadIdx.x & 63;
       float* const wl = gl[threadIdx.x >> 6];
-      const uint64_t rows = __ballot(binned);
+      const uint64_t rows = __ballot(live_row);
       const size_t wave_first = (size_t)blockIdx.x * 256 + (threadIdx.x & ~63);
 #pragma unroll
       for (int half = 0; half < 2; half++) {
@@ -259,7 +266,7 @@
         asm volatile("" ::: "memory");
       }
     }
-    if (binned) {
+    if (live_row) {
       G.xx = -0.5f * a0.z; G.xy = -0.5f * a0.w; G.yy = -0.5f * a1.x;
       dop = a1.y;
       dcol0 = a1.z; dcol1 = a1.w;
@@ -277,7 +284,7 @@
 
   float out_mean[3] = {0, 0, 0}, out_cov[6] = {0, 0, 0, 0, 0, 0}, out_scale[3] = {0, 0, 0}, out_rot[4] = {0, 0, 0, 0};
   float cam[CAM ? CAM_SUMS : 1] = {0};
-  if (binned) {
+  if (live_row) {
     const float tx0 = view[0] * mean.x + view[4] * mean.y + view[8] * mean.z + view[12];
     const float ty0 = view[1] * mean.x + view[5] * mean.y + view[9] * mean.z + view[13];
     const float tz = view[2] * mean.x + view[6] * mean.y + view[10] * mean.z + view[14];
@@ -446,7 +453,7 @@
 
 #define SEGS_PREPROCESS_BWD_ARGS int, const float*, const int*, const float*, const float*, float, const float*, const float*, \
     const float*, float, float, float, float, float*, float, float, float*, float*, float*, float*, float*, float*, float*, float*, int, \
-    const float*, float*
+    const float*, float*, uint8_t*
 template __global__ void preprocess_bwd_kernel<false, false>(SEGS_PREPROCESS_BWD_ARGS);
 template __global__ void preprocess_bwd_kernel<true, false>(SEGS_PREPROCESS_BWD_ARGS);
 template __global__ void preprocess_bwd_kernel<false, true>(SEGS_PREPROCESS_BWD_ARGS);
diff --git a/segs-slam_amd/csrc/render.hip b/segs-slam_amd/csrc/render.hip
--- a/segs-slam_amd/csrc/render.hip
+++ b/segs-slam_amd/csrc/render.hip
@@ -186,6 +186,9 @@
   asm("v_fmac_f32_dpp %0, %1, %2 row_newbcast:%3 row_mask:0xf bank_mask:0xf bound_ctrl:1" : "+v"(acc) : "v"(v), "v"(a), "n"(I));
 }
 constexpr int BW_SLOTS = 16;
+#ifndef PIX_UNROLL
+#define PIX_UNROLL 4
+#endif
 constexpr int BW_STRIDE = 65;
 struct BwdLds {
   float4 rec[BW_SLOTS][3];
@@ -196,12 +199,12 @@
 template <bool USE_BG, bool DEPTH>
 __device__ __forceinline__ void pixel_role(BwdLds& L, int nb, int lane, float pxf, float pyf, uint32_t last_contributor,
                                            float dp0, float dp1, float dp2, float dpz, float T_final, float bg_dot_dpixel,
-                                           float& T, float& accd) {
-#ifndef PIX_UNROLL
-#define PIX_UNROLL 4
-#endif
-#pragma unroll PIX_UNROLL
-  for (int sl = 0; sl < nb; sl++) {
+                                           float& T, float& accd, uint32_t& hitmask) {
+  static_assert(BW_SLOTS % PIX_UNROLL == 0, "the batch is evaluated in whole groups of PIX_UNROLL slots");
+  for (int sl0 = 0; sl0 < nb; sl0 += PIX_UNROLL) {
+#pragma unroll
+  for (int u = 0; u < PIX_UNROLL; u++) {
+    const int sl = sl0 + u;
     const float4 q0 = L.rec[sl][0], q1 = L.rec[sl][1];
     const float2 q2 = *reinterpret_cast<const float2*>(&L.rec[sl][2]);
     const float qz = DEPTH ? L.rec[sl][2].w : 0.f;
@@ -213,6 +216,7 @@
     const float ar = q1.y * fast_exp2(power2);
 #endif
     const bool ok = __float_as_uint(q2.y) < last_contributor && power2 <= 0.0f && ar >= 1.0f / 255.0f;
+    if (__ballot(ok) != 0ull) hitmask |= 1u << sl;
     const float aw = ok ? ar : 0.f;
     const float ae = fminf(0.99f, aw);
 #if defined(SEGS_MEASURE) && defined(ABLATE_NO_TRANS)
@@ -227,16 +231,22 @@
     accd += ae * diff;
     L.wa[sl][lane] = make_float2(aw * dL_dalpha , ae * T );
   }
+  }
 }
 
 typedef float f32x4 __attribute__((ext_vector_type(4)));
+
+#ifdef SEGS_MEASURE
+__device__ uint32_t* g_measure_counts = nullptr;
+__device__ uint32_t g_measure_cap = 0u;
+#endif
 
 template <bool MFMA, bool DEPTH>
 __device__ __forceinline__ void render_bwd_body(
     const uint2* __restrict__ ranges, const uint32_t* __restrict__ point_list, int W, int H,
     const float* __restrict__ rec, const float* __restrict__ bg, const float* __restrict__ final_T,
     const uint32_t* __restrict__ n_contrib, const float* __restrict__ dL_dpix, float* __restrict__ gacc, uint32_t num_tiles,
-    const float* __restrict__ dL_ddepth, const float* __restrict__ dL_dalpha) {
+    const float* __restrict__ dL_ddepth, const float* __restrict__ dL_dalpha, uint8_t* __restrict__ hit) {
   static_assert(!(MFMA && DEPTH), "the depth form of the tile backward is the VALU form");
   __shared__ BwdLds lds_one;
   const uint32_t tiles_x = (W + TILE_X - 1) / TILE_X;
@@ -319,6 +329,9 @@
   }
   float (*mom)[12] = reinterpret_cast<float (*)[12]>(&L.wa[0][0]);
   int fill = 0;
+#ifdef SEGS_MEASURE
+  uint32_t m_walked = 0u, m_contrib = 0u, m_batches = 0u, m_empty = 0u;
+#endif
   for (int32_t cbase = cfirst;; cbase -= 64) {
     const bool tail = cbase < 0;
     const int n = tail ? 0 : __builtin_amdgcn_readfirstlane(cc.n);
@@ -345,10 +358,20 @@
       if (fill < BW_SLOTS && !(tail && fill > 0)) continue;
       const int nb = fill;
       fill = 0;
+      if (lane >= nb && lane < ((nb + PIX_UNROLL - 1) & ~(PIX_UNROLL - 1))) {
+        const float4 z = make_float4(0.f, 0.f, 0.f, 0.f);
+        L.rec[lane][0] = z; L.rec[lane][1] = z; L.rec[lane][2] = z;
+      }
       wave_lds_fence();
-      if (use_bg) pixel_role<true, DEPTH>(L, nb, lane, pxf, pyf, last_contributor, dp0, dp1, dp2, dpz, T_final, bg_dot_dpixel, T, accd);
-      else pixel_role<false, DEPTH>(L, nb, lane, pxf, pyf, last_contributor, dp0, dp1, dp2, dpz, T_final, bg_dot_dpixel, T, accd);
+      uint32_t hitmask = 0u;
+      if (use_bg) pixel_role<true, DEPTH>(L, nb, lane, pxf, pyf, last_contributor, dp0, dp1, dp2, dpz, T_final, bg_dot_dpixel, T, accd, hitmask);
+      else pixel_role<false, DEPTH>(L, nb, lane, pxf, pyf, last_contributor, dp0, dp1, dp2, dpz, T_final, bg_dot_dpixel, T, accd, hitmask);
       wave_lds_fence();
+#ifdef SEGS_MEASURE
+      m_walked += (uint32_t)nb; m_contrib += (uint32_t)__popc(hitmask); m_batches++; m_empty += hitmask == 0u ? 1u : 0u;
+#endif
+      if (hitmask == 0u) continue;
+      if (hit && lane < nb && ((hitmask >> lane) & 1u)) hit[__float_as_uint(L.rec[lane][2].z)] = 1;
 #if defined(SEGS_MEASURE) && defined(ABLATE_NO_GAUSS_ROLE)
       continue;
 #endif
@@ -437,7 +460,7 @@
 #pragma unroll
       for (int j = 0; j < 4; j++) {
         const int slot = 4 * j + part;
-        if (slot < nb && gs < (DEPTH ? 10 : 9)) {
+        if (slot < nb && ((hitmask >> slot) & 1u) && gs < (DEPTH ? 10 : 9)) {
           const uint32_t id = __float_as_uint(reinterpret_cast<const float*>(&L.rec[slot][2])[2]);
 #if !(defined(SEGS_MEASURE) && defined(ABLATE_NO_ATOMICS))
           atomicAdd(gacc + (size_t)id * GACC_DWORDS + gs, mom[slot][gs]);
@@ -448,26 +471,42 @@
     } while (taken < n);
     if (tail) break;
   }
+#ifdef SEGS_MEASURE
+  if (lane == 0 && g_measure_counts && blockIdx.x < g_measure_cap) {
+    uint32_t* row = g_measure_counts + (size_t)blockIdx.x * 4;
+    row[0] = m_walked; row[1] = m_contrib; row[2] = m_batches; row[3] = m_empty;
+  }
+#endif
 }
 
 __global__ void __launch_bounds__(64) render_bwd_kernel(
-    const uint2* __restrict__ ranges, const uint32_t* __restrict__ point_list, int W, int H,
-    const float* __restrict__ rec, const float* __restrict__ bg, const float* __restrict__ final_T,
-    const uint32_t* __restrict__ n_contrib, const float* __restrict__ dL_dpix, float* __restrict__ gacc, uint32_t num_tiles) {
-  render_bwd_body<false, false>(ranges, point_list, W, H, rec, bg, final_T, n_contrib, dL_dpix, gacc, num_tiles, nullptr, nullptr);
-}
-__global__ void __launch_bounds__(64) render_bwd_mfma_kernel(
-    const uint2* __restrict__ ranges, const uint32_t* __restrict__ point_list, int W, int H,
-    const float* __restrict__ rec, const float* __restrict__ bg, const float* __restrict__ final_T,
-    const uint32_t* __restrict__ n_contrib, const float* __restrict__ dL_dpix, float* __restrict__ gacc, uint32_t num_tiles) {
-  render_bwd_body<true, false>(ranges, point_list, W, H, rec, bg, final_T, n_contrib, dL_dpix, gacc, num_tiles, nullptr, nullptr);
-}
-__global__ void __launch_bounds__(64) render_bwd_depth_kernel(
     const uint2* __restrict__ ranges, const uint32_t* __restrict__ point_list, int W, int H,
     const float* __restrict__ rec, const float* __restrict__ bg, const float* __restrict__ final_T,
     const uint32_t* __restrict__ n_contrib, const float* __restrict__ dL_dpix, float* __restrict__ gacc, uint32_t num_tiles,
-    const float* __restrict__ dL_ddepth, const float* __restrict__ dL_dalpha) {
-  render_bwd_body<false, true>(ranges, point_list, W, H, rec, bg, final_T, n_contrib, dL_dpix, gacc, num_tiles, dL_ddepth, dL_dalpha);
-}
-
-}
+    uint8_t* __restrict__ hit) {
+  render_bwd_body<false, false>(ranges, point_list, W, H, rec, bg, final_T, n_contrib, dL_dpix, gacc, num_tiles, nullptr, nullptr, hit);
+}
+__global__ void __launch_bounds__(64) render_bwd_mfma_kernel(
+    const uint2* __restrict__ ranges, const uint32_t* __restrict__ point_list, int W, int H,
+    const float* __restrict__ rec, const float* __restrict__ bg, const float* __restrict__ final_T,
+    const uint32_t* __restrict__ n_contrib, const float* __restrict__ dL_dpix, float* __restrict__ gacc, uint32_t num_tiles,
+    uint8_t* __restrict__ hit) {
+  render_bwd_body<true, false>(ranges, point_list, W, H, rec, bg, final_T, n_contrib, dL_dpix, gacc, num_tiles, nullptr, nullptr, hit);
+}
+__global__ void __launch_bounds__(64) render_bwd_depth_kernel(
+    const uint2* __restrict__ ranges, const uint32_t* __restrict__ point_list, int W, int H,
+    const float* __restrict__ rec, const float* __restrict__ bg, const float* __restrict__ final_T,
+    const uint32_t* __restrict__ n_contrib, const float* __restrict__ dL_dpix, float* __restrict__ gacc, uint32_t num_tiles,
+    const float* __restrict__ dL_ddepth, const float* __restrict__ dL_dalpha, uint8_t* __restrict__ hit) {
+  render_bwd_body<false, true>(ranges, point_list, W, H, rec, bg, final_T, n_contrib, dL_dpix, gacc, num_tiles, dL_ddepth, dL_dalpha, hit);
+}
+
+}
+
+#ifdef SEGS_MEASURE
+extern "C" int segs_measure_rows(uint32_t* counts, uint32_t cap) {
+  if (hipMemcpyToSymbol(HIP_SYMBOL(segs::g_measure_counts), &counts, sizeof(counts)) != hipSuccess) return 1;
+  if (hipMemcpyToSymbol(HIP_SYMBOL(segs::g_measure_cap), &cap, sizeof(cap)) != hipSuccess) return 1;
+  return 0;
+}
+#endif
```

New measurement: 1016 iters/s (median of 6 runs). Within noise of the previous version (+0.7%).
